# edshkim98/LocalDiffusion-Hallucination

Hardware: AMD Instinct MI355X
Metric: local patches/sec (256^2, T=1000) (higher is better)
Workload: dtype bf16; 1 GPU; cfg3: 8 local patches (vertical band masks) of one 3x256x256 image per GPU, 4-stage dim-32 conditional UNet (12.1M params), DDPM T=1000, pred_x0, sigmoid schedule; patches_per_gpu=8, parallelism=patch-sharded x1, one all-gather per sample, step_graph_replay=True, whole_batch_graph_flag=False, concurrent_sub_batches=2, weight_split_levels=0

## Files before the change

include/localdiff_hip.h:

```cpp
#ifndef LOCALDIFF_HIP_H
#define LOCALDIFF_HIP_H

#include <stddef.h>
#include <stdint.h>

#ifdef __cplusplus
extern "C" {
#endif

#define LD_OK 0
#define LD_EINVAL (-1)
#define LD_EHIP (-2)
#define LD_ETIMEOUT (-3)

#define LD_F32 0
#define LD_BF16 1
#define LD_F16 2

#define LD_STAT_STRIPES 16

#define LD_ACT_NONE 0
#define LD_ACT_SILU 1
#define LD_ACT_RELU 2

const char* ld_last_error(void);
int ld_version(void);
int ld_device_info(char* name, int name_len, int* compute_units, int64_t* global_mem_bytes);
int ld_graph_begin(void* stream);
int ld_graph_end(void* stream, void** graph_exec_out);
int ld_graph_launch(void* graph_exec, void* stream);
int ld_graph_destroy(void* graph_exec);
int ld_memset_zero(void* ptr, size_t bytes, void* stream);
int ld_memset_bytes(void* ptr, int value, size_t bytes, void* stream);
int ld_timing_begin(int max_launches);
int ld_timing_count(void);
int ld_timing_end(float* ms, int cap, int* count);
int ld_timing_end_abs(float* start_ms, float* stop_ms, int cap, int* count);
int ld_event_create(void** ev_out);
int ld_event_record(void* ev, void* stream);
int ld_event_elapsed_ms(void* ev_start, void* ev_stop, float* ms_out);
int ld_event_destroy(void* ev);
int ld_stream_wait_event(void* stream, void* ev);
int ld_tuning_set(const char* name, long long value);
int ld_tuning_get(const char* name, long long* value_out);
int ld_tuning_count(void);
const char* ld_tuning_name(int index);
#define LD_COUNTER_CONV3X3_C32 0
#define LD_COUNTER_CONV3X3_GENERIC 1
#define LD_COUNTER_CONV3X3_S32 2
#define LD_COUNTER_MAX 8
long long ld_counter(int which);
int ld_range_push(const char* name );
int ld_range_pop(void);

typedef struct ld_src {
  const void* data;
  int32_t C;
  int32_t pix_stride;
  int32_t upsample;
  const double* gn_stats;
  const float* gn_gamma;
  const float* gn_beta;
  int32_t gn_groups;
  int32_t act;
  const float* film;
  int32_t film_tstride;
  int32_t film_bstride;
} ld_src;

typedef struct ld_conv3x3_args {
  ld_src src[2];
  int32_t nsrc;
  const void* weight;
  const float* bias;
  void* out;
  double* out_stats;
  int32_t out_groups;
  int32_t B, H, W, Cout;
  const int32_t* t_ptr;
  int32_t dtype;
  const void* addend;
  int32_t weight_terms;
  const void* side_weight;
  const float* side_bias;
  void* side_out;
} ld_conv3x3_args;
int ld_conv3x3(const ld_conv3x3_args* args, void* stream);

#define LD_EPI_PLAIN 0
#define LD_EPI_QKV_LINEAR 1
#define LD_EPI_QKV_FULL 2
#define LD_EPI_RMS_RES 3
#define LD_EPI_RES 4
#define LD_EPI_GN_TAIL 5
typedef struct ld_conv1x1_args {
  ld_src src[2];
  int32_t nsrc;
  int32_t unshuffle;
  int32_t rms_in;
  const void* weight;
  int64_t weight_bstride;
  const float* bias;
  int32_t epilogue;
  int32_t hidden;
  float q_scale;
  const float* g2;
  const void* residual;
  ld_src gn_tail;
  void* out;
  uint32_t* kmax_out;
  int32_t B, H, W, Cout;
  int32_t dtype;
  int32_t weight_terms;
} ld_conv1x1_args;
int ld_conv1x1(const ld_conv1x1_args* args, void* stream);

int ld_pack_conv_weight(const float* w_oihw, const float* scale_in, void* out, int cout, int cin,
                        int ksize, int unshuffle, int dtype, void* stream);
int ld_pack_conv_weight_terms(const float* w_oihw, const float* scale_in, void* out, int cout, int cin,
                              int ksize, int unshuffle, int dtype, int terms, void* stream);

int ld_conv_image(const float* x_nchw, const float* w_oihw, const float* bias, void* out,
                  double* out_stats, int out_groups, int B, int Cin, int H, int W, int ksize,
                  int dtype, void* stream);

size_t ld_stem_packed_bytes(void);
int ld_pack_stem_weight(const float* w_oihw , void* out_packed, int Cin, void* stream);
int ld_conv_stem(const float* x, const void* w_packed, const float* bias, void* out, int B, int Cin, int H, int W,
                 int dtype , void* stream);
typedef struct ld_step_begin_args {
  void* zero_a; size_t bytes_a; void* zero_b; size_t bytes_b;
  int32_t* t_ptr; int delta; int32_t* idx_ptr; const int32_t* t_table;
  const float* film_rows; int row_floats; float* film_cur;
} ld_step_begin_args;
int ld_conv_stem_begin(const float* x, const void* w_packed, const float* bias, void* out, int B, int Cin, int H, int W,
                       int dtype, const ld_step_begin_args* begin, void* stream);


typedef struct ld_gn_apply_args {
  ld_src a;
  ld_src b;
  int32_t final_act;
  int32_t pool;
  void* out;
  int32_t B, H, W;
  const int32_t* t_ptr;
  int32_t dtype;
} ld_gn_apply_args;
int ld_gn_apply(const ld_gn_apply_args* args, void* stream);

int ld_linattn_kmax(const void* qkv, uint32_t* kmax_enc, int B, int n, int heads, int dim_head,
                    int dtype, void* stream);
int ld_linattn_ctx(const void* qkv, const uint32_t* kmax_enc, float* ctx_part,
                   int B, int n, int heads, int dim_head, int nchunks, int dtype, void* stream);
int ld_linattn_ctx_reduce(const float* ctx_part, int nchunks, float* ctxn, int B, int heads,
                          int dim_head, void* stream);
int ld_linattn_fold(const float* ctxn, const float* w_out ,
                    void* w_packed , int B, int C, int heads, int dim_head,
                    int perm, int dtype, void* stream);
int ld_linattn_ctxfold(const float* ctx_part, int nchunks, const float* w_out ,
                       void* w_packed , int B, int C, int heads, int dim_head,
                       int perm, int dtype, void* stream);
int ld_linattn_kvctx(const void* x, const void* wkv_packed, const float* kshift, float* ctx_part, int B,
                     int n, int C, int heads, int dim_head, int nchunks, int dtype, void* stream);
int ld_linattn_out(const void* x, const void* wq_packed, const float* qshift, const void* mfold,
                   const float* bias, const float* g2, void* out, int B, int n, int C, float q_scale,
                   int dtype, void* stream);
int ld_linattn_kvctx_terms(const void* x, const void* wkv_packed, const float* kshift, float* ctx_part, int B, int n, int C,
                           int heads, int dim_head, int nchunks, int dtype, int weight_terms, void* stream);
int ld_linattn_out_terms(const void* x, const void* wq_packed, const float* qshift, const void* mfold, const float* bias,
                         const float* g2, void* out, int B, int n, int C, float q_scale, int dtype, int weight_terms,
                         void* stream);
size_t ld_linattn_ctx_part_floats(int B, int heads, int dim_head, int nchunks);

int ld_attention(const void* qkv, void* out, int B, int n, int heads, int dim_head, int dtype,
                 void* stream);

int ld_time_mlp(const int32_t* times, int n, const float* freqs, int dim, const float* w1,
                const float* b1, const float* w2, const float* b2, int time_dim, float* temb,
                void* stream);
int ld_time_mlp_fourier(const int32_t* times, int n, const float* weights, int learned_dim, const float* w1,
                        const float* b1, const float* w2, const float* b2, int time_dim, float* temb, void* stream);
int ld_film(const float* temb, int n, int time_dim, const float* w, const float* b, int two_c,
            float* film, void* stream);

int ld_final_conv(const void* x, const float* w , const float* b, float* out_nchw,
                  int B, int H, int W, int Cin, int Cout, int dtype, void* stream);

int ld_final_step(const void* x, const float* w, const float* b, float* model_out, float* x_t, float* x0_out,
                  const float* sched, const int32_t* t_ptr, float lo, float hi, int objective, uint64_t seed,
                  int64_t noise_stream, int B, int H, int W, int Cin, int Cout, int dtype, void* stream);


int ld_final_step_at(const void* x, const float* w, const float* b, float* model_out, float* x_t, float* x0_out,
                     const float* sched, const int32_t* t_ptr, float lo, float hi, int objective, uint64_t seed,
                     int64_t noise_base, int64_t noise_tmul, int64_t noise_first, const float* keep_mask,
                     int B, int H, int W, int Cin, int Cout, int dtype, void* stream);

#define LD_OBJ_X0 0
#define LD_OBJ_NOISE 1
#define LD_OBJ_V 2
#define LD_SCHED_COLS 8
#define LD_SCHED_COEF1 0
#define LD_SCHED_COEF2 1
#define LD_SCHED_SIGMA 2
#define LD_SCHED_SQRT_RECIP 3
#define LD_SCHED_SQRT_RECIPM1 4
#define LD_SCHED_SQRT_AB 5
#define LD_SCHED_SQRT_1MAB 6
#define LD_SCHED_ABAR 7

int ld_randn(float* out, int64_t n, uint64_t seed, int64_t stream_base, int64_t stream_tmul,
             const int32_t* t_ptr, void* stream);
int ld_randn_at(float* out, int64_t n, int64_t first, uint64_t seed, int64_t stream_base, int64_t stream_tmul,
                const int32_t* t_ptr, void* stream);
int ld_step_add(int32_t* t_ptr, int delta, void* stream);
int ld_step_begin(void* zero_a, size_t bytes_a, void* zero_b, size_t bytes_b, int32_t* t_ptr, int delta,
                  int32_t* idx_ptr, const int32_t* t_table, void* stream);
int ld_step_begin_film(void* zero_a, size_t bytes_a, void* zero_b, size_t bytes_b, int32_t* t_ptr, int delta,
                       int32_t* idx_ptr, const int32_t* t_table, const float* film_rows, int row_floats,
                       float* film_cur, void* stream);

int ld_ddpm_step(const float* x_t, const float* model_out, const float* noise, float* x_prev,
                 float* x0_out, const float* sched, const int32_t* t_ptr, float lo, float hi,
                 int objective, int64_t n, void* stream);
int ld_ddim_step(const float* x_t, const float* model_out, const float* noise, float* x_next,
                 float sqrt_recip, float sqrt_recipm1, float sqrt_ab, float sqrt_1mab,
                 float sqrt_abar_next, float c, float sigma, float lo, float hi, int objective,
                 int last, int64_t n, void* stream);
int ld_ddim_step_at(const float* x_t, const float* model_out, const float* noise, float* x_next,
                    const float* pair_table, const int32_t* idx_ptr, float lo, float hi, int objective, int64_t n,
                    void* stream);
int ld_branch_conditions(const float* cond, const float* mask, float* cond_out, float* cond_in,
                         float lo_clip, int B, int C, int HW, void* stream);
int ld_mask_out(float* model_out, const float* mask, float min_val, int B, int C, int HW,
                void* stream);
int ld_fuse_ddpm(const float* x_out, const float* x_in, const float* x0_out, const float* x0_in,
                 const float* mask, float* x, float* x0, float lo, float hi, int B, int C, int HW,
                 void* stream);
int ld_branch_conditions_k(const float* cond, const float* masks, float* cond_k, float lo_clip, int B, int C, int K,
                           int HW, void* stream);
int ld_fuse_ddpm_k(const float* x_first, const float* x_rest, const float* x0_first, const float* x0_rest,
                   const float* masks, float* x, float* x0, float lo, float hi, int B, int C, int K, int HW,
                   void* stream);
int ld_posterior_step(const float* x_t, const float* x0, const float* noise, float* x_prev,
                      const float* sched, const int32_t* t_ptr, int64_t n, void* stream);
int ld_fuse_ddim(const float* x_out, const float* x_in, const float* x0_out, const float* x0_in,
                 const float* mask, const float* noise, float* x_next, float sqrt_recip,
                 float sqrt_recipm1, float sqrt_abar_next, float c, float sigma, float lo,
                 float hi, int B, int C, int HW, void* stream);
int ld_fuse_ddim_k(const float* x_first, const float* x_rest, const float* x0_first, const float* x0_rest,
                   const float* masks, const float* noise, float* x_next, float sqrt_recip, float sqrt_recipm1,
                   float sqrt_abar_next, float c, float sigma, float lo, float hi, int B, int C, int K, int HW,
                   void* stream);
int ld_q_sample(const float* x0, const float* noise, float* out, float sqrt_ab, float sqrt_1mab,
                int64_t n, void* stream);
int ld_q_sample_t(const float* x0, const float* noise, float* out, const int* t, const float* sqrt_ab,
                  const float* sqrt_1mab, int B, int64_t elems_per_sample, void* stream);
int ld_p_losses(const float* model_out, const float* x_start, const float* noise, const int* t, const float* sqrt_ab,
                const float* sqrt_1mab, const float* loss_weight, float* loss_out, int B, int64_t elems_per_sample,
                int objective, void* stream);
int ld_recompose(const float* patches , const float* masks , float* out,
                 int B, int K, int C, int HW, void* stream);

#define LD_SEG_SRC_PLAIN 0
#define LD_SEG_SRC_POOL 1
#define LD_SEG_SRC_CAT_D2S 2
typedef struct ld_seg_conv_args {
  const void* src0;
  const void* src1;
  int32_t C0, C1;
  int32_t mode;
  int32_t ksize;
  const float* weight;
  const float* scale;
  const float* shift;
  int32_t relu;
  void* out;
  int32_t B, H, W, Cout;
  int32_t dtype;
} ld_seg_conv_args;
int ld_seg_conv(const ld_seg_conv_args* args, void* stream);
int ld_seg_conv_image(const float* x_nchw, const float* w_oihw, const float* scale, const float* shift, void* out,
                      int B, int Cin, int H, int W, int dtype, void* stream);
int ld_seg_head(const void* x, const float* w, const float* bias, float* logits, float* prob, float* mask,
                int B, int H, int W, int C, int dtype, void* stream);
int ld_seg_pack_weight(const float* w_oihw, float* out, int cout, int cin, int ksize, void* stream);
int ld_seg_pack_convt(const float* w, const float* bias, float* w_out, float* bias_out, int cin, int cout, void* stream);

#define LD_SEG_RED_WORK_BYTES (2048 * 2 * 64 * 8)
int ld_seg_wgrad_splits(int B, int H, int W, int Cin, int Cout, int ksize);
int ld_seg_wgrad(const float* dy, const float* a, float* work, float* dw, int B, int H, int W, int Cin, int Cout,
                 int ksize, int splits, void* stream);
int ld_seg_bn_train(const float* y, const float* gamma, const float* beta, double* work, float* stat, float* running_mean,
                    float* running_var, float momentum, float eps, float* out, int64_t M, int C, void* stream);
int ld_seg_bn_backward(const float* da, const float* act, const float* y, const float* gamma, const float* stat, double* work,
                       float* dgamma, float* dbeta, float* dy, int64_t M, int C, void* stream);
int ld_seg_colsum(const float* x, double* work, float* out, int64_t M, int C, int fold, void* stream);
int ld_seg_pool(const float* x, float* out, int B, int H, int W, int C, void* stream);
int ld_seg_pool_backward(const float* x, const float* dpool, const float* dskip, float* dx, int B, int H, int W, int C,
                         void* stream);
int ld_seg_cat_d2s(const float* skip, const float* low, float* out, int B, int H, int W, int C0, int C1, void* stream);
int ld_seg_cat_d2s_backward(const float* dcat, float* dskip, float* dlow, int B, int H, int W, int C0, int C1, void* stream);
int ld_seg_loss(const float* logits, const float* target, double* work, float* out, float* dz, int64_t M, float pos_weight,
                float dice_eps, void* stream);
int ld_seg_head_backward(const float* dz, const float* x, const float* w, double* work, float* dw, float* db, float* dx,
                         int64_t M, int C, void* stream);
int ld_seg_adam(float* param, const float* grad, float* m, float* v, int d0, int d1, int d2, int64_t s0, int64_t s1,
                int64_t s2, double beta1, double beta2, double eps, double step_size, double bc2_sqrt, void* stream);
int ld_seg_permute3(const float* in, float* out, int d0, int d1, int d2, int64_t off, int64_t s0, int64_t s1, int64_t s2,
                    void* stream);

typedef struct ld_pc_conv_args {
  const float* src;
  const float* weight;
  const float* scale;
  const float* shift;
  const float* residual;
  float* out;
  int32_t B, Hi, Wi, Cin, Ho, Wo, Cout;
  int32_t ksize;
  int32_t stride;
  int32_t relu;
} ld_pc_conv_args;
int ld_pc_conv(const ld_pc_conv_args* args, void* stream);
int ld_pc_stem(const float* x_nchw, const float* w_oihw, const float* scale, const float* shift, float* out,
               int B, int H, int W, void* stream);
int ld_pc_maxpool(const float* x, float* out, int B, int H, int W, int C, void* stream);
int ld_pc_embed(const float* l2, const float* l3, float* rows, float* norms, int B, int h2, int w2, int C2, int h3,
                int w3, int C3, void* stream);
int ld_pc_row_norms(const float* x, float* norms, int64_t n, int d, void* stream);
int ld_pc_knn(const float* q, const float* qn, int N, const float* bank, const float* bn, int64_t M, int D,
              unsigned long long* work, float* dist, int32_t* idx, void* stream);
int ld_pc_knn_topk(const float* q, const float* qn, int N, const float* bank, const float* bn, int64_t M, int D, int k,
                   float* d2, float* dist, int32_t* idx, void* stream);
int ld_pc_score_prepare(const float* patch_scores, const int32_t* loc, const float* bank, const float* bn, int B, int P,
                        int D, float* q, float* qn, int32_t* argmax, void* stream);
int ld_pc_score(const float* rows, const float* row_norms, const float* patch_scores, const int32_t* argmax,
                const float* bank, const float* bn, const int32_t* support, int B, int P, int D, int k, float* pred_score,
                void* stream);
int ld_pc_anomaly_map(const float* scores, const float* g, int ks, float* tmp, float* out, int B, int h, int w, int H,
                      int W, void* stream);

int ld_pc_project(const float* e, int64_t N, int D, const int32_t* rowptr, const int32_t* cols, const float* vals, int k,
                  float* out, int64_t ld, void* stream);
int ld_pc_coreset(const float* ft, int64_t ld, int64_t N, int k, int64_t n, int64_t start, float* min_d,
                  unsigned long long* keys, int64_t* idx, void* stream);

int ld_clf_max(const float* x, int groups, int64_t n, uint32_t* words, void* stream);
enum { LD_CLF_PLAIN = 0, LD_CLF_HALVE = 1, LD_CLF_AFFINE = 2 };
typedef struct ld_clf_resize_args {
  const float* x;
  float* out;
  int32_t B, Cin, Cout, Hi, Wi, Ho, Wo;
  int32_t mode;
  const uint32_t* max_words;
  int32_t per_sample;
  uint32_t* zero_words;
  int32_t n_zero;
  float sub, mul, add, div;
  int32_t normalize;
  float mean[3], std[3];
  const float* pred;
  float threshold;
  int32_t* decision;
  int32_t n_decision;
} ld_clf_resize_args;
int ld_clf_resize(const ld_clf_resize_args* args, void* stream);
int ld_clf_decide(const float* pred_score, float threshold, int32_t* decision, int n, void* stream);

int ld_mc_conv1(const float* x, const float* w, const float* bias, float* out, unsigned char* idx, int B, void* stream);
int ld_mc_pool(const float* x, float* out, unsigned char* idx, int B, int H, int W, int C, void* stream);
int ld_mc_pool_backward(const float* dpool, const float* pooled, const unsigned char* idx, float* dx, int B, int H, int W,
                        int C, void* stream);
int ld_mc_gemm(const float* a, const float* b, float* out, int M, int N, int K, int64_t am, int64_t ak, int64_t bn, int64_t bk,
               int64_t cm, int splits, void* stream);
int ld_mc_fc1_finish(const float* work, const float* bias, float* h, int B, int N, int splits, void* stream);
int ld_mc_head(const float* h, const float* w2, const float* b2, const int64_t* label, float* logits, int64_t* pred,
               float* loss_b, float* dz, float* dh, int32_t* bad_label, int B, void* stream);
int ld_mc_small_grads(const float* dz, const float* h, const float* dh, const float* loss_b, float* gw2, float* gb2, float* gb1,
                      float* loss, int B, void* stream);
int64_t ld_mc_conv1_wgrad_work_floats(int B);
int ld_mc_conv1_wgrad(const float* x, const float* p1, const float* dp1, const unsigned char* idx, float* work, float* gw,
                      float* gb, int B, void* stream);
#define LD_MC_ADAM_MAX 8
typedef struct ld_mc_adam_tensor {
  float* param;
  const float* grad;
  float* m;
  float* v;
  int32_t d0, d1, d2;
  int64_t gs0, gs1, gs2;
  float* mirror0;
  int64_t m0_off, m0_s0, m0_s1, m0_s2;
  float* mirror1;
  int64_t m1_off, m1_s0, m1_s1, m1_s2;
} ld_mc_adam_tensor;
int ld_mc_adam(const ld_mc_adam_tensor* tensors, int count, double beta1, double beta2, double eps, double step_size,
               double bc2_sqrt, void* stream);

int ld_p_losses_grad(const float* model_out, const float* x_start, const float* noise, const int* t, const float* sqrt_ab,
                     const float* sqrt_1mab, const float* loss_weight, float g, float* d_model_out, int B,
                     int64_t elems_per_sample, int objective, void* stream);
int64_t ld_dn_gn_work_bytes(int B, int H, int W, int C);
int ld_dn_gn_forward(const float* y, const float* gamma, const float* beta, const float* film, const float* residual,
                     double* work, float* stat, float* out, int B, int H, int W, int C, int ldc, int groups, void* stream);
int ld_dn_gn_backward(const float* dout, const float* y, const float* stat, const float* gamma, const float* beta,
                      const float* film, double* work, float* dgamma, float* dbeta, float* dfilm, float* dy, int B, int H,
                      int W, int C, int ldc, int groups, void* stream);
int ld_dn_colsum(const float* x, double* work, float* out, int B, int H, int W, int C, int ldc, void* stream);
int ld_dn_time_proj(const float* temb, const float* w, const float* bias, float* film, int B, int T, int N, void* stream);
int ld_dn_time_proj_backward(const float* dfilm, const float* temb, const float* w, float* dw, float* db, float* dtemb, int B,
                             int T, int N, void* stream);
int ld_dn_pack_nhwc(const float* x, float* out, int B, int C, int H, int W, int64_t sb, int64_t sc, int64_t sh, int64_t sw,
                    int ldc, void* stream);
int ld_dn_gather3(const float* in, float* out, int d0, int d1, int d2, int64_t off, int64_t s0, int64_t s1, int64_t s2,
                  void* stream);

int64_t ld_dn_rms_work_bytes(int B, int H, int W, int C);
int ld_dn_rms_forward(const float* x, const float* g, float* rinv, float* out, int B, int H, int W, int C, int ldc,
                      void* stream);
int ld_dn_rms_backward(const float* dout, const float* x, const float* g, const float* rinv, double* work, float* dg, float* dx,
                       int B, int H, int W, int C, int ldc, void* stream);
int ld_dn_la_splits(int B, int heads, int H, int W);
int64_t ld_dn_la_work_bytes(int B, int heads, int H, int W);
int ld_dn_la_context(const float* qkv, double* work, float* ctx, float* kstat, int B, int H, int W, int heads, int ld3,
                     void* stream);
int ld_dn_la_out(const float* qkv, const float* ctx, float* out, int B, int H, int W, int heads, int ld3, int ldo, void* stream);
int ld_dn_la_backward_reduce(const float* qkv, const float* dout, const float* ctx, double* work, float* dctx, float* rk, int B,
                             int H, int W, int heads, int ld3, int ldo, void* stream);
int ld_dn_la_backward_apply(const float* qkv, const float* dout, const float* ctx, const float* kstat, const float* dctx,
                            const float* rk, float* dqkv, int B, int H, int W, int heads, int ld3, int ldo, void* stream);

int ld_dn_fa_forward(const float* qkv, float* out, float* lse, int B, int H, int W, int heads, int ld3, int ldo, void* stream);
int64_t ld_dn_fa_work_bytes(int B, int heads, int H, int W);
int ld_dn_fa_backward(const float* qkv, const float* out, const float* dout, const float* lse, void* work, float* dqkv, int B,
                      int H, int W, int heads, int ld3, int ldo, void* stream);

int ld_dn_space_to_depth(const float* x, float* out, int B, int H, int W, int C, int ldc, void* stream);
int ld_dn_depth_to_space(const float* g, float* dx, int B, int H, int W, int C, int ldc, void* stream);
int ld_dn_upsample2x(const float* x, float* out, int B, int H, int W, int C, int ldc, void* stream);
int ld_dn_upsample2x_backward(const float* g, float* dx, int B, int H, int W, int C, int ldc, void* stream);
int ld_dn_im2col(const float* x, float* out, int B, int Cin, int H, int W, int64_t sb, int64_t sc, int64_t sh, int64_t sw,
                 int ldk, void* stream);
int ld_dn_head_forward(const float* x, const float* w, const float* bias, float* out, int B, int H, int W, int C, int ldc,
                       int O, void* stream);
int ld_dn_head_splits(int B, int H, int W);
int64_t ld_dn_head_work_bytes(int B, int H, int W, int C, int O);
int ld_dn_head_backward(const float* dout, const float* x, const float* w, double* work, float* dw, float* db, float* dx,
                        int B, int H, int W, int C, int ldc, int O, void* stream);

int64_t ld_dn_gnr_work_bytes(int B, int H, int W, int C, int groups);
int ld_dn_gnr_forward(const float* y, const float* gamma, const float* beta, const float* y2, const float* gamma2,
                      const float* beta2, double* work, float* stat, float* stat2, float* out, int B, int H, int W, int C, int ldc,
                      int groups, int relu, void* stream);
int ld_dn_gnr_backward(const float* dout, const float* act, const float* y, const float* stat, const float* gamma,
                       const float* y2, const float* stat2, const float* gamma2, double* work, float* dgamma, float* dbeta,
                       float* dy, float* dgamma2, float* dbeta2, float* dy2, int B, int H, int W, int C, int ldc, int groups,
                       int relu, void* stream);
int ld_dn_im2col3(const float* x, float* out, int B, int Cin, int H, int W, int64_t sb, int64_t sc, int64_t sh, int64_t sw, int ldk,
                  void* stream);

int ld_comm_unique_id(void* id_out_128 );
int ld_comm_init(void** comm_out, const void* id_128 , int world, int rank);
int ld_comm_init_timeout(void** comm_out, const void* id_128 , int world, int rank, double timeout_s);
int ld_allgather(const void* send, void* recv, size_t bytes_per_rank, void* comm, void* stream);
int ld_comm_destroy(void* comm);

#ifdef __cplusplus
}
#endif
#endif
```

localdiffusion-hallucination_amd/_cabi.py:

```python
import ctypes as C
import os

from .tuning import lib_override_path

_HERE = os.path.dirname(os.path.abspath(__file__))

LIB_PATH = lib_override_path() or os.path.join(_HERE, "csrc", "liblocaldiff_hip.so")

LD_F32, LD_BF16, LD_F16 = 0, 1, 2
ACT_NONE, ACT_SILU, ACT_RELU = 0, 1, 2
EPI_PLAIN, EPI_QKV_LINEAR, EPI_QKV_FULL, EPI_RMS_RES, EPI_RES, EPI_GN_TAIL = 0, 1, 2, 3, 4, 5
OBJ = {"pred_x0": 0, "pred_noise": 1, "pred_v": 2}
SCHED_COLS = 8
STAT_STRIPES = 16
COUNTER_CONV3X3_C32, COUNTER_CONV3X3_GENERIC, COUNTER_CONV3X3_S32 = 0, 1, 2
SEG_SRC_PLAIN, SEG_SRC_POOL, SEG_SRC_CAT_D2S = 0, 1, 2
CLF_PLAIN, CLF_HALVE, CLF_AFFINE = 0, 1, 2

vp, i32, i64, u64, f32 = C.c_void_p, C.c_int32, C.c_int64, C.c_uint64, C.c_float


class Src(C.Structure):
    _fields_ = [("data", vp), ("C", i32), ("pix_stride", i32), ("upsample", i32), ("gn_stats", vp),
                ("gn_gamma", vp), ("gn_beta", vp), ("gn_groups", i32), ("act", i32), ("film", vp),
                ("film_tstride", i32), ("film_bstride", i32)]


class Conv3x3Args(C.Structure):
    _fields_ = [("src", Src * 2), ("nsrc", i32), ("weight", vp), ("bias", vp), ("out", vp),
                ("out_stats", vp), ("out_groups", i32), ("B", i32), ("H", i32), ("W", i32),
                ("Cout", i32), ("t_ptr", vp), ("dtype", i32), ("addend", vp), ("weight_terms", i32),
                ("side_weight", vp), ("side_bias", vp), ("side_out", vp)]


class Conv1x1Args(C.Structure):
    _fields_ = [("src", Src * 2), ("nsrc", i32), ("unshuffle", i32), ("rms_in", i32), ("weight", vp),
                ("weight_bstride", i64), ("bias", vp), ("epilogue", i32), ("hidden", i32),
                ("q_scale", f32), ("g2", vp), ("residual", vp), ("gn_tail", Src), ("out", vp), ("kmax_out", vp), ("B", i32), ("H", i32),
                ("W", i32), ("Cout", i32), ("dtype", i32), ("weight_terms", i32)]


class GnApplyArgs(C.Structure):
    _fields_ = [("a", Src), ("b", Src), ("final_act", i32), ("pool", i32), ("out", vp), ("B", i32),
                ("H", i32), ("W", i32), ("t_ptr", vp), ("dtype", i32)]


class StepBeginArgs(C.Structure):
    _fields_ = [("zero_a", vp), ("bytes_a", C.c_size_t), ("zero_b", vp), ("bytes_b", C.c_size_t), ("t_ptr", vp), ("delta", i32),
                ("idx_ptr", vp), ("t_table", vp), ("film_rows", vp), ("row_floats", i32), ("film_cur", vp)]


class SegConvArgs(C.Structure):
    _fields_ = [("src0", vp), ("src1", vp), ("C0", i32), ("C1", i32), ("mode", i32), ("ksize", i32), ("weight", vp),
                ("scale", vp), ("shift", vp), ("relu", i32), ("out", vp), ("B", i32), ("H", i32), ("W", i32),
                ("Cout", i32), ("dtype", i32)]


class PcConvArgs(C.Structure):
    _fields_ = [("src", vp), ("weight", vp), ("scale", vp), ("shift", vp), ("residual", vp), ("out", vp), ("B", i32),
                ("Hi", i32), ("Wi", i32), ("Cin", i32), ("Ho", i32), ("Wo", i32), ("Cout", i32), ("ksize", i32),
                ("stride", i32), ("relu", i32)]


class ClfResizeArgs(C.Structure):
    _fields_ = [("x", vp), ("out", vp), ("B", i32), ("Cin", i32), ("Cout", i32), ("Hi", i32), ("Wi", i32), ("Ho", i32),
                ("Wo", i32), ("mode", i32), ("max_words", vp), ("per_sample", i32), ("zero_words", vp), ("n_zero", i32),
                ("sub", f32), ("mul", f32), ("add", f32), ("div", f32), ("normalize", i32), ("mean", f32 * 3),
                ("std", f32 * 3), ("pred", vp), ("threshold", f32), ("decision", vp), ("n_decision", i32)]


class McAdamTensor(C.Structure):
    _fields_ = [("param", vp), ("grad", vp), ("m", vp), ("v", vp), ("d0", i32), ("d1", i32), ("d2", i32), ("gs0", i64),
                ("gs1", i64), ("gs2", i64), ("mirror0", vp), ("m0_off", i64), ("m0_s0", i64), ("m0_s1", i64), ("m0_s2", i64),
                ("mirror1", vp), ("m1_off", i64), ("m1_s0", i64), ("m1_s1", i64), ("m1_s2", i64)]


_SIGS = {
    "ld_last_error": (C.c_char_p, []),
    "ld_version": (C.c_int, []),
    "ld_device_info": (C.c_int, [C.c_char_p, C.c_int, C.POINTER(C.c_int), C.POINTER(i64)]),
    "ld_graph_begin": (C.c_int, [vp]),
    "ld_graph_end": (C.c_int, [vp, C.POINTER(vp)]),
    "ld_graph_launch": (C.c_int, [vp, vp]),
    "ld_graph_destroy": (C.c_int, [vp]),
    "ld_memset_zero": (C.c_int, [vp, C.c_size_t, vp]),
    "ld_memset_bytes": (C.c_int, [vp, C.c_int, C.c_size_t, vp]),
    "ld_event_create": (C.c_int, [C.POINTER(vp)]),
    "ld_event_record": (C.c_int, [vp, vp]),
    "ld_event_elapsed_ms": (C.c_int, [vp, vp, C.POINTER(f32)]),
    "ld_event_destroy": (C.c_int, [vp]),
    "ld_stream_wait_event": (C.c_int, [vp, vp]),
    "ld_counter": (C.c_longlong, [C.c_int]),
    "ld_tuning_set": (C.c_int, [C.c_char_p, C.c_longlong]),
    "ld_tuning_get": (C.c_int, [C.c_char_p, C.POINTER(C.c_longlong)]),
    "ld_tuning_count": (C.c_int, []),
    "ld_tuning_name": (C.c_char_p, [C.c_int]),
    "ld_range_push": (C.c_int, [C.c_char_p]),
    "ld_range_pop": (C.c_int, []),
    "ld_conv3x3": (C.c_int, [C.POINTER(Conv3x3Args), vp]),
    "ld_conv1x1": (C.c_int, [C.POINTER(Conv1x1Args), vp]),
    "ld_pack_conv_weight": (C.c_int, [vp, vp, vp, C.c_int, C.c_int, C.c_int, C.c_int, C.c_int, vp]),
    "ld_pack_conv_weight_terms": (C.c_int, [vp, vp, vp, C.c_int, C.c_int, C.c_int, C.c_int, C.c_int, C.c_int, vp]),
    "ld_conv_image": (C.c_int, [vp, vp, vp, vp, vp, C.c_int, C.c_int, C.c_int, C.c_int, C.c_int,
                                C.c_int, C.c_int, vp]),
    "ld_stem_packed_bytes": (C.c_size_t, []),
    "ld_pack_stem_weight": (C.c_int, [vp, vp, C.c_int, vp]),
    "ld_conv_stem": (C.c_int, [vp, vp, vp, vp, C.c_int, C.c_int, C.c_int, C.c_int, C.c_int, vp]),
    "ld_conv_stem_begin": (C.c_int, [vp, vp, vp, vp, C.c_int, C.c_int, C.c_int, C.c_int, C.c_int, C.POINTER(StepBeginArgs), vp]),
    "ld_gn_apply": (C.c_int, [C.POINTER(GnApplyArgs), vp]),
    "ld_linattn_kmax": (C.c_int, [vp, vp, C.c_int, C.c_int, C.c_int, C.c_int, C.c_int, vp]),
    "ld_linattn_ctx": (C.c_int, [vp, vp, vp, C.c_int, C.c_int, C.c_int, C.c_int, C.c_int, C.c_int, vp]),
    "ld_linattn_ctx_reduce": (C.c_int, [vp, C.c_int, vp, C.c_int, C.c_int, C.c_int, vp]),
    "ld_linattn_fold": (C.c_int, [vp, vp, vp, C.c_int, C.c_int, C.c_int, C.c_int, C.c_int, C.c_int, vp]),
    "ld_linattn_ctxfold": (C.c_int, [vp, C.c_int, vp, vp, C.c_int, C.c_int, C.c_int, C.c_int, C.c_int, C.c_int, vp]),
    "ld_linattn_kvctx": (C.c_int, [vp, vp, vp, vp, C.c_int, C.c_int, C.c_int, C.c_int, C.c_int, C.c_int, C.c_int, vp]),
    "ld_linattn_out": (C.c_int, [vp, vp, vp, vp, vp, vp, vp, C.c_int, C.c_int, C.c_int, f32, C.c_int, vp]),
    "ld_linattn_kvctx_terms": (C.c_int, [vp, vp, vp, vp, C.c_int, C.c_int, C.c_int, C.c_int, C.c_int, C.c_int, C.c_int, C.c_int, vp]),
    "ld_linattn_out_terms": (C.c_int, [vp, vp, vp, vp, vp, vp, vp, C.c_int, C.c_int, C.c_int, f32, C.c_int, C.c_int, vp]),
    "ld_linattn_ctx_part_floats": (C.c_size_t, [C.c_int, C.c_int, C.c_int, C.c_int]),
    "ld_attention": (C.c_int, [vp, vp, C.c_int, C.c_int, C.c_int, C.c_int, C.c_int, vp]),
    "ld_time_mlp": (C.c_int, [vp, C.c_int, vp, C.c_int, vp, vp, vp, vp, C.c_int, vp, vp]),
    "ld_time_mlp_fourier": (C.c_int, [vp, C.c_int, vp, C.c_int, vp, vp, vp, vp, C.c_int, vp, vp]),
    "ld_film": (C.c_int, [vp, C.c_int, C.c_int, vp, vp, C.c_int, vp, vp]),
    "ld_final_conv": (C.c_int, [vp, vp, vp, vp, C.c_int, C.c_int, C.c_int, C.c_int, C.c_int, C.c_int, vp]),
    "ld_final_step": (C.c_int, [vp, vp, vp, vp, vp, vp, vp, vp, f32, f32, C.c_int, u64, i64, C.c_int, C.c_int, C.c_int,
                                C.c_int, C.c_int, C.c_int, vp]),
    "ld_final_step_at": (C.c_int, [vp, vp, vp, vp, vp, vp, vp, vp, f32, f32, C.c_int, u64, i64, i64, i64, vp, C.c_int,
                                   C.c_int, C.c_int, C.c_int, C.c_int, C.c_int, vp]),
    "ld_timing_begin": (C.c_int, [C.c_int]),
    "ld_timing_count": (C.c_int, []),
    "ld_timing_end": (C.c_int, [vp, C.c_int, vp]),
    "ld_timing_end_abs": (C.c_int, [vp, vp, C.c_int, vp]),
    "ld_randn": (C.c_int, [vp, i64, u64, i64, i64, vp, vp]),
    "ld_randn_at": (C.c_int, [vp, i64, i64, u64, i64, i64, vp, vp]),
    "ld_step_add": (C.c_int, [vp, C.c_int, vp]),
    "ld_step_begin": (C.c_int, [vp, C.c_size_t, vp, C.c_size_t, vp, C.c_int, vp, vp, vp]),
    "ld_step_begin_film": (C.c_int, [vp, C.c_size_t, vp, C.c_size_t, vp, C.c_int, vp, vp, vp, C.c_int, vp, vp]),
    "ld_ddim_step_at": (C.c_int, [vp, vp, vp, vp, vp, vp, f32, f32, C.c_int, i64, vp]),
    "ld_ddpm_step": (C.c_int, [vp, vp, vp, vp, vp, vp, vp, f32, f32, C.c_int, i64, vp]),
    "ld_posterior_step": (C.c_int, [vp, vp, vp, vp, vp, vp, i64, vp]),
    "ld_ddim_step": (C.c_int, [vp, vp, vp, vp, f32, f32, f32, f32, f32, f32, f32, f32, f32, C.c_int,
                               C.c_int, i64, vp]),
    "ld_branch_conditions": (C.c_int, [vp, vp, vp, vp, f32, C.c_int, C.c_int, C.c_int, vp]),
    "ld_mask_out": (C.c_int, [vp, vp, f32, C.c_int, C.c_int, C.c_int, vp]),
    "ld_fuse_ddpm": (C.c_int, [vp, vp, vp, vp, vp, vp, vp, f32, f32, C.c_int, C.c_int, C.c_int, vp]),
    "ld_branch_conditions_k": (C.c_int, [vp, vp, vp, f32, C.c_int, C.c_int, C.c_int, C.c_int, vp]),
    "ld_fuse_ddpm_k": (C.c_int, [vp, vp, vp, vp, vp, vp, vp, f32, f32, C.c_int, C.c_int, C.c_int, C.c_int, vp]),
    "ld_fuse_ddim": (C.c_int, [vp, vp, vp, vp, vp, vp, vp, f32, f32, f32, f32, f32, f32, f32, C.c_int,
                               C.c_int, C.c_int, vp]),
    "ld_fuse_ddim_k": (C.c_int, [vp, vp, vp, vp, vp, vp, vp, f32, f32, f32, f32, f32, f32, f32, C.c_int, C.c_int,
                                 C.c_int, C.c_int, vp]),
    "ld_q_sample": (C.c_int, [vp, vp, vp, f32, f32, i64, vp]),
    "ld_q_sample_t": (C.c_int, [vp, vp, vp, vp, vp, vp, C.c_int, i64, vp]),
    "ld_p_losses": (C.c_int, [vp, vp, vp, vp, vp, vp, vp, vp, C.c_int, i64, C.c_int, vp]),
    "ld_recompose": (C.c_int, [vp, vp, vp, C.c_int, C.c_int, C.c_int, C.c_int, vp]),
    "ld_seg_conv": (C.c_int, [C.POINTER(SegConvArgs), vp]),
    "ld_seg_conv_image": (C.c_int, [vp, vp, vp, vp, vp, C.c_int, C.c_int, C.c_int, C.c_int, C.c_int, vp]),
    "ld_seg_head": (C.c_int, [vp, vp, vp, vp, vp, vp, C.c_int, C.c_int, C.c_int, C.c_int, C.c_int, vp]),
    "ld_seg_pack_weight": (C.c_int, [vp, vp, C.c_int, C.c_int, C.c_int, vp]),
    "ld_seg_pack_convt": (C.c_int, [vp, vp, vp, vp, C.c_int, C.c_int, vp]),
    "ld_seg_wgrad_splits": (C.c_int, [C.c_int, C.c_int, C.c_int, C.c_int, C.c_int, C.c_int]),
    "ld_seg_wgrad": (C.c_int, [vp, vp, vp, vp, C.c_int, C.c_int, C.c_int, C.c_int, C.c_int, C.c_int, C.c_int, vp]),
    "ld_seg_bn_train": (C.c_int, [vp, vp, vp, vp, vp, vp, vp, f32, f32, vp, i64, C.c_int, vp]),
    "ld_seg_bn_backward": (C.c_int, [vp, vp, vp, vp, vp, vp, vp, vp, vp, i64, C.c_int, vp]),
    "ld_seg_colsum": (C.c_int, [vp, vp, vp, i64, C.c_int, C.c_int, vp]),
    "ld_seg_pool": (C.c_int, [vp, vp, C.c_int, C.c_int, C.c_int, C.c_int, vp]),
    "ld_seg_pool_backward": (C.c_int, [vp, vp, vp, vp, C.c_int, C.c_int, C.c_int, C.c_int, vp]),
    "ld_seg_cat_d2s": (C.c_int, [vp, vp, vp, C.c_int, C.c_int, C.c_int, C.c_int, C.c_int, vp]),
    "ld_seg_cat_d2s_backward": (C.c_int, [vp, vp, vp, C.c_int, C.c_int, C.c_int, C.c_int, C.c_int, vp]),
    "ld_seg_loss": (C.c_int, [vp, vp, vp, vp, vp, i64, f32, f32, vp]),
    "ld_seg_head_backward": (C.c_int, [vp, vp, vp, vp, vp, vp, vp, i64, C.c_int, vp]),
    "ld_seg_adam": (C.c_int, [vp, vp, vp, vp, C.c_int, C.c_int, C.c_int, i64, i64, i64, C.c_double, C.c_double, C.c_double,
                    C.c_double, C.c_double, vp]),
    "ld_seg_permute3": (C.c_int, [vp, vp, C.c_int, C.c_int, C.c_int, i64, i64, i64, i64, vp]),
    "ld_pc_conv": (C.c_int, [C.POINTER(PcConvArgs), vp]),
    "ld_pc_stem": (C.c_int, [vp, vp, vp, vp, vp, C.c_int, C.c_int, C.c_int, vp]),
    "ld_pc_maxpool": (C.c_int, [vp, vp, C.c_int, C.c_int, C.c_int, C.c_int, vp]),
    "ld_pc_embed": (C.c_int, [vp, vp, vp, vp, C.c_int, C.c_int, C.c_int, C.c_int, C.c_int, C.c_int, C.c_int, vp]),
    "ld_pc_row_norms": (C.c_int, [vp, vp, i64, C.c_int, vp]),
    "ld_pc_knn": (C.c_int, [vp, vp, C.c_int, vp, vp, i64, C.c_int, vp, vp, vp, vp]),
    "ld_pc_knn_topk": (C.c_int, [vp, vp, C.c_int, vp, vp, i64, C.c_int, C.c_int, vp, vp, vp, vp]),
    "ld_pc_score_prepare": (C.c_int, [vp, vp, vp, vp, C.c_int, C.c_int, C.c_int, vp, vp, vp, vp]),
    "ld_pc_score": (C.c_int, [vp, vp, vp, vp, vp, vp, vp, C.c_int, C.c_int, C.c_int, C.c_int, vp, vp]),
    "ld_pc_anomaly_map": (C.c_int, [vp, vp, C.c_int, vp, vp, C.c_int, C.c_int, C.c_int, C.c_int, C.c_int, vp]),
    "ld_pc_project": (C.c_int, [vp, i64, C.c_int, vp, vp, vp, C.c_int, vp, i64, vp]),
    "ld_pc_coreset": (C.c_int, [vp, i64, i64, C.c_int, i64, i64, vp, vp, vp, vp]),
    "ld_clf_max": (C.c_int, [vp, C.c_int, i64, vp, vp]),
    "ld_clf_resize": (C.c_int, [C.POINTER(ClfResizeArgs), vp]),
    "ld_clf_decide": (C.c_int, [vp, f32, vp, C.c_int, vp]),
    "ld_mc_conv1": (C.c_int, [vp, vp, vp, vp, vp, C.c_int, vp]),
    "ld_mc_pool": (C.c_int, [vp, vp, vp, C.c_int, C.c_int, C.c_int, C.c_int, vp]),
    "ld_mc_pool_backward": (C.c_int, [vp, vp, vp, vp, C.c_int, C.c_int, C.c_int, C.c_int, vp]),
    "ld_mc_gemm": (C.c_int, [vp, vp, vp, C.c_int, C.c_int, C.c_int, i64, i64, i64, i64, i64, C.c_int, vp]),
    "ld_mc_fc1_finish": (C.c_int, [vp, vp, vp, C.c_int, C.c_int, C.c_int, vp]),
    "ld_mc_head": (C.c_int, [vp, vp, vp, vp, vp, vp, vp, vp, vp, vp, C.c_int, vp]),
    "ld_mc_small_grads": (C.c_int, [vp, vp, vp, vp, vp, vp, vp, vp, C.c_int, vp]),
    "ld_mc_conv1_wgrad_work_floats": (i64, [C.c_int]),
    "ld_mc_conv1_wgrad": (C.c_int, [vp, vp, vp, vp, vp, vp, vp, C.c_int, vp]),
    "ld_mc_adam": (C.c_int, [C.POINTER(McAdamTensor), C.c_int, C.c_double, C.c_double, C.c_double, C.c_double, C.c_double, vp]),
    "ld_p_losses_grad": (C.c_int, [vp, vp, vp, vp, vp, vp, vp, f32, vp, C.c_int, i64, C.c_int, vp]),
    "ld_dn_gn_work_bytes": (i64, [C.c_int, C.c_int, C.c_int, C.c_int]),
    "ld_dn_gn_forward": (C.c_int, [vp, vp, vp, vp, vp, vp, vp, vp, C.c_int, C.c_int, C.c_int, C.c_int, C.c_int, C.c_int, vp]),
    "ld_dn_gn_backward": (C.c_int, [vp, vp, vp, vp, vp, vp, vp, vp, vp, vp, vp, C.c_int, C.c_int, C.c_int, C.c_int, C.c_int,
                                    C.c_int, vp]),
    "ld_dn_colsum": (C.c_int, [vp, vp, vp, C.c_int, C.c_int, C.c_int, C.c_int, C.c_int, vp]),
    "ld_dn_time_proj": (C.c_int, [vp, vp, vp, vp, C.c_int, C.c_int, C.c_int, vp]),
    "ld_dn_time_proj_backward": (C.c_int, [vp, vp, vp, vp, vp, vp, C.c_int, C.c_int, C.c_int, vp]),
    "ld_dn_pack_nhwc": (C.c_int, [vp, vp, C.c_int, C.c_int, C.c_int, C.c_int, i64, i64, i64, i64, C.c_int, vp]),
    "ld_dn_gather3": (C.c_int, [vp, vp, C.c_int, C.c_int, C.c_int, i64, i64, i64, i64, vp]),
    "ld_dn_rms_work_bytes": (i64, [C.c_int, C.c_int, C.c_int, C.c_int]),
    "ld_dn_rms_forward": (C.c_int, [vp, vp, vp, vp, C.c_int, C.c_int, C.c_int, C.c_int, C.c_int, vp]),
    "ld_dn_rms_backward": (C.c_int, [vp, vp, vp, vp, vp, vp, vp, C.c_int, C.c_int, C.c_int, C.c_int, C.c_int, vp]),
    "ld_dn_la_splits": (C.c_int, [C.c_int, C.c_int, C.c_int, C.c_int]),
    "ld_dn_la_work_bytes": (i64, [C.c_int, C.c_int, C.c_int, C.c_int]),
    "ld_dn_la_context": (C.c_int, [vp, vp, vp, vp, C.c_int, C.c_int, C.c_int, C.c_int, C.c_int, vp]),
    "ld_dn_la_out": (C.c_int, [vp, vp, vp, C.c_int, C.c_int, C.c_int, C.c_int, C.c_int, C.c_int, vp]),
    "ld_dn_la_backward_reduce": (C.c_int, [vp, vp, vp, vp, vp, vp, C.c_int, C.c_int, C.c_int, C.c_int, C.c_int, C.c_int, vp]),
    "ld_dn_la_backward_apply": (C.c_int, [vp, vp, vp, vp, vp, vp, vp, C.c_int, C.c_int, C.c_int, C.c_int, C.c_int, C.c_int, vp]),
    "ld_dn_fa_forward": (C.c_int, [vp, vp, vp, C.c_int, C.c_int, C.c_int, C.c_int, C.c_int, C.c_int, vp]),
    "ld_dn_fa_work_bytes": (i64, [C.c_int, C.c_int, C.c_int, C.c_int]),
    "ld_dn_fa_backward": (C.c_int, [vp, vp, vp, vp, vp, vp, C.c_int, C.c_int, C.c_int, C.c_int, C.c_int, C.c_int, vp]),
    "ld_dn_space_to_depth": (C.c_int, [vp, vp, C.c_int, C.c_int, C.c_int, C.c_int, C.c_int, vp]),
    "ld_dn_depth_to_space": (C.c_int, [vp, vp, C.c_int, C.c_int, C.c_int, C.c_int, C.c_int, vp]),
    "ld_dn_upsample2x": (C.c_int, [vp, vp, C.c_int, C.c_int, C.c_int, C.c_int, C.c_int, vp]),
    "ld_dn_upsample2x_backward": (C.c_int, [vp, vp, C.c_int, C.c_int, C.c_int, C.c_int, C.c_int, vp]),
    "ld_dn_im2col": (C.c_int, [vp, vp, C.c_int, C.c_int, C.c_int, C.c_int, i64, i64, i64, i64, C.c_int, vp]),
    "ld_dn_head_forward": (C.c_int, [vp, vp, vp, vp, C.c_int, C.c_int, C.c_int, C.c_int, C.c_int, C.c_int, vp]),
    "ld_dn_head_splits": (C.c_int, [C.c_int, C.c_int, C.c_int]),
    "ld_dn_head_work_bytes": (i64, [C.c_int, C.c_int, C.c_int, C.c_int, C.c_int]),
    "ld_dn_head_backward": (C.c_int, [vp, vp, vp, vp, vp, vp, vp, C.c_int, C.c_int, C.c_int, C.c_int, C.c_int, C.c_int, vp]),
    "ld_dn_gnr_work_bytes": (i64, [C.c_int, C.c_int, C.c_int, C.c_int, C.c_int]),
    "ld_dn_gnr_forward": (C.c_int, [vp, vp, vp, vp, vp, vp, vp, vp, vp, vp, C.c_int, C.c_int, C.c_int, C.c_int, C.c_int, C.c_int,
                                    C.c_int, vp]),
    "ld_dn_gnr_backward": (C.c_int, [vp, vp, vp, vp, vp, vp, vp, vp, vp, vp, vp, vp, vp, vp, vp, C.c_int, C.c_int, C.c_int, C.c_int,
                                     C.c_int, C.c_int, C.c_int, vp]),
    "ld_dn_im2col3": (C.c_int, [vp, vp, C.c_int, C.c_int, C.c_int, C.c_int, i64, i64, i64, i64, C.c_int, vp]),
    "ld_comm_unique_id": (C.c_int, [vp]),
    "ld_comm_init": (C.c_int, [C.POINTER(vp), vp, C.c_int, C.c_int]),
    "ld_comm_init_timeout": (C.c_int, [C.POINTER(vp), vp, C.c_int, C.c_int, C.c_double]),
    "ld_allgather": (C.c_int, [vp, vp, C.c_size_t, vp, vp]),
    "ld_comm_destroy": (C.c_int, [vp]),
}

EXPORTS = tuple(_SIGS)
_lib = None


def lib():
    global _lib
    if _lib is not None:
        return _lib
    if not os.path.exists(LIB_PATH):
        raise RuntimeError(
            f"{LIB_PATH} is missing: build it with `python -c 'import __graft_entry__ as g; g.build()'` "
            "(or csrc/build.sh).  There is no CPU fallback for the HIP hot path.")
    try:
        l = C.CDLL(LIB_PATH)
    except OSError as e:
        raise RuntimeError(f"cannot load {LIB_PATH}: {e}") from e
    for name, (res, args) in _SIGS.items():
        try:
            fn = getattr(l, name)
        except AttributeError as e:
            raise RuntimeError(f"{LIB_PATH} does not export {name}") from e
        fn.restype, fn.argtypes = res, args
    _lib = l
    return l


LD_ETIMEOUT = -3


def check(rc, what=""):
    if rc != 0:
        msg = lib().ld_last_error().decode("utf-8", "replace")
        if rc == LD_ETIMEOUT:
            raise TimeoutError(f"localdiff_hip {what} timed out: {msg}")
        raise RuntimeError(f"localdiff_hip {what} failed (rc={rc}): {msg}")


class prof_range:

    def __init__(self, name):
        self.name = name.encode()

    def __enter__(self):
        lib().ld_range_push(self.name)

    def __exit__(self, *exc):
        lib().ld_range_pop()


def ptr(t):
    return None if t is None else t.data_ptr()


def dtype_code(name):
    return {"fp32": LD_F32, "float32": LD_F32, "bf16": LD_BF16, "bfloat16": LD_BF16, "fp16": LD_F16, "float16": LD_F16,
            "half": LD_F16}[name]
```

localdiffusion-hallucination_amd/csrc/conv3x3.hip:

```cpp
#include "common.hip.h"
#include <stdlib.h>

int ld_conv3x3_c32_try(const ld_conv3x3_args* p, hipStream_t st);
int ld_conv3x3_s32_try(const ld_conv3x3_args* p, hipStream_t st);
#ifdef LD_DEBUG_VARIANTS
int ld_conv3x3_ksplit_try(const ld_conv3x3_args* p, hipStream_t st);
int ld_conv3x3_ring_try(const ld_conv3x3_args* p, hipStream_t st);
#endif

#include "conv3x3_body.hip.h"

namespace {

#ifdef LD_DEBUG_VARIANTS
int g_span_shape[1024][5];
#endif

template <typename T, int MT, int NW, bool DEEP, int DBG, bool SK = false, bool RAW = false, bool SIDE = false>
int launch_dbg(const Conv3Dev& a, hipStream_t st) {
  constexpr int TR = 4 * NW, HR = TR + 2, HC = 18;
  constexpr int NPIXP = (HR * HC + 15) / 16 * 16;
  const int ctot = a.s[0].C + (a.nsrc > 1 ? a.s[1].C : 0);
  const size_t lds = (SK ? 2 : 1) * (4 * NPIXP * 16 + (9 + (SIDE ? 1 : 0)) * MT * 1024) + 2 * ctot * sizeof(float) + 4 * 2 * 16 * MT * sizeof(double);
  Conv3Dev d = a;
  d.tiles_x = (a.W + 15) / 16;
  const int tiles_y = (a.H + TR - 1) / TR;
  dim3 grid(d.tiles_x * tiles_y, a.Cout / (16 * MT), a.B);
  if (lds > 65536) LD_HIP(ld_allow_lds(conv3x3_kernel<T, MT, NW, DEEP, DBG, SK, RAW, SIDE>, lds));
  LD_LAUNCH((conv3x3_kernel<T, MT, NW, DEEP, DBG, SK, RAW, SIDE>), grid, dim3(SK ? 512 : 256), lds, st, d.s[0].data, d.w, d.H, d.W, d.tiles_x,
            d.s[0].C, d.s[0].ld, d.s[0].ups, d.nsrc, d.wsplit, d.Cout, d);
  LD_LAUNCH_CHECK("conv3x3");
  return LD_OK;
}

template <typename T, int MT, int NW, bool DEEP>
int launch(const Conv3Dev& a, hipStream_t st) {
#ifdef LD_DEBUG_VARIANTS
  if constexpr (std::is_same<T, bf16>::value && !DEEP) {
    switch (a.dbg & 255) {
      case 1: return launch_dbg<T, MT, NW, DEEP, 1>(a, st);
      case 2: return launch_dbg<T, MT, NW, DEEP, 2>(a, st);
      case 3: return launch_dbg<T, MT, NW, DEEP, 3>(a, st);
      case 4: return launch_dbg<T, MT, NW, DEEP, 4>(a, st);
      case 7: return launch_dbg<T, MT, NW, DEEP, 7>(a, st);
      case 8: return launch_dbg<T, MT, NW, DEEP, 8>(a, st);
      case 12: return launch_dbg<T, MT, NW, DEEP, 12>(a, st);
      case 15: return launch_dbg<T, MT, NW, DEEP, 15>(a, st);
      case 64: return launch_dbg<T, MT, NW, DEEP, 64>(a, st);
      case 128:
        if (!a.s[0].stats && !(a.nsrc > 1 && a.s[1].stats)) return launch_dbg<T, MT, NW, DEEP, 128, false, true>(a, st);
        return launch_dbg<T, MT, NW, DEEP, 128>(a, st);
      default: break;
    }
  }
#endif
  if constexpr (!DEEP) {
    const bool raw = !a.s[0].stats && !(a.nsrc > 1 && a.s[1].stats);
    if (raw && ld_tuning().conv_raw) return launch_dbg<T, MT, NW, DEEP, 0, false, true>(a, st);
  }
  return launch_dbg<T, MT, NW, DEEP, 0>(a, st);
}

template <typename T>
int dispatch(const Conv3Dev& a, hipStream_t st) {
#ifdef LD_DEBUG_VARIANTS
  static const int force_mt = getenv("LD_CONV_MT") ? atoi(getenv("LD_CONV_MT")) : 0;
  static const int force_nw = getenv("LD_CONV_NW") ? atoi(getenv("LD_CONV_NW")) : 0;
#else
  constexpr int force_mt = 0, force_nw = 0;
#endif
  const LdTuning& tn = ld_tuning();
  bool mt4 = (a.Cout % 64) == 0;
  const long mt4_min = tn.conv_mt4_min_wgs;
  if (mt4 && (long)((a.W + 15) / 16) * ((a.H + 7) / 8) * (a.Cout / 64) * a.B < mt4_min) mt4 = false;
  const long blocks16 = (long)((a.W + 15) / 16) * ((a.H + 15) / 16) * (a.Cout / (mt4 ? 64 : 32)) * a.B;
  const long big_min = tn.conv_big_min;
  bool big = blocks16 >= big_min && a.H >= 16 && !mt4;
  if (mt4 && a.H >= 16 && blocks16 >= tn.conv_big4_min) big = true;
  if (force_mt == 2) mt4 = false;
  if (force_mt == 4 && (a.Cout % 64) == 0) mt4 = true;
  if (force_nw == 2) big = false;
  if (force_nw == 4) big = true;
#ifdef LD_DEBUG_VARIANTS
  static const int force_deep = getenv("LD_CONV_DEEP") ? atoi(getenv("LD_CONV_DEEP")) : -1;
#else
  constexpr int force_deep = -1;
#endif
  const int ck = sizeof(T) == 4 ? 16 : 32;
  const int nch = (a.s[0].C + (a.nsrc > 1 ? a.s[1].C : 0)) / ck;
  const long wg = (long)((a.W + 15) / 16) * ((a.H + 7) / 8) * (a.Cout / (mt4 ? 64 : 32)) * a.B;
  bool deep = false;
  if (force_deep >= 0) deep = force_deep != 0;
  if constexpr (sizeof(T) == 2) {
    if (a.w2) {
      if (mt4) return launch_dbg<T, 4, 2, false, 0, false, true, true>(a, st);
      return launch_dbg<T, 2, 2, false, 0, false, true, true>(a, st);
    }
  }
  const int force_sk = (int)tn.conv_sk;
  const long sk_max_wgs = tn.conv_sk_max_wgs;
  bool sk = force_sk >= 1 && sizeof(T) == 2 && !big && !deep && ((nch >= 8 && wg <= sk_max_wgs) || force_sk == 2);
  if constexpr (sizeof(T) == 2) {
    if (sk) return mt4 ? launch_dbg<T, 4, 2, false, 0, true>(a, st) : launch_dbg<T, 2, 2, false, 0, true>(a, st);
  }
#ifdef LD_DEBUG_VARIANTS
  if (deep && !big) return mt4 ? launch<T, 4, 2, true>(a, st) : launch<T, 2, 2, true>(a, st);
#endif
  (void)deep;
  if (mt4) return big ? launch<T, 4, 4, false>(a, st) : launch<T, 4, 2, false>(a, st);
  return big ? launch<T, 2, 4, false>(a, st) : launch<T, 2, 2, false>(a, st);
}

}

#ifdef LD_DEBUG_VARIANTS
extern "C" int ld_debug_conv_spans(unsigned long long* spans, int* shapes) {
  LD_HIP(hipDeviceSynchronize());
  LD_HIP(hipMemcpyFromSymbol(spans, HIP_SYMBOL(g_conv_span), sizeof(unsigned long long) * 2048));
  for (int i = 0; i < 1024 * 5; ++i) shapes[i] = g_span_shape[i / 5][i % 5];
  return LD_OK;
}
#endif

extern "C" int ld_debug_conv_trace(unsigned long long* host) {
  LD_HIP(hipDeviceSynchronize());
  LD_HIP(hipMemcpyFromSymbol(host, HIP_SYMBOL(g_conv_trace), sizeof(unsigned long long) * 24));
  return LD_OK;
}

extern "C" int ld_conv3x3(const ld_conv3x3_args* p, void* stream) {
  LD_REQUIRE(p != nullptr, "ld_conv3x3: null args");
  LD_REQUIRE(p->nsrc == 1 || p->nsrc == 2, "ld_conv3x3: nsrc must be 1 or 2 (got %d)", p->nsrc);
  LD_REQUIRE(ld_dtype_ok(p->dtype), "ld_conv3x3: bad dtype %d", p->dtype);
  LD_REQUIRE(p->Cout > 0 && p->Cout % 32 == 0, "ld_conv3x3: Cout %d must be a multiple of 32", p->Cout);
  LD_REQUIRE(p->B > 0 && p->H > 0 && p->W > 0, "ld_conv3x3: bad shape");
  LD_REQUIRE(p->weight && p->bias && p->out, "ld_conv3x3: null weight/bias/out");
  Conv3Dev a;
  a.nsrc = p->nsrc;
  for (int s = 0; s < p->nsrc; ++s) {
    const ld_src& S = p->src[s];
    LD_REQUIRE(S.data != nullptr, "ld_conv3x3: src[%d] null", s);
    LD_REQUIRE(S.C > 0 && S.C % 32 == 0, "ld_conv3x3: src[%d].C=%d must be a multiple of 32", s, S.C);
    if (S.upsample) LD_REQUIRE(p->H % 2 == 0 && p->W % 2 == 0, "ld_conv3x3: upsample needs even H,W");
    if (S.gn_stats) {
      LD_REQUIRE(S.gn_groups <= 16, "ld_conv3x3: src[%d] gn_groups %d > 16 (the stripe reduction uses 16 lanes per group)", s, S.gn_groups);
      LD_REQUIRE(S.gn_gamma && S.gn_beta && S.gn_groups > 0 && S.C % S.gn_groups == 0,
                 "ld_conv3x3: src[%d] GroupNorm prologue incomplete", s);
    }
    a.s[s] = to_dev(S);
  }
  if (p->nsrc == 1) a.s[1] = a.s[0];
  if (p->out_stats) {
    LD_REQUIRE(p->out_groups > 0 && p->Cout % p->out_groups == 0 && (p->Cout / p->out_groups) <= 32,
               "ld_conv3x3: out_groups %d incompatible with Cout %d", p->out_groups, p->Cout);
  }
  a.w = p->weight; a.bias = p->bias; a.out = p->out; a.ostats = p->out_stats;
  a.ogroups = p->out_groups > 0 ? p->out_groups : 1;
  a.B = p->B; a.H = p->H; a.W = p->W; a.Cout = p->Cout; a.t_ptr = p->t_ptr; a.tiles_x = 0;
  a.addend = p->addend;
  a.w2 = p->side_weight; a.bias2 = p->side_bias; a.out2 = p->side_out;
  if (p->side_weight) {
    LD_REQUIRE(ld_dtype_16(p->dtype), "ld_conv3x3: the side (res_conv) output needs 16-bit storage");
    LD_REQUIRE(p->side_bias && p->side_out, "ld_conv3x3: side_weight without side_bias / side_out");
    LD_REQUIRE(p->weight_terms != 2 && !p->addend, "ld_conv3x3: the side output does not combine with two-term weights or an addend");
    for (int s = 0; s < p->nsrc; ++s)
      LD_REQUIRE(!p->src[s].gn_stats && !p->src[s].upsample, "ld_conv3x3: the side output needs raw, un-resampled sources (a ResnetBlock's block1)");
  }
  LD_REQUIRE(p->weight_terms >= 0 && p->weight_terms <= 2 && !(p->weight_terms == 2 && !ld_dtype_16(p->dtype)),
             "ld_conv3x3: weight_terms %d (2 needs 16-bit storage)", p->weight_terms);
  a.wsplit = p->weight_terms == 2 ? 1 : 0;
  a.dbg = 0;
#ifdef LD_DEBUG_VARIANTS
  static const int dbg = getenv("LD_CONV_DEBUG") ? atoi(getenv("LD_CONV_DEBUG")) : 0;
  a.dbg = dbg;
  if (dbg == 128) {
    static int calls = 0;
    const int slot = calls++ & 1023;
    g_span_shape[slot][0] = p->B; g_span_shape[slot][1] = p->H; g_span_shape[slot][2] = p->W;
    g_span_shape[slot][3] = p->src[0].C + (p->nsrc > 1 ? p->src[1].C : 0); g_span_shape[slot][4] = p->Cout;
    a.dbg = 128 | (slot << 8);
  }
#endif
  hipStream_t st = reinterpret_cast<hipStream_t>(stream);
  if (p->side_weight) {
    ld_count(LD_COUNTER_CONV3X3_GENERIC);
    return LD_DISPATCH16(p->dtype, dispatch<T>(a, st));
  }
  if (p->weight_terms != 2) {
    const int rc = ld_conv3x3_c32_try(p, st);
    if (rc != 0) return rc < 0 ? rc : LD_OK;
  }
  {
    const int rc = ld_conv3x3_s32_try(p, st);
    if (rc != 0) return rc < 0 ? rc : LD_OK;
  }
#ifdef LD_DEBUG_VARIANTS
  {
    const int rc = ld_conv3x3_ring_try(p, st);
    if (rc != 0) return rc < 0 ? rc : LD_OK;
  }
  static const int ksplit = getenv("LD_CONV_KSPLIT") ? atoi(getenv("LD_CONV_KSPLIT")) : 0;
  if (ksplit && p->weight_terms != 2) {
    const int rc = ld_conv3x3_ksplit_try(p, st);
    if (rc != 0) return rc < 0 ? rc : LD_OK;
  }
#endif
  ld_count(LD_COUNTER_CONV3X3_GENERIC);
  return LD_DISPATCH(p->dtype, dispatch<T>(a, st));
}
```

localdiffusion-hallucination_amd/csrc/conv3x3_body.hip.h:

```cpp
#pragma once
#include "common.hip.h"

namespace {

struct Conv3Dev {
  SrcDev s[2];
  const void* w;
  const float* bias;
  void* out;
  double* ostats;
  const int* t_ptr;
  const void* addend;
  const void* w2;
  const float* bias2;
  void* out2;
  int nsrc;
  int ogroups;
  int B, H, W, Cout;
  int tiles_x;
  int wsplit;
  int dbg;
};

__device__ unsigned long long g_conv_trace[24];
__device__ unsigned long long g_conv_span[1024][2];
#define TR_STAMP(k) do { if ((DBG & 64) && tracing) tr_t[k] = __builtin_readcyclecounter(); } while (0)

typedef const Conv3Dev __attribute__((address_space(4)))* Conv3KernargPtr;
template <typename T, int MT, int NW, bool DEEP, int DBG, bool SK = false, bool RAW = false, bool SIDE = false>
__device__ __forceinline__ void conv3x3_tile(const Conv3Dev& head, Conv3KernargPtr rest, const int bx, const int by, const int bz,
                                             const int gdx, const int gdz, char* smem) {
  Conv3Dev a = head;
  constexpr int E = DT<T>::E, CK = DT<T>::CK;
  constexpr int TR = 4 * NW, TC = 16, HR = TR + 2, HC = TC + 2;
  constexpr int NPIX = HR * HC, NPIXP = (NPIX + 15) / 16 * 16, PLANE = NPIXP * 16;
  constexpr int ITER = (NPIXP + 63) / 64;
  constexpr int UNITS = 9 * MT * 64, WU = (UNITS + 255) / 256;
  constexpr bool P = DT<T>::precise;

  static_assert(!SIDE || (RAW && !SK && !DEEP && MT * NW < 16 && sizeof(T) == 2), "SIDE: RAW 16-bit launches of the small register tiles");
  constexpr int STAGE = 4 * PLANE + (9 + (SIDE ? 1 : 0)) * MT * 1024;
  const int half = SK ? (int)(threadIdx.x >> 8) : 0;
  char* s_x = smem + half * STAGE;
  char* s_w = s_x + 4 * PLANE;
  char* s_w2 = s_w + 9 * MT * 1024;
  float* s_coef = reinterpret_cast<float*>(smem + (SK ? 2 : 1) * STAGE);
  double* s_stat;

  const int tid = threadIdx.x & 255, lane = tid & 63, wv = tid >> 6, px = lane & 15, kq = lane >> 4;
  unsigned long long tr_t[24] = {0};
  const bool tracing = (DBG & 64) && threadIdx.x == 0 && bz == gdz / 2 && by == 0 &&
                       bx == (gdx * 5) / 8;
  TR_STAMP(0);
  if ((DBG & 128) && threadIdx.x == 0 && bx == 0 && by == 0 && bz == 0)
    g_conv_span[(a.dbg >> 8) & 1023][0] = __builtin_amdgcn_s_memrealtime();
  const int b = bz, m0 = by * MT;
  int ty_, tx_;
  tile_of(bx, a.tiles_x, gdx / a.tiles_x, ty_, tx_);
  const int ty0 = ty_ * TR, tx0 = tx_ * TC;
  const int H = a.H, W = a.W;
  const int nch0 = a.s[0].C / CK;
  const int ws = a.wsplit;
  int nch = 0;
  if constexpr (SK) nch = (nch0 + (a.nsrc > 1 ? a.s[1].C / CK : 0)) << ws;
  const int mt_total = a.Cout / 16;
  const uint4* wg = reinterpret_cast<const uint4*>(a.w);

  uint4 hxA[ITER], wxA[WU], hxB[DEEP ? ITER : 1], wxB[DEEP ? WU : 1];
  uint4 wx2 = make_uint4(0u, 0u, 0u, 0u);
  unsigned hvalid = 0;
  unsigned hoffb0[ITER], hoffb1[ITER];
  const char* sbase0;
  const char* sbase1;
  auto src_base = [&](const SrcDev& S, unsigned (&hoffb)[ITER]) -> const char* {
    const int Hs = S.ups ? H / 2 : H, Ws = S.ups ? W / 2 : W;
    const int row0 = S.ups ? (ty0 - 1) >> 1 : ty0 - 1, col0 = S.ups ? (tx0 - 1) >> 1 : tx0 - 1;
#pragma unroll
    for (int it = 0; it < ITER; ++it) {
      const int q = (it * 4 + wv) * 16 + px;
      const int hy = (q * 3641) >> 16, hx_ = q - hy * HC;
      const int gy = ty0 - 1 + hy, gx = tx0 - 1 + hx_;
      const int r = (S.ups ? gy >> 1 : gy) - row0, c = (S.ups ? gx >> 1 : gx) - col0;
      hoffb[it] = (__umul24(__umul24(r, Ws) + c, S.ld) + kq * E) * (unsigned)sizeof(T);
    }
    return reinterpret_cast<const char*>(S.data) + (((long)b * Hs + row0) * Ws + col0) * S.ld * (long)sizeof(T);
  };
  auto second_source = [&]() {
    if (a.nsrc > 1) sbase1 = src_base(a.s[1], hoffb1);
    else {
#pragma unroll
      for (int it = 0; it < ITER; ++it) hoffb1[it] = hoffb0[it];
    }
  };
#pragma unroll
  for (int it = 0; it < ITER; ++it) {
    const int q = (it * 4 + wv) * 16 + px;
    const int hy = (q * 3641) >> 16, hx_ = q - hy * HC;
    const int gy = ty0 - 1 + hy, gx = tx0 - 1 + hx_;
    if (q < NPIX && gy >= 0 && gy < H && gx >= 0 && gx < W && !(DBG & 1)) hvalid |= 1u << it;
  }
  sbase0 = src_base(a.s[0], hoffb0);
  sbase1 = sbase0;
  if constexpr (SK) second_source();
  unsigned woffb[WU];
#pragma unroll
  for (int k = 0; k < WU; ++k) {
    const int u = k * 256 + tid;
    const int tap = u / (MT * 64), r = u - tap * (MT * 64);
    woffb[k] = (u < UNITS && !(DBG & 2)) ? (__umul24(tap, mt_total) + m0) * 1024u + r * 16u : ~0u;
  }
  const long wstride = 9L * mt_total * 1024;
  auto issue_loads = [&](int ch, uint4 (&hx)[ITER], uint4 (&wx)[WU], auto first_tag) {
    constexpr bool FIRST = decltype(first_tag)::value;
    const int cs = ch >> ws;
    const int si = FIRST ? 0 : (cs >= nch0 ? 1 : 0);
    const char* sp = (si ? sbase1 : sbase0) + (long)(cs - si * nch0) * CK * (long)sizeof(T);
    const bool same_halo = !SK && !DEEP && ws && (ch & 1);
    const char* wc = reinterpret_cast<const char*>(wg) + (long)ch * wstride;
#pragma unroll
    for (int k = 0; k < WU; ++k) {
      wx[k] = make_uint4(0u, 0u, 0u, 0u);
      if (woffb[k] != ~0u) wx[k] = *reinterpret_cast<const uint4*>(wc + woffb[k]);
    }
    if constexpr (SIDE && !FIRST) {
      if (tid < MT * 64) wx2 = *reinterpret_cast<const uint4*>(reinterpret_cast<const char*>(a.w2) + ((long)ch * mt_total + m0) * 1024 + tid * 16);
    }
    if (!same_halo) {
#pragma unroll
      for (int it = 0; it < ITER; ++it) {
        hx[it] = make_uint4(0u, 0u, 0u, 0u);
        if ((hvalid >> it) & 1u) {
          const u32x4 v = load16_act(sp + (FIRST ? hoffb0[it] : (si ? hoffb1[it] : hoffb0[it])));
          hx[it] = make_uint4(v[0], v[1], v[2], v[3]);
        }
      }
    }
  };
  auto write_lds = [&](int ch, const uint4 (&hx)[ITER], const uint4 (&wx)[WU]) {
    const int csrc = ch >> ws;
    const int si = csrc >= nch0 ? 1 : 0;
    const SrcDev S = si ? a.s[1] : a.s[0];
    const int c0 = (csrc - si * nch0) * CK;
    const int coef_off = si ? 2 * a.s[0].C : 0;
    const bool has_coef = !RAW && S.stats != nullptr;
    float ca[E], cs[E];
    if (has_coef) {
      const float* cap = s_coef + coef_off + c0 + kq * E;
#pragma unroll
      for (int e = 0; e < E; ++e) { ca[e] = cap[e]; cs[e] = cap[S.C + e]; }
    }
    const bool same_halo = !SK && !DEEP && ws && (ch & 1);
#pragma unroll
    for (int k = 0; k < WU; ++k) {
      const int u = k * 256 + tid;
      if (u < UNITS) *reinterpret_cast<uint4*>(s_w + (size_t)u * 16) = wx[k];
    }
    if constexpr (SIDE) {
      if (tid < MT * 64) *reinterpret_cast<uint4*>(s_w2 + tid * 16) = wx2;
    }
#pragma unroll
    for (int it = 0; it < ITER; ++it) {
      const int q = (it * 4 + wv) * 16 + px;
      if (q < NPIXP && !same_halo) {
        uint4 raw = hx[it];
        if (has_coef && ((hvalid >> it) & 1u)) {
          float v[E];
          unpack16<T>(raw, v);
          affine_act_n<P, E>(v, ca, cs, S.act);
          raw = pack16<T>(v);
        }
        *reinterpret_cast<uint4*>(s_x + kq * PLANE + q * 16) = raw;
      }
    }
  };

  TR_STAMP(1);
  if constexpr (SK) { if (half < nch) issue_loads(half, hxA, wxA, std::false_type{}); }
  else issue_loads(0, hxA, wxA, std::true_type{});
  TR_STAMP(2);
  if (rest) {
    Conv3KernargPtr pr = rest;
    asm volatile("" : "+s"(pr));
    a.s[1].data = pr->s[1].data; a.s[1].stats = pr->s[1].stats; a.s[1].gamma = pr->s[1].gamma; a.s[1].beta = pr->s[1].beta;
    a.s[1].film = pr->s[1].film; a.s[1].C = pr->s[1].C; a.s[1].ld = pr->s[1].ld; a.s[1].ups = pr->s[1].ups;
    a.s[1].groups = pr->s[1].groups; a.s[1].act = pr->s[1].act; a.s[1].film_tstride = pr->s[1].film_tstride;
    a.s[1].film_bstride = pr->s[1].film_bstride;
    a.s[0].stats = pr->s[0].stats; a.s[0].gamma = pr->s[0].gamma; a.s[0].beta = pr->s[0].beta; a.s[0].film = pr->s[0].film;
    a.s[0].groups = pr->s[0].groups; a.s[0].act = pr->s[0].act; a.s[0].film_tstride = pr->s[0].film_tstride;
    a.s[0].film_bstride = pr->s[0].film_bstride;
    a.bias = pr->bias; a.out = pr->out; a.ostats = pr->ostats; a.t_ptr = pr->t_ptr; a.addend = pr->addend;
    a.ogroups = pr->ogroups; a.B = pr->B; a.dbg = pr->dbg;
    if constexpr (SIDE) { a.w2 = pr->w2; a.bias2 = pr->bias2; a.out2 = pr->out2; }
  }
  if constexpr (!SK) second_source();
  {
    const int c1 = a.nsrc > 1 ? a.s[1].C : 0;
    nch = (nch0 + c1 / CK) << ws;
    s_stat = reinterpret_cast<double*>(s_coef + 2 * (a.s[0].C + c1));
  }
  asm volatile("" ::"s"(a.bias), "s"(a.out), "s"(a.ostats), "s"(a.ogroups), "s"(a.addend), "s"(a.s[1].C), "s"(a.s[1].ld), "s"(a.s[1].ups),
               "s"(a.s[1].data), "s"(a.s[0].stats), "s"(a.s[0].gamma), "s"(a.s[0].beta), "s"(a.s[0].film), "s"(a.s[0].groups), "s"(a.s[0].act));
  float4 bias[MT];
#pragma unroll
  for (int m = 0; m < MT; ++m) bias[m] = *reinterpret_cast<const float4*>(a.bias + (m0 + m) * 16 + kq * 4);
  float4 bias2[SIDE ? MT : 1];
  if constexpr (SIDE) {
    asm volatile("" ::"s"(a.w2), "s"(a.bias2), "s"(a.out2));
    if (tid < MT * 64) wx2 = *reinterpret_cast<const uint4*>(reinterpret_cast<const char*>(a.w2) + (long)m0 * 1024 + tid * 16);
#pragma unroll
    for (int m = 0; m < MT; ++m) bias2[m] = *reinterpret_cast<const float4*>(a.bias2 + (m0 + m) * 16 + kq * 4);
  }

  {
    const bool any = !RAW && (a.s[0].stats != nullptr || (a.nsrc > 1 && a.s[1].stats != nullptr));
    if (any) {
      const int trow = a.t_ptr ? *a.t_ptr : 0;
      int off = 0;
      for (int s = 0; s < a.nsrc; ++s) {
        const SrcDev S = s ? a.s[1] : a.s[0];
        if (S.stats) {
          const long npix = S.ups ? (long)(H / 2) * (W / 2) : (long)H * W;
          build_gn_coef<DT<T>::precise>(S, b, trow, npix, s_coef + off, s_stat, (int)threadIdx.x, SK ? 512 : 256);
        }
        off += 2 * S.C;
      }
    }
  }

  TR_STAMP(3);
  f32x4 acc[MT][NW];
  f32x4 acc2[SIDE ? MT : 1][SIDE ? NW : 1];
#pragma unroll
  for (int m = 0; m < MT; ++m)
#pragma unroll
    for (int j = 0; j < NW; ++j) {
      acc[m][j] = f32x4{0.f, 0.f, 0.f, 0.f};
      if constexpr (SIDE) acc2[m][j] = f32x4{0.f, 0.f, 0.f, 0.f};
    }

  auto compute = [&]() {
    if (DBG & 4) return;
    if constexpr (MT * NW >= 16) {
      uint4 A[2][3], Bq[2][NW + 2];
      auto load_b = [&](int dx, int set) {
#pragma unroll
        for (int rr = 0; rr < NW + 2; ++rr)
          Bq[set][rr] = *reinterpret_cast<const uint4*>(s_x + kq * PLANE + (((wv * NW + rr) * HC + dx + px) * 16));
      };
      auto load_a = [&](int dx, int m, int set) {
#pragma unroll
        for (int dy = 0; dy < 3; ++dy)
          A[set][dy] = *reinterpret_cast<const uint4*>(s_w + ((dy * 3 + dx) * MT + m) * 1024 + lane * 16);
      };
      load_b(0, 0);
      load_a(0, 0, 0);
#pragma unroll
      for (int dx = 0; dx < 3; ++dx) {
        if (dx + 1 < 3) load_b(dx + 1, (dx + 1) & 1);
#pragma unroll
        for (int m = 0; m < MT; ++m) {
          const int idx = dx * MT + m;
          if (idx + 1 < 3 * MT) load_a((idx + 1) / MT, (idx + 1) % MT, (idx + 1) & 1);
#pragma unroll
          for (int rr = 0; rr < NW + 2; ++rr) {
#pragma unroll
            for (int dy = 0; dy < 3; ++dy) {
              const int j = rr - dy;
              if (j >= 0 && j < NW) mma16<T>(acc[m][j], A[idx & 1][dy], Bq[dx & 1][rr]);
            }
          }
        }
      }
      return;
    }
    uint4 A[2][3][MT], Bq[2][NW + 2];
    auto load_frags = [&](int dx, int set) {
#pragma unroll
      for (int dy = 0; dy < 3; ++dy)
#pragma unroll
        for (int m = 0; m < MT; ++m)
          A[set][dy][m] = *reinterpret_cast<const uint4*>(s_w + ((dy * 3 + dx) * MT + m) * 1024 + lane * 16);
#pragma unroll
      for (int rr = 0; rr < NW + 2; ++rr)
        Bq[set][rr] = *reinterpret_cast<const uint4*>(s_x + kq * PLANE + (((wv * NW + rr) * HC + dx + px) * 16));
    };
    load_frags(0, 0);
    uint4 A2[SIDE ? MT : 1];
    if constexpr (SIDE) {
#pragma unroll
      for (int m = 0; m < MT; ++m) A2[m] = *reinterpret_cast<const uint4*>(s_w2 + m * 1024 + lane * 16);
    }
#pragma unroll
    for (int dx = 0; dx < 3; ++dx) {
      if (dx + 1 < 3) load_frags(dx + 1, (dx + 1) & 1);
#pragma unroll
      for (int rr = 0; rr < NW + 2; ++rr) {
#pragma unroll
        for (int dy = 0; dy < 3; ++dy) {
          const int j = rr - dy;
          if (j >= 0 && j < NW) {
#pragma unroll
            for (int m = 0; m < MT; ++m) mma16<T>(acc[m][j], A[dx & 1][dy][m], Bq[dx & 1][rr]);
            if constexpr (SIDE) {
              if (dx == 1 && dy == 1) {
#pragma unroll
                for (int m = 0; m < MT; ++m) mma16<T>(acc2[m][j], A2[m], Bq[dx & 1][rr]);
              }
            }
          }
        }
      }
    }
  };
  if constexpr (SK) {
    for (int k = 0; k <= nch; ++k) {
      __syncthreads();
      if ((k & 1) == half) {
        if (k < nch) {
          write_lds(k, hxA, wxA);
          if (k + 2 < nch) issue_loads(k + 2, hxA, wxA, std::false_type{});
        }
      } else if (k >= 1) {
        compute();
      }
    }
    __syncthreads();
    float4* s_red = reinterpret_cast<float4*>(smem + STAGE);
    if (half == 1) {
#pragma unroll
      for (int m = 0; m < MT; ++m)
#pragma unroll
        for (int j = 0; j < NW; ++j)
          s_red[(m * NW + j) * 256 + tid] = make_float4(acc[m][j][0], acc[m][j][1], acc[m][j][2], acc[m][j][3]);
    }
    __syncthreads();
    if (half == 0) {
#pragma unroll
      for (int m = 0; m < MT; ++m)
#pragma unroll
        for (int j = 0; j < NW; ++j) {
          const float4 o = s_red[(m * NW + j) * 256 + tid];
          acc[m][j][0] += o.x; acc[m][j][1] += o.y; acc[m][j][2] += o.z; acc[m][j][3] += o.w;
        }
    }
  } else if constexpr (!DEEP) {
    for (int ch = 0; ch < nch; ++ch) {
      __syncthreads();
      if (ch == 0) TR_STAMP(4);
      if (ch == 2) TR_STAMP(11);
      write_lds(ch, hxA, wxA);
      if (ch == 0) TR_STAMP(5);
      if (ch == 2) TR_STAMP(12);
      __syncthreads();
      if (ch == 0) TR_STAMP(6);
      if (ch == 2) TR_STAMP(13);
      if (ch + 1 < nch) issue_loads(ch + 1, hxA, wxA, std::false_type{});
      if (ch == 2) TR_STAMP(14);
      compute();
      if (ch == 0) TR_STAMP(7);
      if (ch == 2) TR_STAMP(15);
    }
    TR_STAMP(8);
  } else {
    if (nch > 1) issue_loads(1, hxB, wxB, std::false_type{});
    for (int ch = 0; ch < nch; ch += 2) {
      __syncthreads();
      write_lds(ch, hxA, wxA);
      __syncthreads();
      if (ch + 2 < nch) issue_loads(ch + 2, hxA, wxA, std::false_type{});
      compute();
      if (ch + 1 < nch) {
        __syncthreads();
        write_lds(ch + 1, hxB, wxB);
        __syncthreads();
        if (ch + 3 < nch) issue_loads(ch + 3, hxB, wxB, std::false_type{});
        compute();
      }
    }
  }

  const int gx = tx0 + px;
  const long obase = (((long)b * H + ty0) * W + tx0) * a.Cout + m0 * 16;
  char* outb = reinterpret_cast<char*>(a.out) + obase * (long)sizeof(T);
  const char* addb = reinterpret_cast<const char*>(a.addend) + obase * (long)sizeof(T);
  const unsigned lane_off = (__umul24(__umul24(wv * NW, W) + px, a.Cout) + kq * 4) * (unsigned)sizeof(T);
  const unsigned row_off = __umul24(W, a.Cout) * (unsigned)sizeof(T);
  float ssum[MT][4], ssq[MT][4];
#pragma unroll
  for (int m = 0; m < MT; ++m)
#pragma unroll
    for (int r = 0; r < 4; ++r) ssum[m][r] = ssq[m][r] = 0.f;
#pragma unroll
  for (int m = 0; m < MT; ++m) asm volatile("" ::"v"(bias[m].x), "v"(bias[m].y), "v"(bias[m].z), "v"(bias[m].w));
  if constexpr (SIDE) {
#pragma unroll
    for (int m = 0; m < MT; ++m) asm volatile("" ::"v"(bias2[m].x), "v"(bias2[m].y), "v"(bias2[m].z), "v"(bias2[m].w));
  }
  const bool rows_in = ty0 + TR <= H && tx0 + TC <= W;
  auto emit = [&](auto full_tag) {
    constexpr bool FULL = decltype(full_tag)::value;
    typename Raw4<T>::type ad[FULL ? 1 : MT][FULL ? 1 : NW];
    if constexpr (!FULL) {
      if (a.addend) {
#pragma unroll
        for (int m = 0; m < MT; ++m)
#pragma unroll
          for (int j = 0; j < NW; ++j) {
            const int gy = ty0 + wv * NW + j;
            const bool in = rows_in || (gy < H && gx < W);
            const unsigned off = lane_off + j * row_off + m * 16 * (unsigned)sizeof(T);
            ad[m][j] = load4_raw<T>(reinterpret_cast<const T*>(addb + (in ? off : 0u)));
          }
#pragma unroll
        for (int m = 0; m < MT; ++m)
#pragma unroll
          for (int j = 0; j < NW; ++j) pin_raw4(ad[m][j]);
      }
    }
    constexpr int MS = sizeof(T) == 2 ? 2 : 1;
    static_assert(MT % 2 == 0, "m-tiles are stored in pairs");
#pragma unroll
    for (int m = 0; m < MT; m += MS) {
#pragma unroll
      for (int j = 0; j < NW; ++j) {
        const int gy = ty0 + wv * NW + j;
        const bool valid = FULL || ((rows_in || (gy < H && gx < W)) && half == 0);
        float v[MS][4];
#pragma unroll
        for (int mm = 0; mm < MS; ++mm) {
          const float4 bv = bias[m + mm];
          v[mm][0] = acc[m + mm][j][0] + bv.x; v[mm][1] = acc[m + mm][j][1] + bv.y;
          v[mm][2] = acc[m + mm][j][2] + bv.z; v[mm][3] = acc[m + mm][j][3] + bv.w;
          if constexpr (!FULL) {
            if (a.addend) {
              float av[4];
              unpack4<T>(ad[m + mm][j], av);
#pragma unroll
              for (int r = 0; r < 4; ++r) v[mm][r] += av[r];
            }
          }
        }
        if constexpr (MS == 2) {
          const uint4 w16 = pair_frag16<T>(v[0], v[1]);
          const unsigned off = lane_off - kq * 4 * (unsigned)sizeof(T) + j * row_off + m * 16 * (unsigned)sizeof(T) + pair_frag16_off(kq);
          if (valid && !(DBG & 8)) store16_out(outb + off, w16);
        } else {
          const unsigned off = lane_off + j * row_off + m * 16 * (unsigned)sizeof(T);
          if (valid && !(DBG & 8)) store4<T>(reinterpret_cast<T*>(outb + off), v[0]);
        }
        if (valid) {
#pragma unroll
          for (int mm = 0; mm < MS; ++mm)
#pragma unroll
            for (int r = 0; r < 4; ++r) { ssum[m + mm][r] += v[mm][r]; ssq[m + mm][r] += v[mm][r] * v[mm][r]; }
        }
      }
    }
  };
  if (rows_in && !a.addend && half == 0) emit(std::true_type{});
  else emit(std::false_type{});
  if constexpr (SIDE) {
    char* out2b = reinterpret_cast<char*>(a.out2) + obase * (long)sizeof(T);
#pragma unroll
    for (int m = 0; m < MT; m += 2) {
#pragma unroll
      for (int j = 0; j < NW; ++j) {
        const int gy = ty0 + wv * NW + j;
        const bool valid = rows_in || (gy < H && gx < W);
        float v[2][4];
#pragma unroll
        for (int mm = 0; mm < 2; ++mm) {
          const float4 bv = bias2[m + mm];
          v[mm][0] = acc2[m + mm][j][0] + bv.x; v[mm][1] = acc2[m + mm][j][1] + bv.y;
          v[mm][2] = acc2[m + mm][j][2] + bv.z; v[mm][3] = acc2[m + mm][j][3] + bv.w;
        }
        const uint4 w16 = pair_frag16<T>(v[0], v[1]);
        const unsigned off = lane_off - kq * 4 * (unsigned)sizeof(T) + j * row_off + m * 16 * (unsigned)sizeof(T) + pair_frag16_off(kq);
        if (valid) store16_out(out2b + off, w16);
      }
    }
  }
  TR_STAMP(9);
  if (a.ostats) {
    __syncthreads();
    TR_STAMP(16);
    const int gs = a.Cout / a.ogroups;
    const int ngrp_blk = (16 * MT) / gs;
    const int stripe = bx % LD_STAT_STRIPES;
    if (!P && (gs & 3) == 0) {
#pragma unroll
      for (int m = 0; m < MT; ++m) {
        const float s1 = wave16_sum((ssum[m][0] + ssum[m][1]) + (ssum[m][2] + ssum[m][3]));
        const float s2 = wave16_sum((ssq[m][0] + ssq[m][1]) + (ssq[m][2] + ssq[m][3]));
        if (px == 0 && half == 0) {
          s_stat[(wv * 2 + 0) * 4 * MT + m * 4 + kq] = (double)s1;
          s_stat[(wv * 2 + 1) * 4 * MT + m * 4 + kq] = (double)s2;
        }
      }
      TR_STAMP(17);
      __syncthreads();
      TR_STAMP(18);
      const int q4 = gs >> 2;
      if ((q4 & (q4 - 1)) == 0) {
        if (tid < 32 && half == 0) {
          const int k = tid >> 4, e = tid & 15;
          double v = 0.0;
          if (e < 4 * MT) {
#pragma unroll
            for (int w4 = 0; w4 < 4; ++w4) v += s_stat[(w4 * 2 + k) * 4 * MT + e];
          }
          v = row_group_sum_d(v, q4);
          if (e < 4 * MT && (e & (q4 - 1)) == 0) {
            const int g = (m0 * 16) / gs + e / q4;
            atomicAdd(&a.ostats[(((size_t)b * LD_STAT_STRIPES + stripe) * a.ogroups + g) * 2 + k], v);
          }
        }
      } else if (tid < 2 * ngrp_blk && half == 0) {
        const int gi = tid >> 1, k = tid & 1;
        double acc1 = 0.0;
        for (int w4 = 0; w4 < 4; ++w4)
          for (int c = 0; c < q4; ++c) acc1 += s_stat[(w4 * 2 + k) * 4 * MT + gi * q4 + c];
        const int g = (m0 * 16) / gs + gi;
        atomicAdd(&a.ostats[(((size_t)b * LD_STAT_STRIPES + stripe) * a.ogroups + g) * 2 + k], acc1);
      }
    } else {
#pragma unroll
      for (int m = 0; m < MT; ++m)
#pragma unroll
        for (int r = 0; r < 4; ++r) {
          const float s1 = wave16_sum(ssum[m][r]), s2 = wave16_sum(ssq[m][r]);
          if (px == 0 && half == 0) {
            s_stat[(wv * 2 + 0) * 16 * MT + m * 16 + kq * 4 + r] = (double)s1;
            s_stat[(wv * 2 + 1) * 16 * MT + m * 16 + kq * 4 + r] = (double)s2;
          }
        }
      __syncthreads();
      if (tid < 2 * ngrp_blk && half == 0) {
        const int gi = tid >> 1, k = tid & 1;
        double acc1 = 0.0;
        for (int w4 = 0; w4 < 4; ++w4)
          for (int c = 0; c < gs; ++c) acc1 += s_stat[(w4 * 2 + k) * 16 * MT + gi * gs + c];
        const int g = (m0 * 16) / gs + gi;
        atomicAdd(&a.ostats[(((size_t)b * LD_STAT_STRIPES + stripe) * a.ogroups + g) * 2 + k], acc1);
      }
    }
  }
  if ((DBG & 128) && threadIdx.x == 0) {
    asm volatile("s_waitcnt vmcnt(0)" ::: "memory");
    atomicMax(&g_conv_span[(a.dbg >> 8) & 1023][1], (unsigned long long)__builtin_amdgcn_s_memrealtime());
  }
  if ((DBG & 64) && tracing) {
    tr_t[19] = __builtin_readcyclecounter();
    asm volatile("s_waitcnt vmcnt(0)" ::: "memory");
    tr_t[10] = __builtin_readcyclecounter();
#pragma unroll
    for (int k = 0; k < 24; ++k) g_conv_trace[k] = tr_t[k];
  }
}

template <typename T, int MT, int NW, bool DEEP, int DBG, bool SK = false, bool RAW = false, bool SIDE = false>
__global__ __launch_bounds__(SK ? 512 : 256) __attribute__((amdgpu_waves_per_eu(SK ? 2 : (MT == 2 ? 3 : 1), SK ? 2 : (MT == 2 ? 3 : 2))))
void conv3x3_kernel(const void* data0, const void* w, int H, int W, int tiles_x, int C0, int ld0, int ups0, int nsrc, int wsplit, int Cout,
                    Conv3Dev rest) {
  extern __shared__ __attribute__((aligned(16))) char smem[];
  Conv3Dev a{};
  a.s[0].data = data0; a.w = w; a.H = H; a.W = W; a.tiles_x = tiles_x; a.s[0].C = C0; a.s[0].ld = ld0; a.s[0].ups = ups0;
  a.nsrc = nsrc; a.wsplit = wsplit; a.Cout = Cout;
  constexpr unsigned REST_OFF = ld_kernarg_offset<const void*, const void*, int, int, int, int, int, int, int, int, int>(alignof(Conv3Dev));
  static_assert(REST_OFF == 56, "conv3x3_kernel: leading arguments changed");
  typedef const char __attribute__((address_space(4)))* KChar;
  Conv3KernargPtr pr = (Conv3KernargPtr)((KChar)__builtin_amdgcn_kernarg_segment_ptr() + REST_OFF);
  if constexpr (SK) {
    a = rest;
    a.tiles_x = tiles_x;
    conv3x3_tile<T, MT, NW, DEEP, DBG, SK, RAW>(a, nullptr, blockIdx.x, blockIdx.y, blockIdx.z, gridDim.x, gridDim.z, smem);
  } else {
    conv3x3_tile<T, MT, NW, DEEP, DBG, SK, RAW, SIDE>(a, pr, blockIdx.x, blockIdx.y, blockIdx.z, gridDim.x, gridDim.z, smem);
  }
}

}
```

localdiffusion-hallucination_amd/csrc/conv3x3_s32.hip:

```cpp
#include "common.hip.h"

namespace {

struct S32Dev {
  const void* data1;
  const double* stats;
  const float* gamma;
  const float* beta;
  const float* film;
  const float* bias;
  void* out;
  double* ostats;
  int ld1, film_bstride, act, ogroups;
};

constexpr int TR = 16, TC = 16, HR = 18, HC = 18, NPIX = HR * HC, NPIXP = 336, PLANE = NPIXP * 16, ITER = 6, WU = 5, MT = 2, NW = 4;
constexpr int S32_LDS = 4 * PLANE + 9 * MT * 1024;

typedef const S32Dev __attribute__((address_space(4)))* S32KernargPtr;

template <typename T, int NCH, bool PRO>
__global__ __launch_bounds__(256) __attribute__((amdgpu_waves_per_eu(4, 4)))
void conv3x3_s32_kernel(const void* data0, const void* wts, int hw, int ld0, int c0, S32Dev rest_) {
  static_assert(sizeof(T) == 2, "16-bit storage only");
  static_assert(!PRO || NCH == 1, "the prologue variant stages one chunk");
  constexpr int E = 8;
  __shared__ __attribute__((aligned(256))) char smem[S32_LDS];
  char* s_x = smem;
  char* s_w = smem + 4 * PLANE;

  const int tid = threadIdx.x, lane = tid & 63, wv = tid >> 6, px = lane & 15, kq = lane >> 4;
  const int H = hw & 0xffff, W = hw >> 16;
  const int tiles_x = W >> 4;
  const int bx = blockIdx.x, b = blockIdx.z;
  int ty_, tx_;
  tile_of(bx, tiles_x, H >> 4, ty_, tx_);
  const int ty0 = ty_ * TR, tx0 = tx_ * TC;

  unsigned hvalid = 0, hoff[ITER];
#pragma unroll
  for (int it = 0; it < ITER; ++it) {
    const int q = (it * 4 + wv) * 16 + px;
    const int hy = (q * 3641) >> 16, hx_ = q - hy * HC;
    const int gy = ty0 - 1 + hy, gx = tx0 - 1 + hx_;
    const bool in = q < NPIX && gy >= 0 && gy < H && gx >= 0 && gx < W;
    if (in) hvalid |= 1u << it;
    hoff[it] = in ? (unsigned)(__umul24(gy, W) + gx) : 0u;
  }
  const long img_px = (long)b * H * W;
  u32x4 hx[ITER], wx[WU];
  auto issue_w = [&](int ch) {
    const char* wc = reinterpret_cast<const char*>(wts) + (long)ch * (9 * MT * 1024);
#pragma unroll
    for (int k = 0; k < WU; ++k) {
      const int u = k * 256 + tid;
      wx[k] = u32x4{0u, 0u, 0u, 0u};
      if (u < 9 * MT * 64) wx[k] = *reinterpret_cast<const u32x4*>(wc + u * 16);
    }
  };
  auto issue_h = [&](const void* data, int ld, int coff) {
    const char* sp = reinterpret_cast<const char*>(data) + (img_px * ld + coff + kq * E) * (long)sizeof(T);
    const unsigned ldb = (unsigned)ld * (unsigned)sizeof(T);
#pragma unroll
    for (int it = 0; it < ITER; ++it) {
      hx[it] = u32x4{0u, 0u, 0u, 0u};
      if ((hvalid >> it) & 1u) hx[it] = load16_act(sp + (size_t)hoff[it] * ldb);
    }
  };
  issue_w(0);
  issue_h(data0, ld0, 0);

  constexpr unsigned REST_OFF = ld_kernarg_offset<const void*, const void*, int, int, int>(alignof(S32Dev));
  typedef const char __attribute__((address_space(4)))* KChar;
  S32KernargPtr pr = (S32KernargPtr)((KChar)__builtin_amdgcn_kernarg_segment_ptr() + REST_OFF);
  asm volatile("" : "+s"(pr));
  S32Dev a;
  a.data1 = pr->data1; a.stats = pr->stats; a.gamma = pr->gamma; a.beta = pr->beta; a.film = pr->film; a.bias = pr->bias;
  a.out = pr->out; a.ostats = pr->ostats; a.ld1 = pr->ld1; a.film_bstride = pr->film_bstride; a.act = pr->act; a.ogroups = pr->ogroups;
  (void)rest_;

  float ca[PRO ? E : 1], cs[PRO ? E : 1];
  if constexpr (PRO) {
    const float* fp = a.film ? a.film + (long)b * a.film_bstride : a.gamma;
    const int c = kq * E;
    const f32x4 g0 = *reinterpret_cast<const f32x4*>(a.gamma + c), g1 = *reinterpret_cast<const f32x4*>(a.gamma + c + 4);
    const f32x4 b0 = *reinterpret_cast<const f32x4*>(a.beta + c), b1 = *reinterpret_cast<const f32x4*>(a.beta + c + 4);
    const f32x4 fs0 = *reinterpret_cast<const f32x4*>(fp + c), fs1 = *reinterpret_cast<const f32x4*>(fp + c + 4);
    const f32x4 fh0 = *reinterpret_cast<const f32x4*>(fp + (a.film ? 32 : 0) + c), fh1 = *reinterpret_cast<const f32x4*>(fp + (a.film ? 32 : 0) + c + 4);
    constexpr int SPL = LD_STAT_STRIPES / 16;
    typedef __attribute__((ext_vector_type(2))) double f64x2;
    f64x2 q0[SPL], q1[SPL];
#pragma unroll
    for (int k = 0; k < SPL; ++k) {
      const double* sp = a.stats + (((size_t)b * LD_STAT_STRIPES + k * 16 + px) * 8 + 2 * kq) * 2;
      q0[k] = *reinterpret_cast<const f64x2*>(sp);
      q1[k] = *reinterpret_cast<const f64x2*>(sp + 2);
    }
    __builtin_amdgcn_sched_barrier(0);
    f64x2 t0 = q0[0], t1 = q1[0];
#pragma unroll
    for (int k = 1; k < SPL; ++k) { t0 += q0[k]; t1 += q1[k]; }
    double s1[2] = {row_group_sum_d(t0[0], 16), row_group_sum_d(t1[0], 16)};
    double s2[2] = {row_group_sum_d(t0[1], 16), row_group_sum_d(t1[1], 16)};
    float mean[2], rstd[2];
    const double inv_n = (double)__builtin_amdgcn_rcpf((float)((long)H * W) * 4.0f);
#pragma unroll
    for (int g = 0; g < 2; ++g) {
      const double m = s1[g] * inv_n;
      double var = s2[g] * inv_n - m * m;
      var = var > 0.0 ? var : 0.0;
      mean[g] = (float)m;
      rstd[g] = __builtin_amdgcn_rsqf((float)(var + 1e-5));
    }
    const float gam[E] = {g0[0], g0[1], g0[2], g0[3], g1[0], g1[1], g1[2], g1[3]};
    const float bet[E] = {b0[0], b0[1], b0[2], b0[3], b1[0], b1[1], b1[2], b1[3]};
    const float fsc[E] = {fs0[0], fs0[1], fs0[2], fs0[3], fs1[0], fs1[1], fs1[2], fs1[3]};
    const float fsh[E] = {fh0[0], fh0[1], fh0[2], fh0[3], fh1[0], fh1[1], fh1[2], fh1[3]};
#pragma unroll
    for (int e = 0; e < E; ++e) {
      float aa = rstd[e >> 2] * gam[e];
      float ss = bet[e] - mean[e >> 2] * aa;
      if (a.film) {
        const float sc = fsc[e] + 1.0f;
        aa *= sc;
        ss = ss * sc + fsh[e];
      }
      ca[e] = aa;
      cs[e] = ss;
    }
  }
  f32x4 bias[MT];
  f32x4 acc[MT][NW];
#pragma unroll
  for (int m = 0; m < MT; ++m)
#pragma unroll
    for (int j = 0; j < NW; ++j) acc[m][j] = f32x4{0.f, 0.f, 0.f, 0.f};

#pragma unroll
  for (int ch = 0; ch < NCH; ++ch) {
    if (ch > 0) __syncthreads();
#pragma unroll
    for (int k = 0; k < WU; ++k) {
      const int u = k * 256 + tid;
      if (u < 9 * MT * 64) *reinterpret_cast<u32x4*>(s_w + u * 16) = wx[k];
    }
#pragma unroll
    for (int it = 0; it < ITER; ++it) {
      const int q = (it * 4 + wv) * 16 + px;
      if (q < NPIXP) {
        u32x4 raw = hx[it];
        if constexpr (PRO) {
          if ((hvalid >> it) & 1u) {
            float v[E];
            unpack16<T>(make_uint4(raw[0], raw[1], raw[2], raw[3]), v);
            affine_act_n<false, E>(v, ca, cs, a.act);
            const uint4 p = pack16<T>(v);
            raw = u32x4{p.x, p.y, p.z, p.w};
          }
        }
        *reinterpret_cast<u32x4*>(s_x + kq * PLANE + q * 16) = raw;
      }
    }
    __syncthreads();
    if (ch + 1 < NCH) {
      if (c0 > 32) issue_h(data0, ld0, 32);
      else issue_h(a.data1, a.ld1, 0);
    } else {
#pragma unroll
      for (int m = 0; m < MT; ++m) bias[m] = *reinterpret_cast<const f32x4*>(a.bias + m * 16 + kq * 4);
    }
#pragma unroll
    for (int dx = 0; dx < 3; ++dx) {
      uint4 Bq[NW + 2];
#pragma unroll
      for (int rr = 0; rr < NW + 2; ++rr)
        Bq[rr] = *reinterpret_cast<const uint4*>(s_x + kq * PLANE + (((wv * NW + rr) * HC + dx + px) * 16));
#pragma unroll
      for (int dy = 0; dy < 3; ++dy) {
        uint4 A[MT];
#pragma unroll
        for (int m = 0; m < MT; ++m) A[m] = *reinterpret_cast<const uint4*>(s_w + ((dy * 3 + dx) * MT + m) * 1024 + lane * 16);
#pragma unroll
        for (int j = 0; j < NW; ++j)
#pragma unroll
          for (int m = 0; m < MT; ++m) mma16<T>(acc[m][j], A[m], Bq[j + dy]);
      }
    }
    if (ch + 1 < NCH) issue_w(ch + 1);
  }

  asm volatile("" ::"v"(bias[0]), "v"(bias[1]));
  char* outp = reinterpret_cast<char*>(a.out) + ((img_px + (long)(ty0 + wv * NW) * W + tx0) * 32) * (long)sizeof(T);
  const unsigned lane_off = (unsigned)px * 64u + pair_frag16_off(kq);
  const unsigned row_off = (unsigned)W * 64u;
  float s1[MT] = {0.f, 0.f}, s2[MT] = {0.f, 0.f};
#pragma unroll
  for (int j = 0; j < NW; ++j) {
    float v[MT][4];
#pragma unroll
    for (int m = 0; m < MT; ++m)
#pragma unroll
      for (int r = 0; r < 4; ++r) v[m][r] = acc[m][j][r] + bias[m][r];
    store16_out(outp + lane_off + j * row_off, pair_frag16<T>(v[0], v[1]));
#pragma unroll
    for (int m = 0; m < MT; ++m) {
      s1[m] += (v[m][0] + v[m][1]) + (v[m][2] + v[m][3]);
      s2[m] += (v[m][0] * v[m][0] + v[m][1] * v[m][1]) + (v[m][2] * v[m][2] + v[m][3] * v[m][3]);
    }
  }
  if (a.ostats) {
    double* s_stat = reinterpret_cast<double*>(s_w);
    __syncthreads();
#pragma unroll
    for (int m = 0; m < MT; ++m) {
      const float t1 = wave16_sum(s1[m]), t2 = wave16_sum(s2[m]);
      if (px == 0) {
        s_stat[(wv * 2 + 0) * 8 + m * 4 + kq] = (double)t1;
        s_stat[(wv * 2 + 1) * 8 + m * 4 + kq] = (double)t2;
      }
    }
    __syncthreads();
    if (tid < 32) {
      const int k = tid >> 4, e = tid & 15;
      const int gs = 32 / a.ogroups, q4 = gs >> 2;
      double v = 0.0;
      if (e < 8) {
#pragma unroll
        for (int w4 = 0; w4 < 4; ++w4) v += s_stat[(w4 * 2 + k) * 8 + e];
      }
      v = row_group_sum_d(v, q4);
      if (e < 8 && (e & (q4 - 1)) == 0)
        atomicAdd(&a.ostats[(((size_t)b * LD_STAT_STRIPES + (bx % LD_STAT_STRIPES)) * a.ogroups + e / q4) * 2 + k], v);
    }
  }
}

template <typename T, int NCH, bool PRO>
int launch_s32(const ld_conv3x3_args* p, hipStream_t st) {
  S32Dev d{};
  const ld_src& s0 = p->src[0];
  d.data1 = p->nsrc > 1 ? p->src[1].data : nullptr;
  d.ld1 = p->nsrc > 1 ? (p->src[1].pix_stride > 0 ? p->src[1].pix_stride : p->src[1].C) : 0;
  d.stats = s0.gn_stats; d.gamma = s0.gn_gamma; d.beta = s0.gn_beta; d.film = s0.film;
  d.film_bstride = s0.film_bstride; d.act = s0.act;
  d.bias = p->bias; d.out = p->out; d.ostats = p->out_stats; d.ogroups = p->out_groups > 0 ? p->out_groups : 1;
  const int ld0 = s0.pix_stride > 0 ? s0.pix_stride : s0.C;
  const dim3 grid((p->W / 16) * (p->H / 16), 1, p->B);
  LD_LAUNCH((conv3x3_s32_kernel<T, NCH, PRO>), grid, dim3(256), 0, st, s0.data, p->weight, p->H | (p->W << 16), ld0, s0.C, d);
  LD_LAUNCH_CHECK("conv3x3_s32");
  return LD_OK;
}

}

int ld_conv3x3_s32_try(const ld_conv3x3_args* p, hipStream_t st) {
  const LdTuning& tn = ld_tuning();
  if (!tn.conv_s32 || !ld_dtype_16(p->dtype) || p->Cout != 32 || p->addend || p->weight_terms == 2) return 0;
  if (p->H % 16 != 0 || p->W % 16 != 0 || p->H >= 65536 || p->W >= 32768) return 0;
  const long tiles = (long)(p->W / 16) * (p->H / 16) * p->B;
  if (tiles < tn.conv_s32_min_tiles) return 0;
  int ctot = 0;
  bool pro = false;
  for (int s = 0; s < p->nsrc; ++s) {
    const ld_src& S = p->src[s];
    if (S.upsample) return 0;
    const long ld = S.pix_stride > 0 ? S.pix_stride : S.C;
    if ((long)p->H * p->W * ld * 2 >= (1L << 32)) return 0;
    ctot += S.C;
    pro = pro || S.gn_stats != nullptr;
  }
  if (ctot != 32 && ctot != 64) return 0;
  if (p->nsrc == 2 && (p->src[0].C != 32 || p->src[1].C != 32)) return 0;
  if (pro) {
    const ld_src& S = p->src[0];
    if (p->nsrc != 1 || S.C != 32 || S.gn_groups != 8 || p->t_ptr != nullptr) return 0;
    if (!S.gn_gamma || !S.gn_beta) return 0;
  }
  if (p->out_stats) {
    const int og = p->out_groups;
    if (og <= 0 || 32 % og != 0 || 32 / og < 4) return 0;
  }
  if (!(tn.conv_s32 & (pro ? 2 : (ctot == 32 ? 1 : 4)))) return 0;
  int rc;
  if (pro) rc = LD_DISPATCH16(p->dtype, launch_s32<T, 1, true>(p, st));
  else if (ctot == 32) rc = LD_DISPATCH16(p->dtype, launch_s32<T, 1, false>(p, st));
  else rc = LD_DISPATCH16(p->dtype, launch_s32<T, 2, false>(p, st));
  if (rc == LD_OK) ld_count(LD_COUNTER_CONV3X3_S32);
  return rc == LD_OK ? 1 : rc;
}
```

localdiffusion-hallucination_amd/tuning.py:

```python
import os
from dataclasses import dataclass, field, fields, replace
from typing import Dict, Mapping, Optional, Tuple

_PROCESS_ENV = os.environ


@dataclass
class Tuning:
    sub_batches: int = 2
    min_sub_batch: int = 2
    sub_resync: int = 32
    sub_resync_early: int = 1
    sub_ahead: int = 2
    sub_joint_graph: bool = False
    fused_final_step: bool = True
    fused_step_begin: bool = True
    weight_split_levels: int = 0
    separate_act: bool = True
    sep_act_max_px: int = 32 * 32
    sep_act_min_c: int = 128
    fusion_fold: bool = True
    side_res_conv: bool = True
    side_res_conv_max_px: int = 64 * 64
    side_res_conv_px: Optional[Tuple[int, ...]] = None
    linattn_chunk_px: Optional[Tuple[int, int, int]] = None
    graph_prewarm: bool = True
    pool_by_size: bool = True
    recompute_stem: bool = False
    buffer_reuse: bool = True
    pool_verify: bool = False
    kernel: Dict[str, int] = field(default_factory=dict)

    _ENV = {
        "LD_SUB_BATCHES": ("sub_batches", int), "LD_MIN_SUB_BATCH": ("min_sub_batch", int),
        "LD_SUB_RESYNC": ("sub_resync", int), "LD_SUB_RESYNC_EARLY": ("sub_resync_early", int),
        "LD_SUB_AHEAD": ("sub_ahead", int), "LD_SUB_JOINT_GRAPH": ("sub_joint_graph", lambda v: v not in ("0", "")), "LD_WEIGHT_SPLIT_LEVELS": ("weight_split_levels", int),
        "LD_SEP_ACT_MAX_PX": ("sep_act_max_px", int), "LD_SEP_ACT_MIN_C": ("sep_act_min_c", int),
        "LD_NO_FUSED_FINAL": ("fused_final_step", lambda v: False), "LD_NO_FUSED_BEGIN": ("fused_step_begin", lambda v: False),
        "LD_NO_SEPARATE_ACT": ("separate_act", lambda v: False),
        "LD_NO_FUSION_FOLD": ("fusion_fold", lambda v: False),
        "LD_NO_SIDE_RES_CONV": ("side_res_conv", lambda v: False), "LD_SIDE_RES_CONV_MAX_PX": ("side_res_conv_max_px", int),
        "LD_SIDE_RES_CONV_PX": ("side_res_conv_px", lambda v: tuple(int(x) for x in v.split(","))),
        "LD_NO_GRAPH_PREWARM": ("graph_prewarm", lambda v: False),
        "LD_POOL_BY_START": ("pool_by_size", lambda v: False),
        "LD_RECOMPUTE_STEM": ("recompute_stem", lambda v: v not in ("0", "")),
        "LD_BUFFER_REUSE": ("buffer_reuse", lambda v: v not in ("0", "")), "LD_NO_BUFFER_REUSE": ("buffer_reuse", lambda v: False),
        "LD_POOL_VERIFY": ("pool_verify", lambda v: v not in ("0", "")),
        "LD_LINATTN_CHUNK_PX": ("linattn_chunk_px", lambda v: tuple(int(x) for x in (v.split(",") * 3)[:3])),
    }

    @classmethod
    def from_env(cls, env: Optional[Mapping[str, str]] = None, **overrides) -> "Tuning":
        env = _PROCESS_ENV if env is None else env
        t = cls()
        for var, (name, parse) in cls._ENV.items():
            if env.get(var) not in (None, ""):
                setattr(t, name, parse(env[var]))
        return replace(t, **overrides) if overrides else t

    def chunk_rule(self, batch: int) -> Tuple[int, int, int]:
        if self.linattn_chunk_px is not None:
            return tuple(self.linattn_chunk_px)
        return (512, 256, 128) if batch <= 8 else (1024, 256, 128)

    def apply_kernel_table(self, lib) -> None:
        from . import _cabi as cabi
        for name, value in self.kernel.items():
            cabi.check(lib.ld_tuning_set(name.encode(), int(value)), f"tuning {name}")

    def describe(self) -> dict:
        return {f.name: getattr(self, f.name) for f in fields(self) if not f.name.startswith("_")}


def kernel_table(lib) -> Dict[str, int]:
    import ctypes as C
    out = {}
    for i in range(lib.ld_tuning_count()):
        name = lib.ld_tuning_name(i)
        v = C.c_longlong()
        lib.ld_tuning_get(name, C.byref(v))
        out[name.decode()] = int(v.value)
    return out


def lib_override_path() -> Optional[str]:
    return _PROCESS_ENV.get("LD_LIB_OVERRIDE") or None


def runtime_env_default(var: str, value: str) -> bool:
    if var in _PROCESS_ENV:
        return False
    _PROCESS_ENV[var] = value
    return True


def rendezvous_run_id() -> Optional[str]:
    return _PROCESS_ENV.get("TORCHELASTIC_RUN_ID") or _PROCESS_ENV.get("MASTER_PORT")


RUNTIME_CONFIGURED = False


def runtime_configured(var: str = "DEBUG_CLR_GRAPH_PACKET_CAPTURE") -> bool:
    return RUNTIME_CONFIGURED or var in _PROCESS_ENV
```

localdiffusion-hallucination_amd/unet.py:

```python
import ctypes as C
import math

import numpy as np
import torch
from torch import nn

from . import _cabi as cabi
from .pool import check_declared, intervals_from_declared, peak_live, place_intervals
from .tuning import Tuning
from .weights import UnetConfig, unet_param_shapes

_TORCH_DT = {"fp32": torch.float32, "bf16": torch.bfloat16, "fp16": torch.float16}
_LOWP = ("bf16", "fp16")


def _register(root: nn.Module, dotted: str, tensor: torch.Tensor):
    parts = dotted.split(".")
    mod = root
    for name in parts[:-1]:
        if name not in mod._modules:
            mod.add_module(name, nn.Module())
        mod = mod._modules[name]
    mod.register_parameter(parts[-1], nn.Parameter(tensor, requires_grad=False))


class Unet(nn.Module):
    def __init__(self, dim, init_dim=None, out_dim=None, dim_mults=(1, 2, 4, 8), channels=1,
                 self_condition=False, cond_img=True, resnet_block_groups=8, learned_variance=False,
                 learned_sinusoidal_cond=False, random_fourier_features=False,
                 learned_sinusoidal_dim=16, sinusoidal_pos_emb_theta=10000, attn_dim_head=32,
                 attn_heads=4, full_attn=(False, False, False, True), flash_attn=False, mode="mri",
                 compute_dtype="fp32", tuning=None):
        super().__init__()
        if (learned_sinusoidal_cond or random_fourier_features) and (learned_sinusoidal_dim % 2 or not 2 <= learned_sinusoidal_dim <= 256):
            raise ValueError("learned_sinusoidal_dim must be even (ddpm.py:156) and at most 256")
        if dim != 32:
            raise ValueError("dim must be 32: the conditioning encoder hard-codes its widths "
                             "(unet_model.py:100) and is concatenated with the 8*dim bottleneck")
        if attn_dim_head != 32:
            raise ValueError("attn_dim_head must be 32 (MFMA tile of the attention kernels)")
        if compute_dtype not in _TORCH_DT:
            raise ValueError(f"compute_dtype {compute_dtype!r} (fp32 | bf16 | fp16)")
        full_attn = tuple(full_attn) if isinstance(full_attn, (tuple, list)) else (full_attn,) * len(dim_mults)
        assert len(full_attn) == len(dim_mults)
        init_dim = dim if init_dim is None else init_dim
        learned = bool(learned_sinusoidal_cond or random_fourier_features)
        default_out = channels * (2 if learned_variance else 1)
        self.cfg = UnetConfig(dim=dim, init_dim=init_dim, out_dim=default_out if out_dim is None else out_dim,
                              dim_mults=tuple(dim_mults), channels=channels,
                              resnet_block_groups=resnet_block_groups, attn_dim_head=attn_dim_head,
                              attn_heads=attn_heads, full_attn=full_attn, mode=mode,
                              learned_sinusoidal_dim=int(learned_sinusoidal_dim) if learned else 0)
        self.mode = mode
        self.channels = channels
        self.out_dim = self.cfg.out_dim
        self.self_condition = bool(self_condition)
        self.cond_img = cond_img
        self.random_or_learned_sinusoidal_cond = learned
        self.theta = sinusoidal_pos_emb_theta
        self.compute_dtype = compute_dtype
        g = torch.Generator().manual_seed(0)
        shapes = unet_param_shapes(self.cfg)
        for name, shape in shapes.items():
            if name.endswith(".g"):
                t = torch.ones(shape)
            elif name.endswith(".weights"):
                t = torch.randn(shape, generator=g)
            elif len(shape) == 1 and (".norm." in name or "convblock.1" in name or "convblock.4" in name
                                      or "identity.1" in name):
                t = torch.ones(shape) if name.endswith("weight") else torch.zeros(shape)
            else:
                wshape = shape if name.endswith("weight") else shapes[name[:-4] + "weight"]
                bound = 1.0 / math.sqrt(int(np.prod(wshape[1:])))
                t = (torch.rand(shape, generator=g) * 2 - 1) * bound
            _register(self, name, t)
        self._packed = None
        self._packed_key = None
        self._plans = {}
        self.tuning = tuning if tuning is not None else Tuning.from_env()
        self.weight_split_levels = int(self.tuning.weight_split_levels)
        self._version = 0

    @property
    def downsample_factor(self):
        return self.cfg.downsample_factor

    @property
    def device(self):
        return next(self.parameters()).device

    def set_compute_dtype(self, name):
        if name not in _TORCH_DT:
            raise ValueError(name)
        if name != self.compute_dtype:
            self.compute_dtype = name
            self.invalidate()

    def set_weight_split_levels(self, n):
        if int(n) != self.weight_split_levels:
            self.weight_split_levels = int(n)
            self.invalidate()

    def _layer_level(self, name):
        n = len(self.cfg.dim_mults)
        if name.startswith("downs."):
            return int(name.split(".")[1])
        if name.startswith("ups."):
            return n - 1 - int(name.split(".")[1])
        if name.startswith("final_res_block"):
            return 0
        return n - 1

    def invalidate(self):
        self._packed, self._packed_key, self._plans = None, None, {}
        self._version = getattr(self, "_version", 0) + 1

    def load_state_dict(self, *a, **k):
        out = super().load_state_dict(*a, **k)
        self.invalidate()
        return out

    def _apply(self, fn, *a, **k):
        out = super()._apply(fn, *a, **k)
        self.invalidate()
        return out

    def packed(self):
        dev = self.device
        if dev.type != "cuda":
            raise RuntimeError("the HIP denoiser needs its parameters on a GPU (model.to('cuda')); "
                               "there is no CPU execution path")
        key = (str(dev), self.compute_dtype, self.weight_split_levels)
        if self._packed is not None and self._packed_key == key:
            return self._packed
        lib = cabi.lib()
        self.tuning.apply_kernel_table(lib)
        st = torch.cuda.current_stream().cuda_stream
        dt, tdt = cabi.dtype_code(self.compute_dtype), _TORCH_DT[self.compute_dtype]
        sd = {k: v.detach().to(torch.float32).contiguous() for k, v in self.state_dict().items()}
        P = {"f32": sd, "w": {}, "g2": {}, "terms2": set()}

        def pack(name, ksize, scale_in=None, unshuffle=0):
            w = sd[name]
            cout, cin = w.shape[0], w.shape[1]
            terms = 2 if (self.compute_dtype in _LOWP and scale_in is None and not name.startswith("cond_model.")
                          and self._layer_level(name) < self.weight_split_levels) else 1
            out = torch.empty(terms * cout * cin * ksize * ksize, dtype=tdt, device=dev)
            cabi.check(lib.ld_pack_conv_weight_terms(w.data_ptr(), cabi.ptr(scale_in), out.data_ptr(), cout, cin,
                                                     ksize, unshuffle, dt, terms, st), "pack " + name)
            P["w"][name] = out
            if terms == 2:
                P["terms2"].add(out.data_ptr())
            if scale_in is not None:
                P.setdefault("keep", []).append(scale_in)

        for name, w in sd.items():
            if not name.endswith(".weight") or w.dim() != 4:
                continue
            k = w.shape[-1]
            base = name[:-len(".weight")]
            if k == 7 or w.shape[1] < 32:
                continue
            if base == "final_conv":
                continue
            if base.endswith(".to_qkv"):
                g = sd[base[:-len(".to_qkv")] + ".norm.g"].flatten()
                pack(name, 1, scale_in=(g * math.sqrt(g.numel())).contiguous())
            elif k == 1 and base.endswith(".3.1") and base.startswith("downs."):
                pack(name, 1, unshuffle=1)
            elif k == 1 and (base.endswith(".to_out.0")):
                continue
            else:
                pack(name, k)
        P["wq"], P["wkv"], P["kshift"], P["qshift"] = {}, {}, {}, {}
        if self.compute_dtype in _LOWP:
            hid, heads = self.cfg.hidden, self.cfg.attn_heads
            for name, w in sd.items():
                if not name.endswith(".to_qkv.weight") or (name[:-len(".to_qkv.weight")] + ".to_out.1.g") not in sd:
                    continue
                base = name[:-len(".to_qkv.weight")]
                g = sd[base + ".norm.g"].flatten()
                scale = (g * math.sqrt(g.numel())).contiguous()
                c = w.shape[1]
                if c not in (32, 64, 128):
                    continue

                terms = 2 if (c in (32, 64) and heads == 4 and self._layer_level(name) < self.weight_split_levels) else 1

                def pack_rows(rows, terms=terms):
                    out = torch.empty(terms * rows.numel(), dtype=tdt, device=dev)
                    rows = rows.contiguous()
                    cabi.check(lib.ld_pack_conv_weight_terms(rows.data_ptr(), scale.data_ptr(), out.data_ptr(), rows.shape[0],
                                                             c, 1, 0, dt, terms, st), "pack " + name)
                    P.setdefault("keep", []).append(rows)
                    return out
                P.setdefault("attn_terms", {})[base] = terms
                P["wq"][base] = pack_rows(w[:hid])
                per_head = []
                for h in range(heads):
                    kv = torch.cat([w[hid + 32 * h: hid + 32 * h + 32], w[2 * hid + 32 * h: 2 * hid + 32 * h + 32]], 0)
                    per_head.append(pack_rows(kv))
                P["wkv"][base] = torch.cat(per_head).contiguous()
                wk = (w[hid:2 * hid, :, 0, 0].float() * scale[None, :]).to(tdt).float()
                bound = wk.norm(dim=1) * 1.01
                kmax_ok = 40.0 if self.compute_dtype == "bf16" else 8.0
                P["kshift"][base] = bound.contiguous() if float(bound.max()) <= kmax_ok else None
                wqn = (w[:hid, :, 0, 0].float() * scale[None, :]).to(tdt).float().norm(dim=1) * 1.01
                qb = wqn.reshape(heads, 32).amax(dim=1)
                P["qshift"][base] = qb.contiguous() if float(qb.max()) <= 40.0 else None
                P["keep"].append(scale)
        if self.compute_dtype in _LOWP and "conv_fusion.res_conv.weight" in sd:
            for nm, k in (("conv_fusion.block1.proj.weight", 3), ("conv_fusion.res_conv.weight", 1)):
                wfull = sd[nm]
                half = wfull.shape[1] // 2
                for tag, part in (("#x", wfull[:, :half]), ("#c", wfull[:, half:])):
                    part = part.contiguous()
                    out = torch.empty(part.numel(), dtype=tdt, device=dev)
                    cabi.check(lib.ld_pack_conv_weight(part.data_ptr(), None, out.data_ptr(), part.shape[0], part.shape[1],
                                                       k, 0, dt, st), "pack " + nm + tag)
                    P["w"][nm + tag] = out
                    P.setdefault("keep", []).append(part)
        if self.compute_dtype in _LOWP and self.cfg.init_dim == 32:
            wi = sd["init_conv.weight"].contiguous()
            stem = torch.empty(int(lib.ld_stem_packed_bytes()), dtype=torch.uint8, device=dev)
            cabi.check(lib.ld_pack_stem_weight(wi.data_ptr(), stem.data_ptr(), wi.shape[1], st), "pack init_conv")
            P["stem"] = stem
            P.setdefault("keep", []).append(wi)
        for name, w in sd.items():
            if name.endswith(".to_out.1.g"):
                g = w.flatten()
                P["g2"][name] = (g * math.sqrt(g.numel())).contiguous()
        half = self.cfg.dim // 2
        step = math.log(self.theta) / (half - 1)
        P["freqs"] = torch.exp(torch.arange(half) * -step).to(dev)
        torch.cuda.current_stream().synchronize()
        self._packed, self._packed_key = P, key
        return P

    def plan(self, B, H, W, table_T=None, instance=0):
        f = self.downsample_factor
        assert H % f == 0 and W % f == 0, \
            f"your input dimensions {(H, W)} need to be divisible by {f}, given the unet"
        tn = self.tuning
        key = (B, H, W, table_T, self.compute_dtype, instance, self.weight_split_levels,
               tn.separate_act, tn.sep_act_max_px, tn.sep_act_min_c, tn.fusion_fold, tn.side_res_conv, tn.side_res_conv_max_px, tn.side_res_conv_px, tn.fused_step_begin, tn.linattn_chunk_px, tn.buffer_reuse, tn.recompute_stem, tn.pool_by_size, tn.pool_verify)
        if key not in self._plans:
            self._plans[key] = _Plan(self, B, H, W, table_T)
        return self._plans[key]

    @torch.no_grad()
    def forward(self, x, cond_img, time, x_self_cond=None):
        B, _, H, W = x.shape
        if self.self_condition:
            c = self.cfg.channels
            raise RuntimeError(f"Given groups=1, weight of size [{self.cfg.init_dim}, {c}, 7, 7], expected input[{B}, {2 * c}, {H}, {W}] to have "
                               f"{c} channels, but got {2 * c} channels instead (self_condition=True: ddpm.py:406-413)")
        p = self.plan(B, H, W)
        st = torch.cuda.current_stream().cuda_stream
        p.x_in.copy_(x.to(torch.float32))
        p.cond_in.copy_(cond_img.to(torch.float32))
        p.times.copy_(time.to(torch.int32))
        p.run_time(st)
        p.run_cond(st)
        p.run_main(st)
        return p.model_out.clone()


class _Plan:

    def __init__(self, net: Unet, B, H, W, table_T=None):
        self.net, self.B, self.H, self.W, self.table_T = net, B, H, W, table_T
        self.lib = cabi.lib()
        self.dev = net.device
        self.dt = cabi.dtype_code(net.compute_dtype)
        self.tdt = _TORCH_DT[net.compute_dtype]
        self.esize = 4 if self.dt == cabi.LD_F32 else 2
        self.P = net.packed()
        self.tn = net.tuning
        self.f32 = self.P["f32"]
        cfg = net.cfg
        self.cfg = cfg
        self.keep = []
        self._track = None
        self.named = {}
        self.meta = {}
        self.decl = {}
        self.live_out = []
        self.ops_time, self.ops_cond, self.ops_main = [], [], []
        self.nslot = 0
        self.stats = torch.zeros(160, B, cabi.STAT_STRIPES, 16, 2, dtype=torch.float64, device=self.dev)
        self.cond_slots = 16
        self.kmax_arena = torch.zeros(8, B, cabi.STAT_STRIPES, cfg.hidden, dtype=torch.int32, device=self.dev)
        self._kmax_cursor = 0
        self.x_in = torch.zeros(B, cfg.channels, H, W, dtype=torch.float32, device=self.dev)
        self.cond_in = torch.zeros(B, cfg.cond_in_channels, H, W, dtype=torch.float32, device=self.dev)
        self.model_out = torch.zeros(B, cfg.out_dim, H, W, dtype=torch.float32, device=self.dev)
        self.times = torch.zeros(B, dtype=torch.int32, device=self.dev)
        self.t_dev = torch.zeros(1, dtype=torch.int32, device=self.dev)
        self.rows = table_T if table_T else B
        self.temb = torch.zeros(self.rows, cfg.time_dim, dtype=torch.float32, device=self.dev)
        self.films = {}
        self._film_off, self.film_row = {}, 0
        self._build_time()
        self.film_rows = self.film_cur = None
        if table_T and self.film_row:
            self.film_rows = torch.zeros(table_T, self.film_row, dtype=torch.float32, device=self.dev)
            self.film_cur = torch.zeros(self.film_row, dtype=torch.float32, device=self.dev)
        self._slot_cursor = 0
        self.cond_feat = self._build_cond()
        self.named["cond_model"] = self.cond_feat
        self.fusion_const = None
        if "conv_fusion.block1.proj.weight#c" in self.P["w"] and not cfg.cond_early_exit and self.tn.fusion_fold:
            c = self.cond_feat.shape[-1]
            hh, ww = self.cond_feat.shape[1], self.cond_feat.shape[2]
            p1 = self.conv3(self.ops_cond, [self.src(self.cond_feat, c)], "conv_fusion.block1.proj", c, hh, ww,
                            weight=self.P["w"]["conv_fusion.block1.proj.weight#c"])
            p2 = self.conv1(self.ops_cond, [self.src(self.cond_feat, c)], self.P["w"]["conv_fusion.res_conv.weight#c"],
                            c, hh, ww, bias=self.f32["conv_fusion.res_conv.bias"], what="res_conv(cond) conv_fusion")
            self.fusion_const = (p1, p2, torch.zeros(c, dtype=torch.float32, device=self.dev))
        self._slot_cursor = self.cond_slots
        self._track = [] if (table_T and self.tn.buffer_reuse) else None
        self._build_main()
        if self._track is not None:
            self._pool_buffers()
            self._track = None
        self._slots_used = self._slot_cursor
        s_, km_ = self.stats[self.cond_slots:self._slots_used], self.kmax_arena[:self._kmax_cursor]
        self._begin_args = (s_.data_ptr(), s_.numel() * 8, km_.data_ptr() if km_.numel() else None, km_.numel() * 4)
        self._t_dev_ptr = self.t_dev.data_ptr()
        self._film_args = (None, 0, None)
        if table_T:
            st = torch.cuda.current_stream().cuda_stream
            for op in self.ops_time:
                op(st)
            if self.film_rows is not None:
                for film in self.films.values():
                    off = self._film_off[id(film)]
                    self.film_rows[:, off:off + film.shape[1]].copy_(film)
                self._film_args = (self.film_rows.data_ptr(), self.film_row, self.film_cur.data_ptr())
            torch.cuda.current_stream().synchronize()

    def _kt(self, name):
        v = C.c_longlong()
        cabi.check(self.lib.ld_tuning_get(name.encode(), C.byref(v)), "tuning_get")
        return int(v.value)

    def _separate_act(self, px, c):
        return self.tn.separate_act and px <= self.tn.sep_act_max_px and c >= self.tn.sep_act_min_c

    def buf(self, h, w, c):
        t = torch.empty(self.B, h, w, c, dtype=self.tdt, device=self.dev)
        if self._track is not None:
            self._track.append(t)
        return t

    def _tracked(self, t):
        if self._track is not None:
            self._track.append(t)
        return t

    def _pool_buffers(self):
        import bisect
        bufs = self._track or []
        if not bufs:
            return
        rng = [(t.data_ptr(), t.data_ptr() + t.numel() * t.element_size()) for t in bufs]
        order = sorted(range(len(bufs)), key=lambda k: rng[k][0])
        starts = [rng[k][0] for k in order]
        n_ops = len(self.ops_main)

        def owner(ptr):
            j = bisect.bisect_right(starts, ptr) - 1
            if j >= 0 and rng[order[j]][0] <= ptr < rng[order[j]][1]:
                return order[j]
            return None

        def scan_struct(obj, hit):
            if isinstance(obj, C.Array):
                for e in obj:
                    if isinstance(e, (C.Structure, C.Array)):
                        scan_struct(e, hit)
                return
            for name, typ in obj._fields_:
                v = getattr(obj, name)
                if isinstance(v, (C.Structure, C.Array)):
                    scan_struct(v, hit)
                elif typ is cabi.vp and v:
                    k = owner(v)
                    if k is not None:
                        hit(obj, name, k, v - rng[k][0])

        def tensors(v, depth=0):
            if isinstance(v, torch.Tensor):
                yield v
            elif isinstance(v, (tuple, list)) and depth < 3:
                for e in v:
                    yield from tensors(e, depth + 1)
            elif isinstance(v, dict) and depth < 3:
                for e in v.values():
                    yield from tensors(e, depth + 1)

        def held(op):
            for d in (getattr(op, "__defaults__", None) or ()):
                yield d
            for cell in (getattr(op, "__closure__", None) or ()):
                try:
                    yield cell.cell_contents
                except ValueError:
                    continue

        scanned, patches = [set() for _ in range(n_ops)], []
        for i, op in enumerate(self.ops_main):
            def hit(obj, name, k, delta, i=i):
                scanned[i].add(k)
                patches.append((obj, name, k, delta))
            for v in held(op):
                if hasattr(v, "_obj"):
                    scan_struct(v._obj, hit)
                for t in tensors(v):
                    k = owner(t.data_ptr()) if t.is_cuda else None
                    if k is not None:
                        scanned[i].add(k)
        def declared_set(ts):
            out = set()
            for t in ts:
                k = owner(t.data_ptr()) if (t is not None and t.is_cuda) else None
                if k is not None:
                    out.add(k)
            return out
        declared = [declared_set(self.decl.get(i, ((), ()))[0]) | declared_set(self.decl.get(i, ((), ()))[1]) for i in range(n_ops)]
        op_names = [self.meta.get(i, {}).get("what", "?") for i in range(n_ops)]
        buf_names = [f"#{k} {tuple(t.shape)}" for k, t in enumerate(bufs)]
        check_declared(declared, scanned, op_names, buf_names)
        live_out = declared_set(self.live_out)
        for name, v in self.__dict__.items():
            if name in ("_track", "keep", "named", "decl", "live_out"):
                continue
            for t in tensors(v):
                k = owner(t.data_ptr()) if t.is_cuda else None
                if k is not None and k not in live_out:
                    raise RuntimeError(f"pool: plan attribute {name!r} reaches pooled buffer {buf_names[k]} that is not in live_out")
        first, last = intervals_from_declared(declared, len(bufs), live_out)
        size = [(r[1] - r[0] + 255) // 256 * 256 for r in rng]
        offset, top = place_intervals(size, first, last, self.tn.pool_by_size)
        self._pool = torch.empty(top, dtype=torch.uint8, device=self.dev)
        base = self._pool.data_ptr()
        for obj, name, k, delta in patches:
            setattr(obj, name, base + offset[k] + delta)
        pooled = set()
        for k, t in enumerate(bufs):
            t.set_(self._pool.untyped_storage(), offset[k] // t.element_size(), t.size(), t.stride())
            assert t.data_ptr() == base + offset[k]
            if last[k] < n_ops:
                pooled.add(id(t))
        def stale(v):
            return isinstance(v, int) and not isinstance(v, bool) and owner(v) is not None
        cur = [0]

        def still(obj, name, k, delta):
            raise RuntimeError(f"pool: launch {cur[0]} ({op_names[cur[0]]}) field {name} still points into the old allocation of {buf_names[k]}")
        for i, op in enumerate(self.ops_main):
            cur[0] = i
            for v in held(op):
                if hasattr(v, "_obj"):
                    scan_struct(v._obj, still)
                vals = list(v) if isinstance(v, (tuple, list)) else (list(v.values()) if isinstance(v, dict) else [v])
                for e in vals:
                    if stale(e):
                        raise RuntimeError(f"pool: launch {i} ({op_names[i]}) holds the old address of {buf_names[owner(e)]} as a plain integer")
                for t in tensors(v):
                    if t.is_cuda and owner(t.data_ptr()) is not None:
                        raise RuntimeError(f"pool: launch {i} ({op_names[i]}) holds a tensor that was not re-pointed at the pool")
        self.named = {k: v for k, v in self.named.items() if id(v) not in pooled}
        peak = peak_live(size, first, last)
        self.pool_stats = dict(buffers=len(bufs), bytes_unshared=sum(size), bytes_pool=top, bytes_peak_live=peak)
        self.pool_intervals = [(first[k], last[k], offset[k], size[k]) for k in range(len(bufs))]
        if self.tn.pool_verify:
            dying = {}
            for k in range(len(bufs)):
                if 0 <= last[k] < n_ops:
                    dying.setdefault(last[k], []).append((base + offset[k], size[k]))
            lib = self.lib
            for i, regions in dying.items():
                def poisoned(st, op=self.ops_main[i], regions=tuple(regions)):
                    op(st)
                    for ptr, nbytes in regions:
                        cabi.check(lib.ld_memset_bytes(ptr, 0xFF, nbytes, st), "pool verify")
                self.ops_main[i] = poisoned
            self.pool_stats["verify_poisoned_buffers"] = sum(len(r) for r in dying.values())

    def slot(self):
        s = self._slot_cursor
        self._slot_cursor += 1
        assert s < self.stats.shape[0]
        return self.stats[s]

    def t_ptr(self):
        return None

    def src(self, t, c, stride=0, ups=0, gn=None, act=cabi.ACT_NONE, film=None):
        s = cabi.Src()
        s.data, s.C, s.pix_stride, s.upsample = t.data_ptr(), c, stride, ups
        if gn is not None:
            stats, gamma, beta, groups = gn
            s.gn_stats, s.gn_gamma, s.gn_beta, s.gn_groups = stats.data_ptr(), gamma.data_ptr(), beta.data_ptr(), groups
        s.act = act
        if film is not None and self.table_T:
            s.film = self.film_cur.data_ptr() + 4 * self._film_off[id(film)]
            s.film_tstride = s.film_bstride = 0
        elif film is not None:
            s.film = film.data_ptr()
            s.film_tstride = 0
            s.film_bstride = 2 * c
        self.keep.append(t)
        s._tensor = t
        return s

    def _call(self, ops, fn, args, what, meta=None, reads=(), writes=()):
        self.keep.append(args)
        ref = C.byref(args)
        ops.append(lambda st, fn=fn, ref=ref, what=what: cabi.check(fn(ref, st), what))
        if ops is self.ops_main:
            self.meta[len(ops) - 1] = dict(what=what, **(meta or {}))
            self.decl[len(ops) - 1] = ([t for t in reads if t is not None], [t for t in writes if t is not None])

    def _raw(self, ops, fn, what, nbytes=0, flops=0, reads=(), writes=()):
        ops.append(fn)
        if ops is self.ops_main:
            self.meta[len(ops) - 1] = dict(what=what, family=what, bytes=nbytes, flops=flops)
            self.decl[len(ops) - 1] = ([t for t in reads if t is not None], [t for t in writes if t is not None])

    def conv3(self, ops, srcs, wname, cout, h, w, stats=None, groups=8, weight=None, bias=None, addend=None, side=None):
        a = cabi.Conv3x3Args()
        for i, s in enumerate(srcs):
            a.src[i] = s
        a.nsrc = len(srcs)
        weight = self.P["w"][wname + ".weight"] if weight is None else weight
        bias = self.f32[wname + ".bias"] if bias is None else bias
        a.weight, a.bias = weight.data_ptr(), bias.data_ptr()
        a.weight_terms = 2 if weight.data_ptr() in self.P["terms2"] else 1
        a.addend = cabi.ptr(addend)
        self.keep += [weight, bias, addend]
        out = self.buf(h, w, cout)
        a.out = out.data_ptr()
        side_out = None
        if side is not None:
            side_out = self.buf(h, w, cout)
            a.side_weight, a.side_bias, a.side_out = side[0].data_ptr(), side[1].data_ptr(), side_out.data_ptr()
            self.keep += [side[0], side[1]]
        if stats is not None:
            a.out_stats, a.out_groups = stats.data_ptr(), groups
        a.B, a.H, a.W, a.Cout = self.B, h, w, cout
        a.t_ptr = self.t_ptr()
        a.dtype = self.dt
        cin = sum(s.C for s in srcs)
        npx = self.B * h * w
        mt4 = cout % 64 == 0 and ((w + 15) // 16) * ((h + 7) // 8) * (cout // 64) * self.B >= 256
        blocks16 = ((w + 15) // 16) * ((h + 15) // 16) * (cout // (64 if mt4 else 32)) * self.B
        big = blocks16 >= 512 and h >= 16 and not mt4
        big = big or (mt4 and h >= 16 and blocks16 >= self._kt("conv_big4_min"))
        dname = {cabi.LD_F32: "f32", cabi.LD_BF16: "bf16", cabi.LD_F16: "f16"}[self.dt]
        if side is not None:
            big = False
        fam = f"conv3x3<{dname},{4 if mt4 else 2},{4 if big else 2}>"
        ck = 16 if self.dt == cabi.LD_F32 else 32
        if side is not None:
            pass
        elif (cout == 32 and len(srcs) == 1 and cin == ck and addend is None and h >= 32 and w >= 32 and h % 16 == 0
                and w % 16 == 0 and (w // 16) * (h // 16) * self.B >= self._kt("conv_c32_min_tiles")
                and self._kt("conv_c32") and a.weight_terms != 2):
            fam = f"conv3x3_c32<{dname}>"
        elif (self.dt != cabi.LD_F32 and cout == 32 and addend is None and a.weight_terms != 2 and h % 16 == 0 and w % 16 == 0
              and (w // 16) * (h // 16) * self.B >= self._kt("conv_s32_min_tiles") and not any(s.upsample for s in srcs)
              and cin in (32, 64) and (len(srcs) == 1 or all(s.C == 32 for s in srcs)) and groups in (1, 2, 4, 8)):
            pro = any(s.gn_stats for s in srcs)
            bit = 2 if pro else (1 if cin == 32 else 4)
            if (self._kt("conv_s32") & bit) and (not pro or (len(srcs) == 1 and srcs[0].C == 32 and srcs[0].gn_groups == 8)):
                fam = f"conv3x3_s32<{dname}>"
        in_el = sum(s.C * (npx // 4 if s.upsample else npx) for s in srcs)
        side_b = (in_el + npx * cout + cin * cout) * self.esize + 4 * cout if side is not None else 0
        self._call(ops, self.lib.ld_conv3x3, a, "conv3x3 " + wname + (" + res_conv" if side is not None else ""),
                   dict(family=fam, bytes=(in_el + npx * cout + 9 * cin * cout) * self.esize + 4 * cout + side_b,
                        flops=2 * (9 + (1 if side is not None else 0)) * cin * cout * npx, shape=f"{cin}->{cout}@{h}x{w}"),
                   reads=[s._tensor for s in srcs] + [addend], writes=[out, side_out])
        return out if side is None else (out, side_out)

    def conv1(self, ops, srcs, weight, cout, h, w, bias=None, epi=cabi.EPI_PLAIN, unshuffle=0, rms_in=0,
              bstride=0, g2=None, residual=None, what="conv1x1", out=None, kmax_out=None, gn_tail=None):
        a = cabi.Conv1x1Args()
        for i, s in enumerate(srcs):
            a.src[i] = s
        a.nsrc, a.unshuffle, a.rms_in = len(srcs), unshuffle, rms_in
        a.weight, a.weight_bstride = weight.data_ptr(), bstride
        a.weight_terms = 2 if weight.data_ptr() in self.P["terms2"] else 1
        a.bias = cabi.ptr(bias)
        a.epilogue, a.hidden, a.q_scale = epi, self.cfg.hidden, self.cfg.attn_dim_head ** -0.5
        a.g2, a.residual = cabi.ptr(g2), cabi.ptr(residual)
        a.kmax_out = cabi.ptr(kmax_out)
        if gn_tail is not None:
            a.gn_tail = gn_tail
        out = self.buf(h, w, cout) if out is None else out
        a.out = out.data_ptr()
        a.B, a.H, a.W, a.Cout, a.dtype = self.B, h, w, cout, self.dt
        self.keep += [weight, bias, g2, residual]
        cin = sum(s.C for s in srcs) * (4 if unshuffle else 1)
        npx = self.B * h * w
        el = npx * cin + npx * cout + cin * cout * (self.B if bstride else 1) + (npx * cout if (residual is not None or gn_tail is not None) else 0)
        self._call(ops, self.lib.ld_conv1x1, a, what,
                   dict(family="conv1x1", bytes=el * self.esize, flops=2 * cin * cout * npx, shape=f"{cin}->{cout}@{h}x{w}"),
                   reads=[s._tensor for s in srcs] + [residual, gn_tail._tensor if gn_tail is not None else None], writes=[out])
        return out

    def gn_apply(self, ops, a_src, b_src, h, w, c, final_act=cabi.ACT_NONE, pool=0):
        g = cabi.GnApplyArgs()
        g.a = a_src
        if b_src is not None:
            g.b = b_src
        g.final_act, g.pool = final_act, pool
        out = self.buf(h // 2 if pool else h, w // 2 if pool else w, c)
        g.out = out.data_ptr()
        g.B, g.H, g.W, g.t_ptr, g.dtype = self.B, h, w, self.t_ptr(), self.dt
        nel = self.B * h * w * c
        self._call(ops, self.lib.ld_gn_apply, g, "gn_apply",
                   dict(family="gn_apply", bytes=(nel * (2 if b_src is not None else 1) + nel // (4 if pool else 1)) * self.esize, flops=0),
                   reads=[a_src._tensor, b_src._tensor if b_src is not None else None], writes=[out])
        return out

    def _build_time(self):
        cfg, f, lib = self.cfg, self.f32, self.lib
        if self.table_T:
            times = torch.arange(self.table_T, dtype=torch.int32, device=self.dev)
        else:
            times = self.times
        self.keep.append(times)
        freqs = self.P["freqs"]
        n, td = self.rows, cfg.time_dim
        if cfg.learned_sinusoidal_dim:
            wts = f["time_mlp.0.weights"]
            self.ops_time.append(lambda st: cabi.check(lib.ld_time_mlp_fourier(
                times.data_ptr(), n, wts.data_ptr(), cfg.learned_sinusoidal_dim, f["time_mlp.1.weight"].data_ptr(),
                f["time_mlp.1.bias"].data_ptr(), f["time_mlp.3.weight"].data_ptr(), f["time_mlp.3.bias"].data_ptr(),
                td, self.temb.data_ptr(), st), "time_mlp (learned Fourier features)"))
        else:
            self.ops_time.append(lambda st: cabi.check(lib.ld_time_mlp(
                times.data_ptr(), n, freqs.data_ptr(), cfg.dim, f["time_mlp.1.weight"].data_ptr(),
                f["time_mlp.1.bias"].data_ptr(), f["time_mlp.3.weight"].data_ptr(), f["time_mlp.3.bias"].data_ptr(),
                td, self.temb.data_ptr(), st), "time_mlp"))
        for name in f:
            if name.endswith(".mlp.1.weight") and not name.startswith("conv_fusion"):
                p = name[:-len(".mlp.1.weight")]
                two_c = f[name].shape[0]
                film = torch.zeros(n, two_c, dtype=torch.float32, device=self.dev)
                self.films[p] = film
                self._film_off[id(film)] = self.film_row
                self.film_row += two_c
                w, b = f[name], f[p + ".mlp.1.bias"]
                self.ops_time.append(lambda st, w=w, b=b, film=film, two_c=two_c: cabi.check(lib.ld_film(
                    self.temb.data_ptr(), n, td, w.data_ptr(), b.data_ptr(), two_c, film.data_ptr(), st), "film"))

    def resnet_block(self, ops, p, srcs_fn, cin_total, cout, h, w, res_tensor=None):
        f, G = self.f32, self.cfg.resnet_block_groups
        s1, s2 = self.slot(), self.slot()
        wres = self.P["w"].get(p + ".res_conv.weight")
        side = None
        px_ok = (h * w in self.tn.side_res_conv_px) if self.tn.side_res_conv_px is not None else h * w <= self.tn.side_res_conv_max_px
        if (wres is not None and self.tn.side_res_conv and self.dt != cabi.LD_F32 and px_ok and self.net.weight_split_levels == 0
                and wres.data_ptr() not in self.P["terms2"] and self.P["w"][p + ".block1.proj.weight"].data_ptr() not in self.P["terms2"]):
            side = (wres, f[p + ".res_conv.bias"])
        rc = None
        if side is not None:
            raw1, rc = self.conv3(ops, srcs_fn(), p + ".block1.proj", cout, h, w, stats=s1, groups=G, side=side)
        else:
            raw1 = self.conv3(ops, srcs_fn(), p + ".block1.proj", cout, h, w, stats=s1, groups=G)
        film = self.films.get(p)
        n1 = self.src(raw1, cout, gn=(s1, f[p + ".block1.norm.weight"], f[p + ".block1.norm.bias"], G),
                      act=cabi.ACT_SILU, film=film)
        if self._separate_act(h * w, cout):
            act1 = self.gn_apply(ops, n1, None, h, w, cout)
            n1 = self.src(act1, cout)
        raw2 = self.conv3(ops, [n1], p + ".block2.proj", cout, h, w, stats=s2, groups=G)
        n2 = self.src(raw2, cout, gn=(s2, f[p + ".block2.norm.weight"], f[p + ".block2.norm.bias"], G),
                      act=cabi.ACT_SILU)
        if rc is not None:
            out = self.gn_apply(ops, n2, self.src(rc, cout), h, w, cout)
        elif (p + ".res_conv.weight") in f:
            out = self.conv1(ops, srcs_fn(), self.P["w"][p + ".res_conv.weight"], cout, h, w,
                             bias=f[p + ".res_conv.bias"], epi=cabi.EPI_GN_TAIL, gn_tail=n2, what="res_conv+tail " + p)
        else:
            assert res_tensor is not None and cin_total == cout
            out = self.gn_apply(ops, n2, self.src(res_tensor, cout), h, w, cout)
        self.named[p] = out
        return out

    def fusion_block_folded(self, ops, x, c, h, w):
        f, G, p = self.f32, self.cfg.resnet_block_groups, "conv_fusion"
        p1, p2, zero = self.fusion_const
        s1, s2 = self.slot(), self.slot()
        raw1 = self.conv3(ops, [self.src(x, c)], p + ".block1.proj", c, h, w, stats=s1, groups=G,
                          weight=self.P["w"][p + ".block1.proj.weight#x"], bias=zero, addend=p1)
        n1 = self.src(raw1, c, gn=(s1, f[p + ".block1.norm.weight"], f[p + ".block1.norm.bias"], G),
                      act=cabi.ACT_SILU, film=self.films.get(p))
        if self._separate_act(h * w, c):
            n1 = self.src(self.gn_apply(ops, n1, None, h, w, c), c)
        raw2 = self.conv3(ops, [n1], p + ".block2.proj", c, h, w, stats=s2, groups=G)
        n2 = self.src(raw2, c, gn=(s2, f[p + ".block2.norm.weight"], f[p + ".block2.norm.bias"], G), act=cabi.ACT_SILU)
        out = self.conv1(ops, [self.src(x, c)], self.P["w"][p + ".res_conv.weight#x"], c, h, w, bias=None,
                         epi=cabi.EPI_GN_TAIL, gn_tail=n2, residual=p2, what="res_conv+tail " + p)
        self.named[p] = out
        return out

    def linear_attention_fused(self, ops, p, x, c, h, w):
        f, cfg, lib = self.f32, self.cfg, self.lib
        n, hid, B, heads, dt, es = h * w, cfg.hidden, self.B, cfg.attn_heads, self.dt, self.esize
        rule = self.tn.chunk_rule(B)
        chunk_px = rule[0] if n >= 65536 else (rule[1] if n >= 16384 else rule[2])
        nchunks = max(1, min(128, n // chunk_px)) if heads == 4 else max(1, min(32, n // 256))
        if heads == 4 and self.tn.linattn_chunk_px is None:
            while B * nchunks < 512 and nchunks < 512 and n // (2 * nchunks) >= 256:
                nchunks *= 2
        ctx = self._tracked(torch.empty(int(lib.ld_linattn_ctx_part_floats(B, heads, 32, nchunks)), dtype=torch.float32, device=self.dev))
        wfold = self._tracked(torch.empty(B, c * hid, dtype=self.tdt, device=self.dev))
        wout = f[p + ".to_out.0.weight"].reshape(c, hid).contiguous()
        wq, wkv = self.P["wq"][p], self.P["wkv"][p]
        kshift = self.P["kshift"].get(p) if heads == 4 else None
        ksp = kshift.data_ptr() if kshift is not None else None
        qshift = self.P["qshift"].get(p) if heads == 4 else None
        qsp = qshift.data_ptr() if qshift is not None else None
        bias, g2 = f[p + ".to_out.0.bias"], self.P["g2"][p + ".to_out.1.g"]
        out = self.buf(h, w, c)
        self.keep += [ctx, wfold, wout, wq, wkv, kshift, qshift, bias, g2, out, x]
        npx = B * n
        terms = self.P.get("attn_terms", {}).get(p, 1)
        self._raw(ops, lambda st: cabi.check(lib.ld_linattn_kvctx_terms(x.data_ptr(), wkv.data_ptr(), ksp, ctx.data_ptr(), B, n, c,
                                                                        heads, 32, nchunks, dt, terms, st), "linattn_kvctx"),
                  "linattn_kvctx", nbytes=npx * c * es, flops=2 * npx * c * 2 * hid * (1 if kshift is not None else 2) + 2 * npx * hid * 32,
                  reads=[x], writes=[ctx])
        self._raw(ops, lambda st: cabi.check(lib.ld_linattn_ctxfold(ctx.data_ptr(), nchunks, wout.data_ptr(), wfold.data_ptr(), B, c,
                                                                    heads, 32, 1, dt, st), "linattn_ctxfold"),
                  "linattn_ctxfold", nbytes=B * c * hid * es, flops=2 * B * c * hid * 32, reads=[ctx], writes=[wfold])
        scale = cfg.attn_dim_head ** -0.5
        self._raw(ops, lambda st: cabi.check(lib.ld_linattn_out_terms(x.data_ptr(), wq.data_ptr(), qsp, wfold.data_ptr(), bias.data_ptr(),
                                                                      g2.data_ptr(), out.data_ptr(), B, n, c, scale, dt, terms, st),
                                             "linattn_out"),
                  "linattn_out", nbytes=2 * npx * c * es, flops=2 * npx * hid * c * 2, reads=[x, wfold], writes=[out])
        return out

    def linear_attention(self, ops, p, x, c, h, w):
        if self.dt != cabi.LD_F32 and c in (32, 64, 128) and p in self.P["wq"]:
            return self.linear_attention_fused(ops, p, x, c, h, w)
        f, cfg, lib = self.f32, self.cfg, self.lib
        n, hid, B = h * w, cfg.hidden, self.B
        kmax = self.kmax_arena[self._kmax_cursor]
        self._kmax_cursor += 1
        qkv = self.conv1(ops, [self.src(x, c)], self.P["w"][p + ".to_qkv.weight"], 3 * hid, h, w,
                         epi=cabi.EPI_QKV_LINEAR, rms_in=1, what="to_qkv " + p, kmax_out=kmax)
        nchunks = max(1, min(32, n // 256))
        ctx = torch.empty(int(lib.ld_linattn_ctx_part_floats(B, cfg.attn_heads, 32, nchunks)),
                          dtype=torch.float32, device=self.dev)
        wfold = torch.empty(B, c * hid, dtype=self.tdt, device=self.dev)
        wout = f[p + ".to_out.0.weight"].reshape(c, hid).contiguous()
        self.keep += [kmax, ctx, wfold, wout, qkv]
        dt, heads = self.dt, cfg.attn_heads
        es = self.esize
        self._raw(ops, lambda st: cabi.check(lib.ld_linattn_ctx(qkv.data_ptr(), kmax.data_ptr(), ctx.data_ptr(),
                                                                B, n, heads, 32, nchunks, dt, st), "linattn_ctx"),
                  "linattn_ctx", nbytes=2 * B * n * hid * es, flops=2 * B * n * hid * 32, reads=[qkv], writes=[ctx])
        self._raw(ops, lambda st: cabi.check(lib.ld_linattn_ctxfold(ctx.data_ptr(), nchunks, wout.data_ptr(), wfold.data_ptr(),
                                                                    B, c, heads, 32, 0, dt, st), "linattn_ctxfold"),
                  "linattn_ctxfold", nbytes=B * c * hid * es, flops=2 * B * c * hid * 32, reads=[ctx], writes=[wfold])
        q = self.src(qkv, hid, stride=3 * hid)
        return self.conv1(ops, [q], wfold, c, h, w, bias=f[p + ".to_out.0.bias"], epi=cabi.EPI_RMS_RES,
                          bstride=c * hid * self.esize, g2=self.P["g2"][p + ".to_out.1.g"], residual=x,
                          what="lin to_out " + p)

    def full_attention(self, ops, p, x, c, h, w):
        f, cfg, lib = self.f32, self.cfg, self.lib
        n, hid, B = h * w, cfg.hidden, self.B
        qkv = self.conv1(ops, [self.src(x, c)], self.P["w"][p + ".to_qkv.weight"], 3 * hid, h, w,
                         epi=cabi.EPI_QKV_FULL, rms_in=1, what="to_qkv " + p)
        att = self.buf(h, w, hid)
        dt, heads = self.dt, cfg.attn_heads
        self.keep += [qkv, att]
        self._raw(ops, lambda st: cabi.check(lib.ld_attention(qkv.data_ptr(), att.data_ptr(), B, n, heads, 32, dt, st),
                                             "attention"),
                  "attention", nbytes=4 * B * n * hid * self.esize, flops=4 * B * n * n * hid, reads=[qkv], writes=[att])
        return self.conv1(ops, [self.src(att, hid)], self.P["w"][p + ".to_out.weight"], c, h, w,
                          bias=f[p + ".to_out.bias"], epi=cabi.EPI_RES, residual=x, what="full to_out " + p)

    def attention(self, ops, p, x, c, h, w, full):
        out = (self.full_attention if full else self.linear_attention)(ops, p, x, c, h, w)
        self.named[p] = out
        return out

    def _basic_block(self, ops, p, x, cin, cmid, cout, h, w, pool, image=False):
        f, lib, G = self.f32, self.lib, 16
        s1, s2, s3 = self.slot(), self.slot(), self.slot()

        def image_conv(wname, c_out, stats):
            out = self.buf(h, w, c_out)
            wt, bs = f[wname + ".weight"], f[wname + ".bias"]
            B, dt = self.B, self.dt
            self.keep += [out, wt, bs]
            ops.append(lambda st: cabi.check(lib.ld_conv_image(
                self.cond_in.data_ptr(), wt.data_ptr(), bs.data_ptr(), out.data_ptr(), stats.data_ptr(), G,
                B, cin, h, w, 3, dt, st), "conv_image " + wname))
            return out

        if image:
            a1 = image_conv(p + ".convblock.0", cmid, s1)
            idr = image_conv(p + ".identity.0", cout, s3)
        else:
            a1 = self.conv3(ops, [self.src(x, cin)], p + ".convblock.0", cmid, h, w, stats=s1, groups=G)
            idr = self.conv3(ops, [self.src(x, cin)], p + ".identity.0", cout, h, w, stats=s3, groups=G)
        n1 = self.src(a1, cmid, gn=(s1, f[p + ".convblock.1.weight"], f[p + ".convblock.1.bias"], G),
                      act=cabi.ACT_RELU)
        a2 = self.conv3(ops, [n1], p + ".convblock.3", cout, h, w, stats=s2, groups=G)
        na = self.src(a2, cout, gn=(s2, f[p + ".convblock.4.weight"], f[p + ".convblock.4.bias"], G))
        nb = self.src(idr, cout, gn=(s3, f[p + ".identity.1.weight"], f[p + ".identity.1.bias"], G))
        return self.gn_apply(ops, na, nb, h, w, cout, final_act=cabi.ACT_RELU, pool=1 if pool else 0)

    def _build_cond(self):
        cfg, ops, H, W = self.cfg, self.ops_cond, self.H, self.W
        x = self._basic_block(ops, "cond_model.residual_conv1.0", None, cfg.cond_in_channels, 32, 32, H, W,
                              pool=True, image=True)
        x = self._basic_block(ops, "cond_model.residual_conv2.0", x, 32, 32, 64, H // 2, W // 2, pool=True)
        early = cfg.cond_early_exit
        x = self._basic_block(ops, "cond_model.residual_conv3.0", x, 64, 64, 128, H // 4, W // 4, pool=not early)
        if early:
            return x
        return self._basic_block(ops, "cond_model.mid_conv.0", x, 128, 128, 256, H // 8, W // 8, pool=False)

    def _build_main(self):
        cfg, ops, f, lib, B = self.cfg, self.ops_main, self.f32, self.lib, self.B
        H, W = self.H, self.W
        r = self.buf(H, W, cfg.init_dim)
        wi, bi = f["init_conv.weight"], f["init_conv.bias"]
        if self.dt != cabi.LD_F32 and cfg.init_dim == 32:
            wstem = self.P["stem"]
            self.keep.append(wstem)

            def stem_begin(st, delta, idx_ptr, t_table):
                za, ba, zb, bb = self._begin_args
                rows, row_floats, cur = self._film_args
                g = cabi.StepBeginArgs(za, ba, zb, bb, self._t_dev_ptr, int(delta), idx_ptr, t_table, rows, row_floats, cur)
                cabi.check(lib.ld_conv_stem_begin(self.x_in.data_ptr(), wstem.data_ptr(), bi.data_ptr(), r.data_ptr(), B, cfg.channels,
                                                  H, W, self.dt, C.byref(g), st), "init_conv + step_begin")
            self._stem_begin = stem_begin
            self._raw(ops, lambda st: cabi.check(lib.ld_conv_stem(
                self.x_in.data_ptr(), wstem.data_ptr(), bi.data_ptr(), r.data_ptr(), B, cfg.channels, H, W, self.dt, st),
                "init_conv"), "conv_image7x7",
                nbytes=B * H * W * (4 * cfg.channels + self.esize * cfg.init_dim), flops=2 * 49 * cfg.channels * cfg.init_dim * B * H * W, writes=[r])
        else:
            self._raw(ops, lambda st: cabi.check(lib.ld_conv_image(
                self.x_in.data_ptr(), wi.data_ptr(), bi.data_ptr(), r.data_ptr(), None, 1, B, cfg.channels, H, W, 7,
                self.dt, st), "init_conv"), "conv_image7x7",
                nbytes=B * H * W * (4 * cfg.channels + self.esize * cfg.init_dim), flops=2 * 49 * cfg.channels * cfg.init_dim * B * H * W, writes=[r])
        self.named["init_conv"] = r
        x, c, h, w = r, cfg.init_dim, H, W
        skips = []
        io, n = cfg.in_out, len(cfg.in_out)
        for i, (cin, cout) in enumerate(io):
            p = f"downs.{i}"
            x = self.resnet_block(ops, p + ".0", lambda x=x, c=c: [self.src(x, c)], c, c, h, w, res_tensor=x)
            skips.append((x, c))
            x = self.resnet_block(ops, p + ".1", lambda x=x, c=c: [self.src(x, c)], c, c, h, w, res_tensor=x)
            x = self.attention(ops, p + ".2", x, c, h, w, cfg.full_attn[i])
            skips.append((x, c))
            if i < n - 1:
                h, w = h // 2, w // 2
                x = self.conv1(ops, [self.src(x, c)], self.P["w"][p + ".3.1.weight"], cout, h, w,
                               bias=f[p + ".3.1.bias"], unshuffle=1, what="downsample " + p)
            else:
                x = self.conv3(ops, [self.src(x, c)], p + ".3", cout, h, w)
            self.named[p + ".3"] = x
            c = cout
        x = self.resnet_block(ops, "mid_block1", lambda x=x, c=c: [self.src(x, c)], c, c, h, w, res_tensor=x)
        x = self.attention(ops, "mid_attn", x, c, h, w, True)
        x = self.resnet_block(ops, "mid_block2", lambda x=x, c=c: [self.src(x, c)], c, c, h, w, res_tensor=x)
        feat = self.cond_feat
        if self.fusion_const is not None:
            x = self.fusion_block_folded(ops, x, c, h, w)
        else:
            x = self.resnet_block(ops, "conv_fusion", lambda x=x, c=c: [self.src(x, c), self.src(feat, c)], 2 * c, c, h, w)
        for j, ((cin, cout), full) in enumerate(zip(reversed(io), reversed(cfg.full_attn))):
            p = f"ups.{j}"
            for k in (0, 1):
                sk, sc = skips.pop()
                x = self.resnet_block(ops, f"{p}.{k}", lambda x=x, c=c, sk=sk, sc=sc: [self.src(x, c), self.src(sk, sc)],
                                      c + sc, cout, h, w)
                c = cout
            x = self.attention(ops, p + ".2", x, c, h, w, full)
            if j < n - 1:
                h, w = h * 2, w * 2
                x = self.conv3(ops, [self.src(x, c, ups=1)], p + ".3.1", cin, h, w)
            else:
                x = self.conv3(ops, [self.src(x, c)], p + ".3", cin, h, w)
            self.named[p + ".3"] = x
            c = cin
        if self.tn.recompute_stem and self._track is not None and self.dt != cabi.LD_F32 and cfg.init_dim == 32:
            r2 = self.buf(H, W, cfg.init_dim)
            wstem2 = self.P["stem"]
            self._raw(ops, lambda st, r2=r2: cabi.check(lib.ld_conv_stem(
                self.x_in.data_ptr(), wstem2.data_ptr(), bi.data_ptr(), r2.data_ptr(), B, cfg.channels, H, W, self.dt, st),
                "init_conv (again)"), "conv_image7x7",
                nbytes=B * H * W * (4 * cfg.channels + self.esize * cfg.init_dim), flops=2 * 49 * cfg.channels * cfg.init_dim * B * H * W, writes=[r2])
            r_cat = r2
        else:
            r_cat = r
        x = self.resnet_block(ops, "final_res_block", lambda x=x, c=c, r_cat=r_cat: [self.src(x, c), self.src(r_cat, cfg.init_dim)],
                              c + cfg.init_dim, cfg.dim, h, w)
        wf = f["final_conv.weight"].reshape(cfg.out_dim, cfg.dim).contiguous()
        bf = f["final_conv.bias"]
        self.keep += [wf, bf, x, r]
        self.final = (x, wf, bf)
        self.live_out.append(x)
        self._raw(ops, lambda st, x=x: cabi.check(lib.ld_final_conv(
            x.data_ptr(), wf.data_ptr(), bf.data_ptr(), self.model_out.data_ptr(), B, H, W, cfg.dim, cfg.out_dim,
            self.dt, st), "final_conv"), "final_conv",
            nbytes=B * H * W * (self.esize * cfg.dim + 4 * cfg.out_dim), flops=2 * cfg.dim * cfg.out_dim * B * H * W, reads=[x])

    def __del__(self):
        try:
            if getattr(self, "_cond_graph", None) is not None:
                self.lib.ld_graph_destroy(self._cond_graph)
        except Exception:
            pass

    def run_time(self, st):
        for op in self.ops_time:
            op(st)

    def run_cond(self, st):
        self.cond_version = getattr(self, "cond_version", 0) + 1
        s = self.stats[:self.cond_slots]
        self.lib.ld_range_push(b"encoder")
        try:
            cabi.check(self.lib.ld_memset_zero(s.data_ptr(), s.numel() * 8, st), "memset")
            for op in self.ops_cond:
                op(st)
        finally:
            self.lib.ld_range_pop()

    def run_cond_replayed(self, stream):
        st = stream.cuda_stream
        g = getattr(self, "_cond_graph", None)
        if g is None:
            self.run_cond(st)
            stream.synchronize()
            s = self.stats[:self.cond_slots]
            cabi.check(self.lib.ld_graph_begin(st), "graph_begin")
            try:
                cabi.check(self.lib.ld_memset_zero(s.data_ptr(), s.numel() * 8, st), "memset")
                for op in self.ops_cond:
                    op(st)
            finally:
                g = C.c_void_p()
                rc = self.lib.ld_graph_end(st, C.byref(g))
            cabi.check(rc, "graph_end")
            self._cond_graph = g
            if self.tn.graph_prewarm:
                cabi.check(self.lib.ld_graph_launch(g, st), "graph_launch")
            return
        self.cond_version = getattr(self, "cond_version", 0) + 1
        self.lib.ld_range_push(b"encoder (graph replay)")
        try:
            cabi.check(self.lib.ld_graph_launch(g, st), "graph_launch")
        finally:
            self.lib.ld_range_pop()

    def run_main(self, st, skip_final=False, step_delta=0, idx_ptr=None, t_table=None):
        self.lib.ld_range_push(b"step")
        try:
            ops = self.ops_main[:-1] if skip_final else self.ops_main
            stem_begin = getattr(self, "_stem_begin", None) if self.tn.fused_step_begin else None
            if stem_begin is not None:
                stem_begin(st, 0 if idx_ptr is not None else int(step_delta), idx_ptr, t_table)
                ops = ops[1:]
            elif idx_ptr is not None:
                cabi.check(self.lib.ld_step_begin_film(*self._begin_args, self._t_dev_ptr, 0, idx_ptr, t_table, *self._film_args, st),
                           "step_begin")
            else:
                cabi.check(self.lib.ld_step_begin_film(*self._begin_args, self._t_dev_ptr, int(step_delta), None, None,
                                                       *self._film_args, st), "step_begin")
            for op in ops:
                op(st)
        finally:
            self.lib.ld_range_pop()

    def run_main_timed(self, st, acc):
        lib = self.lib
        cabi.check(lib.ld_step_begin_film(*self._begin_args, self._t_dev_ptr, 0, None, None, *self._film_args, st), "step_begin")
        cabi.check(lib.ld_timing_begin(8 * len(self.ops_main)), "timing_begin")
        marks = [0]
        try:
            for op in self.ops_main:
                op(st)
                marks.append(lib.ld_timing_count())
        finally:
            n = max(1, lib.ld_timing_count())
            ms, cnt = (C.c_float * n)(), C.c_int()
            rc = lib.ld_timing_end(ms, n, C.byref(cnt))
        cabi.check(rc, "timing_end")
        for i in range(len(self.ops_main)):
            a = acc.setdefault(i, [0.0, 0])
            a[0] += sum(ms[marks[i]:marks[i + 1]])
            a[1] += 1

    def set_step(self, t):
        self.t_dev.fill_(int(t))
```

Before: 6.485 patches/s.

## Fuse GroupNorm prologue into block2 conv3x3 via per-chunk register coefficients

For the small, wide ResNet block2 convolutions that previously used a separate GroupNorm+SiLU apply kernel, the conv3x3 kernel now computes GroupNorm/FiLM coefficients in registers per channel chunk. It loads group stats and gamma/beta alongside each chunk's data. This removes an extra kernel launch and a full activation round trip through memory, and drops the LDS coefficient table. The cost is more registers and redundant per-chunk stat loads, and this path forces the non-big, non-split-K tile configuration.

Result: slower. 6.213 patches/s (-4.2%).

```diff
diff --git a/include/localdiff_hip.h b/include/localdiff_hip.h
--- a/include/localdiff_hip.h
+++ b/include/localdiff_hip.h
@@ -84,6 +84,7 @@
   const void* side_weight;
   const float* side_bias;
   void* side_out;
+  int32_t gn_regs;
 } ld_conv3x3_args;
 int ld_conv3x3(const ld_conv3x3_args* args, void* stream);
 
diff --git a/localdiffusion-hallucination_amd/_cabi.py b/localdiffusion-hallucination_amd/_cabi.py
--- a/localdiffusion-hallucination_amd/_cabi.py
+++ b/localdiffusion-hallucination_amd/_cabi.py
@@ -30,7 +30,7 @@
     _fields_ = [("src", Src * 2), ("nsrc", i32), ("weight", vp), ("bias", vp), ("out", vp),
                 ("out_stats", vp), ("out_groups", i32), ("B", i32), ("H", i32), ("W", i32),
                 ("Cout", i32), ("t_ptr", vp), ("dtype", i32), ("addend", vp), ("weight_terms", i32),
-                ("side_weight", vp), ("side_bias", vp), ("side_out", vp)]
+                ("side_weight", vp), ("side_bias", vp), ("side_out", vp), ("gn_regs", i32)]
 
 
 class Conv1x1Args(C.Structure):
diff --git a/localdiffusion-hallucination_amd/csrc/conv3x3.hip b/localdiffusion-hallucination_amd/csrc/conv3x3.hip
--- a/localdiffusion-hallucination_amd/csrc/conv3x3.hip
+++ b/localdiffusion-hallucination_amd/csrc/conv3x3.hip
@@ -16,25 +16,29 @@
 int g_span_shape[1024][5];
 #endif
 
-template <typename T, int MT, int NW, bool DEEP, int DBG, bool SK = false, bool RAW = false, bool SIDE = false>
+template <typename T, int MT, int NW, bool DEEP, int DBG, bool SK = false, bool RAW = false, bool SIDE = false, bool GNR = false>
 int launch_dbg(const Conv3Dev& a, hipStream_t st) {
   constexpr int TR = 4 * NW, HR = TR + 2, HC = 18;
   constexpr int NPIXP = (HR * HC + 15) / 16 * 16;
   const int ctot = a.s[0].C + (a.nsrc > 1 ? a.s[1].C : 0);
-  const size_t lds = (SK ? 2 : 1) * (4 * NPIXP * 16 + (9 + (SIDE ? 1 : 0)) * MT * 1024) + 2 * ctot * sizeof(float) + 4 * 2 * 16 * MT * sizeof(double);
+  const size_t lds = (SK ? 2 : 1) * (4 * NPIXP * 16 + (9 + (SIDE ? 1 : 0)) * MT * 1024) + (GNR ? 0 : 2 * ctot * sizeof(float)) + 4 * 2 * 16 * MT * sizeof(double);
   Conv3Dev d = a;
   d.tiles_x = (a.W + 15) / 16;
   const int tiles_y = (a.H + TR - 1) / TR;
   dim3 grid(d.tiles_x * tiles_y, a.Cout / (16 * MT), a.B);
-  if (lds > 65536) LD_HIP(ld_allow_lds(conv3x3_kernel<T, MT, NW, DEEP, DBG, SK, RAW, SIDE>, lds));
-  LD_LAUNCH((conv3x3_kernel<T, MT, NW, DEEP, DBG, SK, RAW, SIDE>), grid, dim3(SK ? 512 : 256), lds, st, d.s[0].data, d.w, d.H, d.W, d.tiles_x,
+  if (lds > 65536) LD_HIP(ld_allow_lds(conv3x3_kernel<T, MT, NW, DEEP, DBG, SK, RAW, SIDE, GNR>, lds));
+  LD_LAUNCH((conv3x3_kernel<T, MT, NW, DEEP, DBG, SK, RAW, SIDE, GNR>), grid, dim3(SK ? 512 : 256), lds, st, d.s[0].data, d.w, d.H, d.W, d.tiles_x,
             d.s[0].C, d.s[0].ld, d.s[0].ups, d.nsrc, d.wsplit, d.Cout, d);
   LD_LAUNCH_CHECK("conv3x3");
   return LD_OK;
 }
 
 template <typename T, int MT, int NW, bool DEEP>
-int launch(const Conv3Dev& a, hipStream_t st) {
+int launch(const Conv3Dev& a, hipStream_t st, bool gnr) {
+  if constexpr (!DEEP && sizeof(T) == 2 && NW == 2) {
+    if (gnr) return launch_dbg<T, MT, NW, DEEP, 0, false, false, false, true>(a, st);
+  }
+  (void)gnr;
 #ifdef LD_DEBUG_VARIANTS
   if constexpr (std::is_same<T, bf16>::value && !DEEP) {
     switch (a.dbg & 255) {
@@ -62,7 +66,7 @@
 }
 
 template <typename T>
-int dispatch(const Conv3Dev& a, hipStream_t st) {
+int dispatch(const Conv3Dev& a, hipStream_t st, bool gnr) {
 #ifdef LD_DEBUG_VARIANTS
   static const int force_mt = getenv("LD_CONV_MT") ? atoi(getenv("LD_CONV_MT")) : 0;
   static const int force_nw = getenv("LD_CONV_NW") ? atoi(getenv("LD_CONV_NW")) : 0;
@@ -77,6 +81,7 @@
   const long big_min = tn.conv_big_min;
   bool big = blocks16 >= big_min && a.H >= 16 && !mt4;
   if (mt4 && a.H >= 16 && blocks16 >= tn.conv_big4_min) big = true;
+  if (gnr) big = false;
   if (force_mt == 2) mt4 = false;
   if (force_mt == 4 && (a.Cout % 64) == 0) mt4 = true;
   if (force_nw == 2) big = false;
@@ -99,16 +104,16 @@
   }
   const int force_sk = (int)tn.conv_sk;
   const long sk_max_wgs = tn.conv_sk_max_wgs;
-  bool sk = force_sk >= 1 && sizeof(T) == 2 && !big && !deep && ((nch >= 8 && wg <= sk_max_wgs) || force_sk == 2);
+  bool sk = force_sk >= 1 && sizeof(T) == 2 && !big && !deep && !gnr && ((nch >= 8 && wg <= sk_max_wgs) || force_sk == 2);
   if constexpr (sizeof(T) == 2) {
     if (sk) return mt4 ? launch_dbg<T, 4, 2, false, 0, true>(a, st) : launch_dbg<T, 2, 2, false, 0, true>(a, st);
   }
 #ifdef LD_DEBUG_VARIANTS
-  if (deep && !big) return mt4 ? launch<T, 4, 2, true>(a, st) : launch<T, 2, 2, true>(a, st);
+  if (deep && !big && !gnr) return mt4 ? launch<T, 4, 2, true>(a, st, false) : launch<T, 2, 2, true>(a, st, false);
 #endif
   (void)deep;
-  if (mt4) return big ? launch<T, 4, 4, false>(a, st) : launch<T, 4, 2, false>(a, st);
-  return big ? launch<T, 2, 4, false>(a, st) : launch<T, 2, 2, false>(a, st);
+  if (mt4) return big ? launch<T, 4, 4, false>(a, st, gnr) : launch<T, 4, 2, false>(a, st, gnr);
+  return big ? launch<T, 2, 4, false>(a, st, gnr) : launch<T, 2, 2, false>(a, st, gnr);
 }
 
 }
@@ -169,6 +174,13 @@
   LD_REQUIRE(p->weight_terms >= 0 && p->weight_terms <= 2 && !(p->weight_terms == 2 && !ld_dtype_16(p->dtype)),
              "ld_conv3x3: weight_terms %d (2 needs 16-bit storage)", p->weight_terms);
   a.wsplit = p->weight_terms == 2 ? 1 : 0;
+  const bool gnr = p->gn_regs != 0;
+  if (gnr) {
+    const ld_src& S = p->src[0];
+    LD_REQUIRE(ld_dtype_16(p->dtype) && p->weight_terms != 2, "ld_conv3x3: gn_regs needs 16-bit storage and one-term weights");
+    LD_REQUIRE(p->nsrc == 1 && S.gn_stats && !S.upsample && !p->side_weight, "ld_conv3x3: gn_regs needs ONE un-resampled source with a GroupNorm prologue and no side output");
+    LD_REQUIRE((S.C / S.gn_groups) % 8 == 0, "ld_conv3x3: gn_regs needs groups of a multiple of 8 channels (C %d, groups %d)", S.C, S.gn_groups);
+  }
   a.dbg = 0;
 #ifdef LD_DEBUG_VARIANTS
   static const int dbg = getenv("LD_CONV_DEBUG") ? atoi(getenv("LD_CONV_DEBUG")) : 0;
@@ -184,7 +196,11 @@
   hipStream_t st = reinterpret_cast<hipStream_t>(stream);
   if (p->side_weight) {
     ld_count(LD_COUNTER_CONV3X3_GENERIC);
-    return LD_DISPATCH16(p->dtype, dispatch<T>(a, st));
+    return LD_DISPATCH16(p->dtype, dispatch<T>(a, st, false));
+  }
+  if (gnr) {
+    ld_count(LD_COUNTER_CONV3X3_GENERIC);
+    return LD_DISPATCH16(p->dtype, dispatch<T>(a, st, true));
   }
   if (p->weight_terms != 2) {
     const int rc = ld_conv3x3_c32_try(p, st);
@@ -206,5 +222,5 @@
   }
 #endif
   ld_count(LD_COUNTER_CONV3X3_GENERIC);
-  return LD_DISPATCH(p->dtype, dispatch<T>(a, st));
-}
+  return LD_DISPATCH(p->dtype, dispatch<T>(a, st, false));
+}
diff --git a/localdiffusion-hallucination_amd/csrc/conv3x3_body.hip.h b/localdiffusion-hallucination_amd/csrc/conv3x3_body.hip.h
--- a/localdiffusion-hallucination_amd/csrc/conv3x3_body.hip.h
+++ b/localdiffusion-hallucination_amd/csrc/conv3x3_body.hip.h
@@ -1,5 +1,6 @@
 #pragma once
 #include "common.hip.h"
+#include "gn_coef_regs.hip.h"
 
 namespace {
 
@@ -27,7 +28,7 @@
 #define TR_STAMP(k) do { if ((DBG & 64) && tracing) tr_t[k] = __builtin_readcyclecounter(); } while (0)
 
 typedef const Conv3Dev __attribute__((address_space(4)))* Conv3KernargPtr;
-template <typename T, int MT, int NW, bool DEEP, int DBG, bool SK = false, bool RAW = false, bool SIDE = false>
+template <typename T, int MT, int NW, bool DEEP, int DBG, bool SK = false, bool RAW = false, bool SIDE = false, bool GNR = false>
 __device__ __forceinline__ void conv3x3_tile(const Conv3Dev& head, Conv3KernargPtr rest, const int bx, const int by, const int bz,
                                              const int gdx, const int gdz, char* smem) {
   Conv3Dev a = head;
@@ -39,6 +40,7 @@
   constexpr bool P = DT<T>::precise;
 
   static_assert(!SIDE || (RAW && !SK && !DEEP && MT * NW < 16 && sizeof(T) == 2), "SIDE: RAW 16-bit launches of the small register tiles");
+  static_assert(!GNR || (!RAW && !SK && !DEEP && !SIDE && sizeof(T) == 2), "GNR: the plain chunk loop, 16-bit storage");
   constexpr int STAGE = 4 * PLANE + (9 + (SIDE ? 1 : 0)) * MT * 1024;
   const int half = SK ? (int)(threadIdx.x >> 8) : 0;
   char* s_x = smem + half * STAGE;
@@ -68,6 +70,20 @@
 
   uint4 hxA[ITER], wxA[WU], hxB[DEEP ? ITER : 1], wxB[DEEP ? WU : 1];
   uint4 wx2 = make_uint4(0u, 0u, 0u, 0u);
+  constexpr int SPL = LD_STAT_STRIPES / 16;
+  f64x2 gn_st[GNR ? SPL : 1];
+  GnOctet gn_ops;
+  const float* gn_fp = nullptr;
+  int gn_fh = 0, gn_gs = 8;
+  double gn_inv_n = 0.0;
+  auto issue_coef = [&](int ch) {
+    const int c = ch * CK + kq * E;
+    const unsigned g = (unsigned)c / (unsigned)gn_gs;
+    const double* sp = a.s[0].stats + (((size_t)b * LD_STAT_STRIPES + px) * a.s[0].groups + g) * 2;
+#pragma unroll
+    for (int k = 0; k < SPL; ++k) gn_st[k] = *reinterpret_cast<const f64x2*>(sp + (size_t)k * 16 * a.s[0].groups * 2);
+    gn_octet_request(a.s[0].gamma, a.s[0].beta, gn_fp, gn_fh, c, gn_ops);
+  };
   unsigned hvalid = 0;
   unsigned hoffb0[ITER], hoffb1[ITER];
   const char* sbase0;
@@ -113,7 +129,8 @@
   auto issue_loads = [&](int ch, uint4 (&hx)[ITER], uint4 (&wx)[WU], auto first_tag) {
     constexpr bool FIRST = decltype(first_tag)::value;
     const int cs = ch >> ws;
-    const int si = FIRST ? 0 : (cs >= nch0 ? 1 : 0);
+    const int si = (FIRST || GNR) ? 0 : (cs >= nch0 ? 1 : 0);
+    if constexpr (GNR && !FIRST) issue_coef(ch);
     const char* sp = (si ? sbase1 : sbase0) + (long)(cs - si * nch0) * CK * (long)sizeof(T);
     const bool same_halo = !SK && !DEEP && ws && (ch & 1);
     const char* wc = reinterpret_cast<const char*>(wg) + (long)ch * wstride;
@@ -138,13 +155,22 @@
   };
   auto write_lds = [&](int ch, const uint4 (&hx)[ITER], const uint4 (&wx)[WU]) {
     const int csrc = ch >> ws;
-    const int si = csrc >= nch0 ? 1 : 0;
+    const int si = GNR ? 0 : (csrc >= nch0 ? 1 : 0);
     const SrcDev S = si ? a.s[1] : a.s[0];
     const int c0 = (csrc - si * nch0) * CK;
     const int coef_off = si ? 2 * a.s[0].C : 0;
-    const bool has_coef = !RAW && S.stats != nullptr;
+    const bool has_coef = GNR || (!RAW && S.stats != nullptr);
     float ca[E], cs[E];
-    if (has_coef) {
+    if constexpr (GNR) {
+      double s1 = gn_st[0][0], s2 = gn_st[0][1];
+#pragma unroll
+      for (int k = 1; k < SPL; ++k) { s1 += gn_st[k][0]; s2 += gn_st[k][1]; }
+      s1 = row_group_sum_d(s1, 16);
+      s2 = row_group_sum_d(s2, 16);
+      float mean, rstd;
+      gn_group_mean_rstd(s1, s2, gn_inv_n, mean, rstd);
+      if constexpr (E == 8) gn_octet_coef(gn_ops, mean, rstd, mean, rstd, a.s[0].film != nullptr, ca, cs);
+    } else if (has_coef) {
       const float* cap = s_coef + coef_off + c0 + kq * E;
 #pragma unroll
       for (int e = 0; e < E; ++e) { ca[e] = cap[e]; cs[e] = cap[S.C + e]; }
@@ -196,7 +222,17 @@
   {
     const int c1 = a.nsrc > 1 ? a.s[1].C : 0;
     nch = (nch0 + c1 / CK) << ws;
-    s_stat = reinterpret_cast<double*>(s_coef + 2 * (a.s[0].C + c1));
+    s_stat = reinterpret_cast<double*>(s_coef + (GNR ? 0 : 2 * (a.s[0].C + c1)));
+  }
+  if constexpr (GNR) {
+    const SrcDev& S = a.s[0];
+    const int trow = a.t_ptr ? *a.t_ptr : 0;
+    const float* film = S.film ? S.film + (long)trow * S.film_tstride + (long)b * S.film_bstride : nullptr;
+    gn_fp = film ? film : S.gamma;
+    gn_fh = film ? S.C : 0;
+    gn_gs = S.C / S.groups;
+    gn_inv_n = gn_inv_n16((long)H * W, gn_gs);
+    issue_coef(0);
   }
   asm volatile("" ::"s"(a.bias), "s"(a.out), "s"(a.ostats), "s"(a.ogroups), "s"(a.addend), "s"(a.s[1].C), "s"(a.s[1].ld), "s"(a.s[1].ups),
                "s"(a.s[1].data), "s"(a.s[0].stats), "s"(a.s[0].gamma), "s"(a.s[0].beta), "s"(a.s[0].film), "s"(a.s[0].groups), "s"(a.s[0].act));
@@ -212,7 +248,7 @@
   }
 
   {
-    const bool any = !RAW && (a.s[0].stats != nullptr || (a.nsrc > 1 && a.s[1].stats != nullptr));
+    const bool any = !RAW && !GNR && (a.s[0].stats != nullptr || (a.nsrc > 1 && a.s[1].stats != nullptr));
     if (any) {
       const int trow = a.t_ptr ? *a.t_ptr : 0;
       int off = 0;
@@ -558,7 +594,7 @@
   }
 }
 
-template <typename T, int MT, int NW, bool DEEP, int DBG, bool SK = false, bool RAW = false, bool SIDE = false>
+template <typename T, int MT, int NW, bool DEEP, int DBG, bool SK = false, bool RAW = false, bool SIDE = false, bool GNR = false>
 __global__ __launch_bounds__(SK ? 512 : 256) __attribute__((amdgpu_waves_per_eu(SK ? 2 : (MT == 2 ? 3 : 1), SK ? 2 : (MT == 2 ? 3 : 2))))
 void conv3x3_kernel(const void* data0, const void* w, int H, int W, int tiles_x, int C0, int ld0, int ups0, int nsrc, int wsplit, int Cout,
                     Conv3Dev rest) {
@@ -575,7 +611,7 @@
     a.tiles_x = tiles_x;
     conv3x3_tile<T, MT, NW, DEEP, DBG, SK, RAW>(a, nullptr, blockIdx.x, blockIdx.y, blockIdx.z, gridDim.x, gridDim.z, smem);
   } else {
-    conv3x3_tile<T, MT, NW, DEEP, DBG, SK, RAW, SIDE>(a, pr, blockIdx.x, blockIdx.y, blockIdx.z, gridDim.x, gridDim.z, smem);
+    conv3x3_tile<T, MT, NW, DEEP, DBG, SK, RAW, SIDE, GNR>(a, pr, blockIdx.x, blockIdx.y, blockIdx.z, gridDim.x, gridDim.z, smem);
   }
 }
 
diff --git a/localdiffusion-hallucination_amd/csrc/conv3x3_s32.hip b/localdiffusion-hallucination_amd/csrc/conv3x3_s32.hip
--- a/localdiffusion-hallucination_amd/csrc/conv3x3_s32.hip
+++ b/localdiffusion-hallucination_amd/csrc/conv3x3_s32.hip
@@ -1,4 +1,5 @@
 #include "common.hip.h"
+#include "gn_coef_regs.hip.h"
 
 namespace {
 
@@ -82,13 +83,9 @@
   float ca[PRO ? E : 1], cs[PRO ? E : 1];
   if constexpr (PRO) {
     const float* fp = a.film ? a.film + (long)b * a.film_bstride : a.gamma;
-    const int c = kq * E;
-    const f32x4 g0 = *reinterpret_cast<const f32x4*>(a.gamma + c), g1 = *reinterpret_cast<const f32x4*>(a.gamma + c + 4);
-    const f32x4 b0 = *reinterpret_cast<const f32x4*>(a.beta + c), b1 = *reinterpret_cast<const f32x4*>(a.beta + c + 4);
-    const f32x4 fs0 = *reinterpret_cast<const f32x4*>(fp + c), fs1 = *reinterpret_cast<const f32x4*>(fp + c + 4);
-    const f32x4 fh0 = *reinterpret_cast<const f32x4*>(fp + (a.film ? 32 : 0) + c), fh1 = *reinterpret_cast<const f32x4*>(fp + (a.film ? 32 : 0) + c + 4);
+    GnOctet ops;
+    gn_octet_request(a.gamma, a.beta, fp, a.film ? 32 : 0, kq * E, ops);
     constexpr int SPL = LD_STAT_STRIPES / 16;
-    typedef __attribute__((ext_vector_type(2))) double f64x2;
     f64x2 q0[SPL], q1[SPL];
 #pragma unroll
     for (int k = 0; k < SPL; ++k) {
@@ -103,31 +100,10 @@
     double s1[2] = {row_group_sum_d(t0[0], 16), row_group_sum_d(t1[0], 16)};
     double s2[2] = {row_group_sum_d(t0[1], 16), row_group_sum_d(t1[1], 16)};
     float mean[2], rstd[2];
-    const double inv_n = (double)__builtin_amdgcn_rcpf((float)((long)H * W) * 4.0f);
-#pragma unroll
-    for (int g = 0; g < 2; ++g) {
-      const double m = s1[g] * inv_n;
-      double var = s2[g] * inv_n - m * m;
-      var = var > 0.0 ? var : 0.0;
-      mean[g] = (float)m;
-      rstd[g] = __builtin_amdgcn_rsqf((float)(var + 1e-5));
-    }
-    const float gam[E] = {g0[0], g0[1], g0[2], g0[3], g1[0], g1[1], g1[2], g1[3]};
-    const float bet[E] = {b0[0], b0[1], b0[2], b0[3], b1[0], b1[1], b1[2], b1[3]};
-    const float fsc[E] = {fs0[0], fs0[1], fs0[2], fs0[3], fs1[0], fs1[1], fs1[2], fs1[3]};
-    const float fsh[E] = {fh0[0], fh0[1], fh0[2], fh0[3], fh1[0], fh1[1], fh1[2], fh1[3]};
-#pragma unroll
-    for (int e = 0; e < E; ++e) {
-      float aa = rstd[e >> 2] * gam[e];
-      float ss = bet[e] - mean[e >> 2] * aa;
-      if (a.film) {
-        const float sc = fsc[e] + 1.0f;
-        aa *= sc;
-        ss = ss * sc + fsh[e];
-      }
-      ca[e] = aa;
-      cs[e] = ss;
-    }
+    const double inv_n = gn_inv_n16((long)H * W, 4);
+#pragma unroll
+    for (int g = 0; g < 2; ++g) gn_group_mean_rstd(s1[g], s2[g], inv_n, mean[g], rstd[g]);
+    gn_octet_coef(ops, mean[0], rstd[0], mean[1], rstd[1], a.film != nullptr, ca, cs);
   }
   f32x4 bias[MT];
   f32x4 acc[MT][NW];
diff --git a/localdiffusion-hallucination_amd/csrc/gn_coef_regs.hip.h b/localdiffusion-hallucination_amd/csrc/gn_coef_regs.hip.h
--- /dev/null
+++ b/localdiffusion-hallucination_amd/csrc/gn_coef_regs.hip.h
@@ -0,0 +1,42 @@
+#pragma once
+#include "common.hip.h"
+
+typedef __attribute__((ext_vector_type(2))) double f64x2;
+
+__device__ __forceinline__ double gn_inv_n16(long npix, int gs) {
+  return (double)__builtin_amdgcn_rcpf((float)npix * (float)gs);
+}
+
+__device__ __forceinline__ void gn_group_mean_rstd(double s1, double s2, double inv_n, float& mean, float& rstd) {
+  const double m = s1 * inv_n;
+  double var = s2 * inv_n - m * m;
+  var = var > 0.0 ? var : 0.0;
+  mean = (float)m;
+  rstd = __builtin_amdgcn_rsqf((float)(var + 1e-5));
+}
+
+struct GnOctet {
+  f32x4 g[2], b[2], fs[2], fh[2];
+};
+__device__ __forceinline__ void gn_octet_request(const float* gamma, const float* beta, const float* fp, int fh_off, int c, GnOctet& o) {
+  o.g[0] = *reinterpret_cast<const f32x4*>(gamma + c); o.g[1] = *reinterpret_cast<const f32x4*>(gamma + c + 4);
+  o.b[0] = *reinterpret_cast<const f32x4*>(beta + c); o.b[1] = *reinterpret_cast<const f32x4*>(beta + c + 4);
+  o.fs[0] = *reinterpret_cast<const f32x4*>(fp + c); o.fs[1] = *reinterpret_cast<const f32x4*>(fp + c + 4);
+  o.fh[0] = *reinterpret_cast<const f32x4*>(fp + fh_off + c); o.fh[1] = *reinterpret_cast<const f32x4*>(fp + fh_off + c + 4);
+}
+__device__ __forceinline__ void gn_octet_coef(const GnOctet& o, float mean0, float rstd0, float mean1, float rstd1, bool film,
+                                              float (&ca)[8], float (&cs)[8]) {
+#pragma unroll
+  for (int e = 0; e < 8; ++e) {
+    const float mean = e < 4 ? mean0 : mean1, rstd = e < 4 ? rstd0 : rstd1;
+    float aa = rstd * o.g[e >> 2][e & 3];
+    float ss = o.b[e >> 2][e & 3] - mean * aa;
+    if (film) {
+      const float sc = o.fs[e >> 2][e & 3] + 1.0f;
+      aa *= sc;
+      ss = ss * sc + o.fh[e >> 2][e & 3];
+    }
+    ca[e] = aa;
+    cs[e] = ss;
+  }
+}
diff --git a/localdiffusion-hallucination_amd/tuning.py b/localdiffusion-hallucination_amd/tuning.py
--- a/localdiffusion-hallucination_amd/tuning.py
+++ b/localdiffusion-hallucination_amd/tuning.py
@@ -19,6 +19,7 @@
     separate_act: bool = True
     sep_act_max_px: int = 32 * 32
     sep_act_min_c: int = 128
+    conv_gn_regs: bool = field(default=True, metadata={"describe": False})
     fusion_fold: bool = True
     side_res_conv: bool = True
     side_res_conv_max_px: int = 64 * 64
@@ -38,6 +39,7 @@
         "LD_SEP_ACT_MAX_PX": ("sep_act_max_px", int), "LD_SEP_ACT_MIN_C": ("sep_act_min_c", int),
         "LD_NO_FUSED_FINAL": ("fused_final_step", lambda v: False), "LD_NO_FUSED_BEGIN": ("fused_step_begin", lambda v: False),
         "LD_NO_SEPARATE_ACT": ("separate_act", lambda v: False),
+        "LD_NO_CONV_GN_REGS": ("conv_gn_regs", lambda v: False),
         "LD_NO_FUSION_FOLD": ("fusion_fold", lambda v: False),
         "LD_NO_SIDE_RES_CONV": ("side_res_conv", lambda v: False), "LD_SIDE_RES_CONV_MAX_PX": ("side_res_conv_max_px", int),
         "LD_SIDE_RES_CONV_PX": ("side_res_conv_px", lambda v: tuple(int(x) for x in v.split(","))),
@@ -68,8 +70,9 @@
         for name, value in self.kernel.items():
             cabi.check(lib.ld_tuning_set(name.encode(), int(value)), f"tuning {name}")
 
-    def describe(self) -> dict:
-        return {f.name: getattr(self, f.name) for f in fields(self) if not f.name.startswith("_")}
+    def describe(self, every_field: bool = False) -> dict:
+        return {f.name: getattr(self, f.name) for f in fields(self)
+                if not f.name.startswith("_") and (every_field or f.metadata.get("describe", True))}
 
 
 def kernel_table(lib) -> Dict[str, int]:
diff --git a/localdiffusion-hallucination_amd/unet.py b/localdiffusion-hallucination_amd/unet.py
--- a/localdiffusion-hallucination_amd/unet.py
+++ b/localdiffusion-hallucination_amd/unet.py
@@ -243,7 +243,7 @@
             f"your input dimensions {(H, W)} need to be divisible by {f}, given the unet"
         tn = self.tuning
         key = (B, H, W, table_T, self.compute_dtype, instance, self.weight_split_levels,
-               tn.separate_act, tn.sep_act_max_px, tn.sep_act_min_c, tn.fusion_fold, tn.side_res_conv, tn.side_res_conv_max_px, tn.side_res_conv_px, tn.fused_step_begin, tn.linattn_chunk_px, tn.buffer_reuse, tn.recompute_stem, tn.pool_by_size, tn.pool_verify)
+               tn.separate_act, tn.sep_act_max_px, tn.sep_act_min_c, tn.conv_gn_regs, tn.fusion_fold, tn.side_res_conv, tn.side_res_conv_max_px, tn.side_res_conv_px, tn.fused_step_begin, tn.linattn_chunk_px, tn.buffer_reuse, tn.recompute_stem, tn.pool_by_size, tn.pool_verify)
         if key not in self._plans:
             self._plans[key] = _Plan(self, B, H, W, table_T)
         return self._plans[key]
@@ -345,7 +345,14 @@
         cabi.check(self.lib.ld_tuning_get(name.encode(), C.byref(v)), "tuning_get")
         return int(v.value)
 
-    def _separate_act(self, px, c):
+    def _separate_act(self, px, c, gn_regs=False):
+        return not gn_regs and self.tn.separate_act and px <= self.tn.sep_act_max_px and c >= self.tn.sep_act_min_c
+
+    def _gn_regs(self, px, c, groups, wname):
+        if not self.tn.conv_gn_regs or self.dt == cabi.LD_F32 or self.P["w"][wname + ".weight"].data_ptr() in self.P["terms2"]:
+            return False
+        if c % groups or (c // groups) % 8:
+            return False
         return self.tn.separate_act and px <= self.tn.sep_act_max_px and c >= self.tn.sep_act_min_c
 
     def buf(self, h, w, c):
@@ -530,8 +537,9 @@
             self.meta[len(ops) - 1] = dict(what=what, family=what, bytes=nbytes, flops=flops)
             self.decl[len(ops) - 1] = ([t for t in reads if t is not None], [t for t in writes if t is not None])
 
-    def conv3(self, ops, srcs, wname, cout, h, w, stats=None, groups=8, weight=None, bias=None, addend=None, side=None):
+    def conv3(self, ops, srcs, wname, cout, h, w, stats=None, groups=8, weight=None, bias=None, addend=None, side=None, gn_regs=False):
         a = cabi.Conv3x3Args()
+        a.gn_regs = 1 if gn_regs else 0
         for i, s in enumerate(srcs):
             a.src[i] = s
         a.nsrc = len(srcs)
@@ -560,11 +568,11 @@
         big = blocks16 >= 512 and h >= 16 and not mt4
         big = big or (mt4 and h >= 16 and blocks16 >= self._kt("conv_big4_min"))
         dname = {cabi.LD_F32: "f32", cabi.LD_BF16: "bf16", cabi.LD_F16: "f16"}[self.dt]
-        if side is not None:
+        if side is not None or gn_regs:
             big = False
         fam = f"conv3x3<{dname},{4 if mt4 else 2},{4 if big else 2}>"
         ck = 16 if self.dt == cabi.LD_F32 else 32
-        if side is not None:
+        if side is not None or gn_regs:
             pass
         elif (cout == 32 and len(srcs) == 1 and cin == ck and addend is None and h >= 32 and w >= 32 and h % 16 == 0
                 and w % 16 == 0 and (w // 16) * (h // 16) * self.B >= self._kt("conv_c32_min_tiles")
@@ -579,7 +587,7 @@
                 fam = f"conv3x3_s32<{dname}>"
         in_el = sum(s.C * (npx // 4 if s.upsample else npx) for s in srcs)
         side_b = (in_el + npx * cout + cin * cout) * self.esize + 4 * cout if side is not None else 0
-        self._call(ops, self.lib.ld_conv3x3, a, "conv3x3 " + wname + (" + res_conv" if side is not None else ""),
+        self._call(ops, self.lib.ld_conv3x3, a, "conv3x3 " + wname + (" + res_conv" if side is not None else "") + (" (gn regs)" if gn_regs else ""),
                    dict(family=fam, bytes=(in_el + npx * cout + 9 * cin * cout) * self.esize + 4 * cout + side_b,
                         flops=2 * (9 + (1 if side is not None else 0)) * cin * cout * npx, shape=f"{cin}->{cout}@{h}x{w}"),
                    reads=[s._tensor for s in srcs] + [addend], writes=[out, side_out])
@@ -675,10 +683,11 @@
         film = self.films.get(p)
         n1 = self.src(raw1, cout, gn=(s1, f[p + ".block1.norm.weight"], f[p + ".block1.norm.bias"], G),
                       act=cabi.ACT_SILU, film=film)
-        if self._separate_act(h * w, cout):
+        regs = self._gn_regs(h * w, cout, G, p + ".block2.proj")
+        if self._separate_act(h * w, cout, regs):
             act1 = self.gn_apply(ops, n1, None, h, w, cout)
             n1 = self.src(act1, cout)
-        raw2 = self.conv3(ops, [n1], p + ".block2.proj", cout, h, w, stats=s2, groups=G)
+        raw2 = self.conv3(ops, [n1], p + ".block2.proj", cout, h, w, stats=s2, groups=G, gn_regs=regs)
         n2 = self.src(raw2, cout, gn=(s2, f[p + ".block2.norm.weight"], f[p + ".block2.norm.bias"], G),
                       act=cabi.ACT_SILU)
         if rc is not None:
@@ -700,9 +709,10 @@
                           weight=self.P["w"][p + ".block1.proj.weight#x"], bias=zero, addend=p1)
         n1 = self.src(raw1, c, gn=(s1, f[p + ".block1.norm.weight"], f[p + ".block1.norm.bias"], G),
                       act=cabi.ACT_SILU, film=self.films.get(p))
-        if self._separate_act(h * w, c):
+        regs = self._gn_regs(h * w, c, G, p + ".block2.proj")
+        if self._separate_act(h * w, c, regs):
             n1 = self.src(self.gn_apply(ops, n1, None, h, w, c), c)
-        raw2 = self.conv3(ops, [n1], p + ".block2.proj", c, h, w, stats=s2, groups=G)
+        raw2 = self.conv3(ops, [n1], p + ".block2.proj", c, h, w, stats=s2, groups=G, gn_regs=regs)
         n2 = self.src(raw2, c, gn=(s2, f[p + ".block2.norm.weight"], f[p + ".block2.norm.bias"], G), act=cabi.ACT_SILU)
         out = self.conv1(ops, [self.src(x, c)], self.P["w"][p + ".res_conv.weight#x"], c, h, w, bias=None,
                          epi=cabi.EPI_GN_TAIL, gn_tail=n2, residual=p2, what="res_conv+tail " + p)
```
